# lyclyc52/NeRF_RPN

Measured on AMD Instinct MI355X. Metric: scenes/sec (160^3x4 grids, VGG19-3D+FPN+RPN fwd+bwd), higher is better.
Workload: dtype bf16; 1 GPU; configs[1]: one 160x160x160x4 rgb-sigma grid per GPU, VGG19-EF 3D + FPN + anchor RPN (OBB, 16 GT boxes per scene), fwd+bwd+clip+AdamW, random-init weights; scenes_per_gpu=1, parallelism=dp1, world_size_seen=1, backend=single process

## Files before the change

include/nerfrpn.h:

```cpp
#ifndef NERFRPN_H
#define NERFRPN_H

#include <stddef.h>
#include <stdint.h>

#ifdef __cplusplus
extern "C" {
#endif

typedef void *nrpn_stream_t;

enum nrpn_status {
  NRPN_OK = 0,
  NRPN_ERR_ARG = -1,
  NRPN_ERR_LAUNCH = -2,
  NRPN_ERR_DEVICE = -3
};

enum nrpn_dtype { NRPN_F32 = 0, NRPN_BF16 = 1 };

const char *nrpn_last_error(void);
int nrpn_abi_version(void);
int nrpn_check_device(int ordinal);

// ... 2 lines not shown
int nrpn_iou3d_obb_pair_f32(const float *b1, const float *b2, float *iou, int64_t n, nrpn_stream_t stream);
int nrpn_rotated_iou_loss_f32(const float *pred, const float *target, int64_t n, int mode, float *loss, float *grad, float *iou,
                              nrpn_stream_t stream);
int nrpn_projection_loss_f32(const float *pred, const float *target, int64_t n, int box_dim, const float *views, const float *intrinsics,
                             float beta, float max_mesh_dim, float *out, nrpn_stream_t stream);
int nrpn_recall_match_f32(float *overlaps, int num_proposals, int num_gt, float *covered, nrpn_stream_t stream);
int nrpn_ap_mark(const int64_t *order, const float *best_iou, const int64_t *key, int64_t n, int64_t num_keys, float iou_thresh,
                 int32_t *first_ws, uint8_t *tp, nrpn_stream_t stream);
int nrpn_iou3d_matrix_f32(const float *a, const float *b, float *iou, int64_t n, int64_t m, int box_dim,
                          nrpn_stream_t stream);

size_t nrpn_nms3d_workspace_bytes(int64_t n_max);
int nrpn_nms3d(const float *boxes, const int32_t *levels, const int32_t *d_count, int64_t n_max, int box_dim,
               float thr, uint8_t *keep, void *workspace, nrpn_stream_t stream);

int nrpn_segmented_topk_f32(const float *scores, const int64_t *h_offsets, int nseg, int k,
                            int32_t *out_idx, float *out_val, nrpn_stream_t stream);
size_t nrpn_segmented_topk_workspace_bytes(int nseg, int k);
int nrpn_segmented_topk_f32_ws(const float *scores, const int64_t *h_offsets, int nseg, int k,
                               int32_t *out_idx, float *out_val, void *workspace, size_t workspace_bytes, nrpn_stream_t stream);

int64_t nrpn_anchor_table_words(int levels, int anchors_per_cell);
int nrpn_anchors_f32(const int32_t *table, const int64_t *sel, int64_t count, float *anchors, nrpn_stream_t stream);
int nrpn_decode_boxes_f32(const int32_t *table, const float *deltas, const int64_t *sel, int64_t count,
                          int coder, float *boxes, nrpn_stream_t stream);
int nrpn_encode_boxes_f32(const int32_t *table, const float *gt, const int64_t *sel, int64_t count,
                          int coder, float *deltas, nrpn_stream_t stream);

int nrpn_coder_pairs_f32(const float *in, const float *anchors, int64_t count, int coder, int encode, float *out,
                         nrpn_stream_t stream);
int nrpn_head_flatten_f32(const float *head, int64_t cells, int ld, int anchors_per_cell, int dw, float *logits,
                          float *deltas, nrpn_stream_t stream);
int nrpn_head_unflatten(const float *g_logits, const float *g_deltas, int64_t cells, int ld, int anchors_per_cell, int dw,
                        const float *scale2, void *d_head, int dtype, nrpn_stream_t stream);

size_t nrpn_filter_workspace_bytes(int64_t n, int box_dim);
int nrpn_filter_candidates_f32(const float *boxes, const float *logits, const int32_t *levels,
                               const uint8_t *cand_valid, int64_t n, int box_dim, const float *h_grid_size3,
                               float min_size, float score_thresh, int fix_obb_clip, float *out_boxes,
                               float *out_scores, int32_t *out_levels, int32_t *d_count, void *workspace,
                               nrpn_stream_t stream);
int nrpn_select_kept_f32(const float *boxes, const float *scores, const int32_t *levels, const uint8_t *keep,
                         const int32_t *d_count, int64_t n, int box_dim, int post_top_n, float *out_boxes,
                         float *out_scores, float *out_levels, int32_t *d_out_count, nrpn_stream_t stream);

int nrpn_match_anchors_f32(const int32_t *table, int64_t total_anchors, const float *gt_aabb, int num_gt,
                           float fg_thresh, float bg_thresh, const float *h_ori_size3, float *labels,
                           int32_t *matched, float *workspace, nrpn_stream_t stream);
int nrpn_obb_to_aabb_f32(const float *obb, float *aabb, int64_t n, nrpn_stream_t stream);

size_t nrpn_sample_workspace_bytes(void);
int nrpn_sample_pos_neg(const float *labels, int64_t total, int max_pos, int batch, int64_t seed, void *workspace, int64_t *out_pos,
                        int64_t *out_neg, int32_t *counts, nrpn_stream_t stream);
int nrpn_rpn_sampled_loss_f32(const float *logits, const float *deltas, int dw, const float *targets,
                              const int64_t *pos, int64_t npos, const int64_t *neg, int64_t nneg, float beta,
                              float *loss2, float *g_logits, float *g_deltas, nrpn_stream_t stream);

enum { NRPN_CONV_BIAS = 1, NRPN_CONV_RELU = 2, NRPN_CONV_OUT_F32 = 4,
       NRPN_CONV_DEBUG_ALIAS_TAPS = 256, NRPN_CONV_DEBUG_NO_SYNC = 512,
       NRPN_CONV_DEBUG_STAGGER = 1024,
       NRPN_CONV_DEBUG_VARIANT = 0x3000 };
int nrpn_pack_conv_weight(const float *w_ref, int cout, int cin, int taps, int dtype, void *wp_fwd, void *wp_dgrad,
                          int rows_total, int row_offset, nrpn_stream_t stream);
int nrpn_unpack_conv_wgrad(const float *gw_packed, int cout, int cin, int taps, int rows_total, int row_offset,
                           float *gw_ref, int accumulate, int slices, nrpn_stream_t stream);
size_t nrpn_conv3d_fwd_workspace_bytes(int n, int gx, int gy, int gz, int cin, int cout, int ksize, int dtype);
int nrpn_conv3d_fwd(const void *x, const void *wp, const float *bias, void *y, int n, int gx, int gy, int gz, int cin,
                    int cout, int wrows, int ksize, int dtype, int flags, void *workspace, const void *relu_mask,
                    nrpn_stream_t stream);
enum { NRPN_TILE_AUTO = 0, NRPN_TILE_128 = 128, NRPN_TILE_256X128_WS = 256, NRPN_TILE_256X256 = 512, NRPN_TILE_256X256_W4 = 1024,
       NRPN_TILE_HALO = 2048  };
typedef struct nrpn_conv_opts {
  int32_t size;
  int32_t tile;
  int32_t lds_dma;
  int32_t kstep_bytes;
  int32_t stagger;
  int32_t big_split;
  int32_t debug;
  int32_t halo_pairing;
  const float *scale;
  const void *relu_mask;
  float *stats;
} nrpn_conv_opts;
int nrpn_conv3d_fwd_ex(const void *x, const void *wp, const float *bias, void *y, int n, int gx, int gy, int gz, int cin,
                       int cout, int wrows, int ksize, int dtype, int flags, void *workspace, const nrpn_conv_opts *opts,
                       nrpn_stream_t stream);
size_t nrpn_conv3d_fwd_workspace_bytes_ex(int n, int gx, int gy, int gz, int cin, int cout, int ksize, int dtype,
                                          const nrpn_conv_opts *opts);
int nrpn_conv3d_fwd_plan_ex(int n, int gx, int gy, int gz, int cin, int cout, int ksize, int dtype, const nrpn_conv_opts *opts);
int nrpn_conv3d_fwd_stats_rows_ex(int n, int gx, int gy, int gz, int cin, int cout, int ksize, int dtype, const nrpn_conv_opts *opts);
size_t nrpn_conv3d_wgrad_workspace_bytes(int n, int gx, int gy, int gz, int cin, int cout, int wrows, int ksize, int dtype);
int nrpn_conv3d_wgrad_slices(int n, int gx, int gy, int gz, int cin, int cout, int wrows, int ksize, int dtype);
enum { NRPN_WGRAD_ACC_BIAS = 1, NRPN_WGRAD_MASK_READY = 2,
       NRPN_WGRAD_DEFER_BIAS = 4  };
int nrpn_conv3d_wgrad(const void *x, const void *dy, float *gw_packed, float *gbias, int n, int gx, int gy, int gz,
                      int cin, int cout, int wrows, int ksize, int dtype, int accumulate_bias, void *workspace,
                      nrpn_stream_t stream);
int nrpn_conv3d_fwd_ragged(const void *x, const void *wp, const float *bias, void *y, int nseg, const int32_t *dims, int cin,
                           int cout, int wrows, int ksize, int dtype, int flags, void *workspace, nrpn_stream_t stream);
int nrpn_conv3d_wgrad_ragged(const void *x, const void *dy, float *gw_packed, float *gbias, int nseg, const int32_t *dims,
                             int cin, int cout, int wrows, int ksize, int dtype, int accumulate_bias, void *workspace,
                             nrpn_stream_t stream);
size_t nrpn_cone_workspace_bytes(int64_t total_voxels);
int nrpn_cone_build(const int64_t *pos, const int64_t *neg, const int32_t *counts, int n_scenes, int64_t pos_stride, int64_t neg_stride,
                    int nlevels, const int64_t *level_anchor_off, int num_anchors, const int32_t *dims, int depth, uint32_t *lists,
                    int64_t cap, int32_t *counts_out, void *workspace, nrpn_stream_t stream);
size_t nrpn_conv3d_fwd_rows_workspace_bytes(int64_t nrows, int cin, int cout, int ksize, int dtype);
int nrpn_conv3d_fwd_rows(const void *x, const void *wp, const float *bias, void *y, const uint32_t *rows, int64_t nrows, int nseg,
                         const int32_t *dims, int cin, int cout, int wrows, int ksize, int dtype, int flags, const void *relu_mask,
                         void *workspace, nrpn_stream_t stream);
int nrpn_conv3d_wgrad_rows(const void *x, const void *dy, float *gw_packed, float *gbias, const uint32_t *rows, int64_t nrows, int nseg,
                           const int32_t *dims, int cin, int cout, int wrows, int ksize, int dtype, int accumulate_bias, void *workspace,
                           nrpn_stream_t stream);
int nrpn_conv3d_fwd_plan(int n, int gx, int gy, int gz, int cin, int cout, int ksize, int dtype);
int nrpn_conv3d_fwd_stats_rows(int n, int gx, int gy, int gz, int cin, int cout, int ksize, int dtype);
int nrpn_conv3d_fwd_stats(const void *x, const void *wp, const float *bias, void *y, int n, int gx, int gy, int gz, int cin,
                          int cout, int wrows, int ksize, int dtype, int flags, float *stats, nrpn_stream_t stream);
int nrpn_bn_stats_finalize(const float *partials, int nparts, int64_t rows, int c, float *mean, float *var, float *running_mean,
                           float *running_var, float momentum, nrpn_stream_t stream);
int nrpn_conv3d_wgrad_plan(int n, int gx, int gy, int gz, int cin, int cout, int wrows, int ksize, int dtype);
int nrpn_stem_kpad(int dtype);
int nrpn_pack_stem_weight(const float *w_ref, int cout, int dtype, void *wp, nrpn_stream_t stream);
int nrpn_stem_wgrad_slices(int n, int gx, int gy, int gz, int cout, int stride, int dtype);
int64_t nrpn_stem_wgrad_slice_floats(int n, int gx, int gy, int gz, int cout, int stride, int dtype);
int nrpn_unpack_stem_wgrad(const float *gw_packed, int cout, int dtype, float *gw_ref, int accumulate, int slices,
                           int64_t slice_floats, nrpn_stream_t stream);
int nrpn_conv3d_stem_fwd(const void *x, const void *wp, const float *bias, void *y, int n, int gx, int gy, int gz,
                         int cout, int stride, int dtype, int flags, nrpn_stream_t stream);
int nrpn_stem_halo_supported(int gz, int cout, int stride, int dtype);
int nrpn_stem_halo_kpad(void);
int nrpn_pack_stem_weight_halo(const float *w_ref, int cout, void *wp, nrpn_stream_t stream);
int nrpn_conv3d_stem_fwd_halo(const void *x, const void *wp, const float *bias, const float *scale, void *y, int n, int gx, int gy,
                              int gz, int cout, int flags, nrpn_stream_t stream);
int nrpn_conv3d_stem_fwd_ex(const void *x, const void *wp, const float *bias, void *y, int n, int gx, int gy, int gz,
                            int cout, int stride, int dtype, int flags, const nrpn_conv_opts *opts, nrpn_stream_t stream);
size_t nrpn_stem_wgrad_workspace_bytes(int n, int gx, int gy, int gz, int cout, int stride, int dtype);
int nrpn_conv3d_stem_wgrad(const void *x, const void *dy, float *gw_packed, float *gbias, int n, int gx, int gy, int gz,
                           int cout, int stride, int dtype, int accumulate_bias, void *workspace, nrpn_stream_t stream);

size_t nrpn_bn_workspace_bytes(int64_t rows, int c);
int nrpn_bn_stats(const void *x, int64_t rows, int c, int dtype, float *mean, float *var, float *running_mean,
                  float *running_var, float momentum, void *workspace, nrpn_stream_t stream);
int nrpn_bn_apply(const void *x, void *y, int64_t rows, int c, int dtype, const float *mean, const float *var,
                  const float *gamma, const float *beta, float eps, int relu, nrpn_stream_t stream);
int nrpn_bn_backward(const void *x, const void *y, const void *dy, void *dx, int64_t rows, int c, int dtype,
                     const float *mean, const float *var, const float *gamma, const float *beta, float eps, int relu,
                     float *dgamma, float *dbeta, float *acc_dgamma, float *acc_dbeta, void *workspace, nrpn_stream_t stream);
int nrpn_relu_backward(const void *y, const void *dy, void *dx, int64_t count, int dtype, nrpn_stream_t stream);
int nrpn_pool_out_size(int in, int k, int s, int p, int ceil_mode);
int nrpn_maxpool3d_fwd(const void *x, void *y, int8_t *argmax, int n, int gx, int gy, int gz, int c, int k, int s,
                       int p, int ceil_mode, int dtype, nrpn_stream_t stream);
int nrpn_maxpool3d_bwd(const void *dy, const int8_t *argmax, void *dx, int n, int gx, int gy, int gz, int c, int k,
                       int s, int p, int ceil_mode, int dtype, nrpn_stream_t stream);
int nrpn_upsample_add_fwd(void *fine, const void *coarse, int n, int fx, int fy, int fz, int cx, int cy, int cz, int c,
                          int dtype, nrpn_stream_t stream);
int nrpn_upsample_add_bwd(const void *dfine, void *dcoarse, int n, int fx, int fy, int fz, int cx, int cy, int cz,
                          int c, int dtype, int accumulate, nrpn_stream_t stream);
int nrpn_subsample3d(const void *src, void *dst, int n, int gx, int gy, int gz, int c, int stride, int backward, int dtype,
                     nrpn_stream_t stream);
int nrpn_add_relu(const void *a, const void *b, void *y, int64_t count, int relu, int dtype, nrpn_stream_t stream);
int nrpn_ingest_rgbsigma(const void *src, int src_is_u8, void *dst, int64_t voxels, int alpha_mode, int dtype, nrpn_stream_t stream);
int nrpn_ingest_augment(const void *src, int src_is_u8, void *dst, int w, int l, int h, int alpha_mode, int dtype, int rot90,
                        int z_up, int flip0, int flip1, const float *h_xform, nrpn_stream_t stream);
int nrpn_ncdhw_to_ndhwc(const float *src, void *dst, int n, int c, int64_t voxels, int dtype, nrpn_stream_t stream);
int nrpn_ndhwc_to_ncdhw(const void *src, float *dst, int n, int c, int64_t voxels, int dtype, nrpn_stream_t stream);
int nrpn_cast(const void *src, void *dst, int64_t count, int src_dtype, int dst_dtype, nrpn_stream_t stream);
size_t nrpn_column_sum_workspace_bytes(int64_t rows, int c);
int nrpn_column_sum_f32(const float *x, int64_t rows, int c, float *out, int accumulate, void *workspace, nrpn_stream_t stream);
int nrpn_split_bf16x3(const float *src, int64_t rows, int c, void *interleaved, int ipattern, void *planes, int nplanes, int ppattern,
                      nrpn_stream_t stream);

int nrpn_patchify(const void *x, void *y, int n, int gx, int gy, int gz, int patch, int dtype, nrpn_stream_t stream);
int nrpn_layernorm_fwd(const void *x, void *y, const float *gamma, const float *beta, float *mean, float *rstd, int64_t rows,
                       int c, float eps, int dtype, nrpn_stream_t stream);
size_t nrpn_layernorm_workspace_bytes(int64_t rows, int c);
int nrpn_layernorm_bwd(const void *x, const void *dy, void *dx, const float *gamma, const float *mean, const float *rstd,
                       float *dgamma, float *dbeta, int64_t rows, int c, int dtype, int accumulate_params, void *workspace,
                       nrpn_stream_t stream);
int nrpn_gelu(const void *x, const void *dy, void *out, int64_t count, int backward, int dtype, nrpn_stream_t stream);
int nrpn_scale_add(const void *a, const void *b, const float *scale, void *y, int n, int64_t per_sample, int dtype,
                   nrpn_stream_t stream);
int nrpn_patch_merge(const void *src, void *dst, int n, int gx, int gy, int gz, int c, int backward, int dtype,
                     nrpn_stream_t stream);
int nrpn_window_attn_fwd(const void *qkv, const float *qkv_bias, const float *bias_table, const int32_t *rel_index, void *out,
                         int n, int gx, int gy, int gz, int c, int heads, int shift, int dtype, nrpn_stream_t stream);
size_t nrpn_window_attn_bwd_workspace_bytes(int n, int gx, int gy, int gz, int heads);
int nrpn_window_attn_bwd(const void *qkv, const float *qkv_bias, const float *bias_table, const int32_t *rel_index,
                         const void *dout, void *dqkv, float *dtable, float *dbias_pad, int n, int gx, int gy, int gz, int c,
                         int heads, int shift, int dtype, int accumulate_table, void *workspace, nrpn_stream_t stream);

size_t nrpn_groupnorm_workspace_bytes(int n, int c, int groups);
int nrpn_groupnorm_fwd(const void *x, void *y, const float *gamma, const float *beta, float *mean, float *rstd, int n,
                       int64_t rows, int c, int groups, float eps, int relu, int dtype, void *workspace, nrpn_stream_t stream);
int nrpn_groupnorm_bwd(const void *x, const void *y, const void *dy, void *dx, const float *gamma, const float *mean,
                       const float *rstd, float *dgamma, float *dbeta, int n, int64_t rows, int c, int groups, int relu, int dtype,
                       int accumulate_params, void *workspace, nrpn_stream_t stream);
int nrpn_fcos_reduce_floats(void);
int nrpn_fcos_head_out_f32(const float *cls_out, const float *box_out, int wrows, const float *scale, float stride_mul,
                           int norm_reg, int reg_dim, int ctr_on_reg, int64_t rows, float *logits, float *reg, float *ctr,
                           nrpn_stream_t stream);
int nrpn_fcos_head_out_bwd_f32(const float *box_out, int wrows, const float *scale, float stride_mul, int norm_reg, int reg_dim,
                               int ctr_on_reg, int64_t rows, const float *d_logits, const float *d_reg, const float *d_ctr,
                               float *d_cls_out, float *d_box_out, float *d_scale, nrpn_stream_t stream);
int nrpn_fcos_gt_summary_f32(const float *gt, int count, int width, float *summary, nrpn_stream_t stream);
int nrpn_fcos_targets_f32(const float *summary, const int32_t *gt_offsets, int n, int levels, const int32_t *dims,
                          const int32_t *strides, const float *ori_sizes, float radius, int norm_reg, int reg_dim, int8_t *labels,
                          float *reg_targets, int32_t *num_pos, nrpn_stream_t stream);
int nrpn_fcos_focal_f32(const float *logits, const int8_t *labels, int64_t count, float alpha, float *loss_sum, float *dlogits,
                        nrpn_stream_t stream);
int nrpn_fcos_scores_f32(const float *logits, const float *ctr, int n, int levels, const int32_t *dims, const int32_t *strides,
                         const float *ori_sizes, float pre_nms_thresh, float *scores, nrpn_stream_t stream);
int nrpn_fcos_decode_f32(const int32_t *idx, const float *score, int64_t count, int64_t seg_len, const float *reg, int n,
                         int levels, const int32_t *dims, const int32_t *strides, const float *ori_sizes, int reg_dim,
                         float min_size, float *boxes, float *out_scores, float *out_levels, nrpn_stream_t stream);

int nrpn_roi_align_rotated_3d_fwd(const void *feat, const float *rois, int num_rois, int n, int x, int y, int z, int c,
                                  float spatial_scale, int pw, int pl, int ph, int sampling_ratio, void *out, int dtype,
                                  nrpn_stream_t stream);
size_t nrpn_roi_align_rotated_3d_bwd_workspace_bytes(int n, int x, int y, int z, int c);
int nrpn_roi_align_rotated_3d_bwd(const void *grad_out, const float *rois, int num_rois, int n, int x, int y, int z, int c,
                                  float spatial_scale, int pw, int pl, int ph, int sampling_ratio, void *grad_in, void *workspace,
                                  int dtype, nrpn_stream_t stream);

size_t nrpn_roipool_bwd_workspace_bytes(int x, int y, int z, int c);
int nrpn_roipool_aabb_fwd(const void *feat, int x, int y, int z, int c, const int32_t *crop, const int32_t *level_of, int level, int num_rois,
                          int o0, int o1, int o2, float *out, int32_t *argmax, int dtype, nrpn_stream_t stream);
int nrpn_roipool_aabb_bwd(const float *dout, const int32_t *argmax, const int32_t *crop, const int32_t *level_of, int level, int num_rois,
                          int x, int y, int z, int c, int o0, int o1, int o2, void *dfeat, void *workspace, int dtype, nrpn_stream_t stream);
int nrpn_roipool_obb_fwd(const void *feat, int x, int y, int z, int c, const float *rois, const int32_t *level_of, int level, int num_rois,
                         float scale, int interpolation, int o0, int o1, int o2, float *out, int32_t *argmax, int dtype, nrpn_stream_t stream);
// ... 125 lines not shown
```

nerf_rpn_amd/csrc/common.h:

```cpp
#pragma once
#include <hip/hip_runtime.h>
#include <hip/hip_bf16.h>

#include <cstdarg>
#include <cstdint>
#include <cstdio>

#include "../../include/nerfrpn.h"
#include "../../include/nerfrpn_tools.h"

int nrpn_fail(int code, const char *fmt, ...);

#define NRPN_REQUIRE(cond, ...)                                 \
  do {                                                          \
    if (!(cond)) return nrpn_fail(NRPN_ERR_ARG, __VA_ARGS__);   \
  } while (0)

#define NRPN_HIP(call)                                                                          \
  do {                                                                                          \
    hipError_t e_ = (call);                                                                     \
    if (e_ != hipSuccess) return nrpn_fail(NRPN_ERR_LAUNCH, "%s: %s", #call, hipGetErrorString(e_)); \
  } while (0)

#define NRPN_LAUNCH_CHECK(name)                                                                  \
  do {                                                                                           \
    hipError_t e_ = hipGetLastError();                                                           \
    if (e_ != hipSuccess) return nrpn_fail(NRPN_ERR_LAUNCH, "%s: %s", name, hipGetErrorString(e_)); \
  } while (0)

struct FastDiv {
  unsigned m, sh, d;
};
static inline FastDiv make_fastdiv(unsigned d) {
  FastDiv f{0u, 0u, d};
  if (d <= 1) return f;
  unsigned l = 0;
  while ((1ull << l) < d) ++l;
  f.m = (unsigned)((((unsigned long long)1 << (31 + l)) + d - 1) / d);
  f.sh = l - 1;
  return f;
}
__device__ __forceinline__ unsigned fastdiv(unsigned n, const FastDiv &f) { return f.d == 1 ? n : (__umulhi(n, f.m) >> f.sh); }


int nrpn_ensure_dynamic_lds(const void *kernel, int bytes);
#define NRPN_LDS(kernel, bytes)                                                                         \
  do {                                                                                                  \
    if (int rc_ = nrpn_ensure_dynamic_lds(reinterpret_cast<const void *>(kernel), (int)(bytes))) return rc_; \
  } while (0)

static inline hipStream_t as_stream(nrpn_stream_t s) { return reinterpret_cast<hipStream_t>(s); }
static inline int64_t cdiv64(int64_t a, int64_t b) { return (a + b - 1) / b; }

__device__ __forceinline__ float bf16_bits_to_f32(unsigned short h) { return __uint_as_float(((unsigned)h) << 16); }
__device__ __forceinline__ unsigned short f32_to_bf16_bits(float f) { return __builtin_bit_cast(unsigned short, (__bf16)f); }

template <typename T> struct elem;
template <> struct elem<float> {
  static __device__ __forceinline__ float ld(const float *p) { return *p; }
  static __device__ __forceinline__ void st(float *p, float v) { *p = v; }
};
template <> struct elem<unsigned short> {
  static __device__ __forceinline__ float ld(const unsigned short *p) { return bf16_bits_to_f32(*p); }
  static __device__ __forceinline__ void st(unsigned short *p, float v) { *p = f32_to_bf16_bits(v); }
};
```

nerf_rpn_amd/csrc/conv3d.hip:

```cpp
#include "conv_common.cuh"

#ifndef NRPN_HALO_PAIRING_DEFAULT
#define NRPN_HALO_PAIRING_DEFAULT 2
#endif

template <typename T, int BN, int MODE, bool OUTF32, int KB, bool GLDS, int BM = 128, bool ROWS = false>
__global__ void __launch_bounds__(256, BM == 128 ? 2 : 1) conv_igemm_kernel(const ConvArgs p) {
  constexpr int WAVES_N = (BN == 128) ? 2 : 1;
  constexpr int TM = BM / (32 * (4 / WAVES_N));
  constexpr int TN = 2;
  constexpr int KE = KB / (int)sizeof(T);
  constexpr int PPR = KB / 16;
  constexpr int RSTEP = 256 / PPR;
  constexpr int A_RPT = BM / RSTEP;
  constexpr int B_RPT = BN / RSTEP;
  constexpr int SWZ_SH = (KB == 64) ? 2 : 1;
  constexpr int A_BYTES = BM * KB, B_BYTES = BN * KB;
  extern __shared__ __attribute__((aligned(16))) char lds[];

  const int tid = threadIdx.x, lane = tid & 63, wave = tid >> 6;
  const int wm = wave / WAVES_N, wn = wave % WAVES_N;
  const unsigned ntiles = (p.Cout + BN - 1) / BN;
  const unsigned tiles = (unsigned)((p.M + BM - 1) / BM) * ntiles;
  unsigned zsplit, tile;
  int my_ks = p.ksplit > 1 ? p.ksplit : 1;
  long long part_row0 = 0;
  if (p.tail_ks > 1) {
    const unsigned full = (unsigned)p.tail_tile0 * ntiles;
    if (blockIdx.x < full) {
      zsplit = 0; my_ks = 1;
      tile = xcd_remap(blockIdx.x, full);
    } else {
      const unsigned t = blockIdx.x - full, ntail = tiles - full;
      zsplit = t / ntail; my_ks = p.tail_ks;
      tile = full + t % ntail;
      part_row0 = (long long)p.tail_tile0 * BM;
    }
  } else {
    zsplit = blockIdx.x / tiles;
    tile = xcd_remap(blockIdx.x - zsplit * tiles, tiles);
  }
  const long long m0 = (long long)(tile / ntiles) * BM;
  const int n0 = (int)(tile % ntiles) * BN;
  const int lr = tid / PPR, ls = tid % PPR;

  long long a_off[A_RPT];
  int a_x[A_RPT], a_y[A_RPT], a_z[A_RPT];
  bool a_ok[A_RPT];
  unsigned a_mask[A_RPT];
  int a_yz[A_RPT], a_zs[A_RPT];
  long long a_nbase[A_RPT];
#pragma unroll
  for (int i = 0; i < A_RPT; ++i) {
    const long long v = m0 + lr + RSTEP * i;
    a_ok[i] = v < p.M;
    const long long vv = a_ok[i] ? v : 0;
    int ox, oy, oz, gX = p.X, gY = p.Y, gZ = p.Z;
    long long n = 0;
    unsigned row_word = 0;
    long long row_vox = vv;
    if (MODE == 0 && ROWS) {
      if (a_ok[i]) { row_vox = p.rows[2 * vv]; row_word = p.rows[2 * vv + 1]; }
      const int seg = (int)(row_word >> 27);
#pragma unroll
      for (int q = 0; q < kMaxSeg; ++q)
        if (q == seg && q < p.segs.n) { gY = p.segs.Y[q]; gZ = p.segs.Z[q]; }
      ox = oy = oz = 0;
    } else if (MODE == 0) {
      if (p.segs.n == 0) {
        const unsigned u = (unsigned)vv, sc = fastdiv(u, p.dvs), local = u - sc * (unsigned)(p.X * p.Y * p.Z), t1 = fastdiv(local, p.dvz);
        oz = (int)(local - t1 * (unsigned)p.Z);
        ox = (int)fastdiv(t1, p.dvy);
        oy = (int)(t1 - (unsigned)ox * (unsigned)p.Y);
      } else {
        locate_voxel(p.segs, vv, p.X, p.Y, p.Z, ox, oy, oz, gX, gY, gZ);
      }
    } else {
      oz = (int)(vv % p.OZ);
      const long long t1 = vv / p.OZ;
      oy = (int)(t1 % p.OY);
      const long long t2 = t1 / p.OY;
      ox = (int)(t2 % p.OX);
      n = t2 / p.OX;
    }
    a_x[i] = ox; a_y[i] = oy; a_z[i] = oz;
    a_yz[i] = gY * gZ * p.Cin * (int)sizeof(T);
    a_zs[i] = gZ * p.Cin * (int)sizeof(T);
    a_off[i] = (MODE == 0) ? row_vox * p.Cin : 0;
    a_nbase[i] = (MODE == 0) ? 0 : n * (long long)p.X * p.Y * p.Z * 4;
// ... 134 lines not shown
    const char *A = lds + buf * (A_BYTES + B_BYTES);
    const char *B = A + A_BYTES;
#pragma unroll
    for (int s = 0; s < KB / 32; ++s) {
      f4 af[TM], bfv[TN];
#pragma unroll
      for (int i = 0; i < TM; ++i) {
        const int r = (wm * TM + i) * 32 + fr;
        af[i] = *reinterpret_cast<const f4 *>(A + r * KB + (((s * 2 + fk) ^ ((r >> SWZ_SH) & (PPR - 1))) << 4));
      }
#pragma unroll
      for (int j = 0; j < TN; ++j) {
        const int r = (wn * TN + j) * 32 + fr;
        bfv[j] = *reinterpret_cast<const f4 *>(B + r * KB + (((s * 2 + fk) ^ ((r >> SWZ_SH) & (PPR - 1))) << 4));
      }
#pragma unroll
      for (int i = 0; i < TM; ++i)
#pragma unroll
        for (int j = 0; j < TN; ++j) Mma<T>::run(acc[i][j], af[i], bfv[j]);
    }
  };

  int ks = ks_begin;
  if (GLDS && MODE == 0) {
    issue_glds(0);
    __syncthreads();
    for (; ks + 1 < ks_end; ks += 2) {
      issue_glds(1);
      compute_step(0);
      __syncthreads();
      if (ks + 2 < ks_end) issue_glds(0);
      compute_step(1);
      __syncthreads();
    }
    if (ks < ks_end) {
      compute_step(0);
      __syncthreads();
    }
  } else {
    load_step(ks_begin, ra0, rb0);
    store_step(0, ra0, rb0);
    __syncthreads();
    for (; ks + 1 < ks_end; ks += 2) {
      load_step(ks + 1, ra0, rb0);
      compute_step(0);
      store_step(1, ra0, rb0);
      __syncthreads();
      if (ks + 2 < ks_end) load_step(ks + 2, ra0, rb0);
      compute_step(1);
      if (ks + 2 < ks_end) store_step(0, ra0, rb0);
      __syncthreads();
    }
    if (ks < ks_end) {
      compute_step(0);
      __syncthreads();
    }
  }

  if (my_ks > 1) {
    float *wsz = p.ws + (long long)zsplit * (p.M - part_row0) * p.Cout;
#pragma unroll
    for (int j = 0; j < TN; ++j) {
      const int col = n0 + (wn * TN + j) * 32 + fr;
      if (col >= p.Cout) continue;
#pragma unroll
      for (int i = 0; i < TM; ++i)
#pragma unroll
        for (int r = 0; r < 16; ++r) {
          const long long v = m0 + (wm * TM + i) * 32 + frag_row(r, lane);
          if (v < p.M) wsz[(v - part_row0) * p.Cout + col] = acc[i][j][r];
        }
    }
    return;
  }

  const bool has_bias = (p.flags & NRPN_CONV_BIAS) && p.bias;
  const bool relu = p.flags & NRPN_CONV_RELU;
  constexpr int PITCH = 144;
  if (sizeof(T) == 2 && !OUTF32 && 2 * (A_BYTES + B_BYTES) >= 4 * TM * 32 * PITCH && (p.Cout & 7) == 0) {
    char *stage = lds + wave * (TM * 32 * PITCH);
    const T *maskp = reinterpret_cast<const T *>(p.mask);
    T *yp = reinterpret_cast<T *>(p.y);
    const bool full_tile = m0 + BM <= p.M;
#pragma unroll
    for (int j = 0; j < TN; ++j) {
      const int col = n0 + (wn * TN + j) * 32 + fr;
      const float bv = (has_bias && col < p.Cout) ? p.bias[col] : 0.f;
      const float sv = (p.scale && col < p.Cout) ? p.scale[col] : 1.f;
      float ssum = 0.f, qsum = 0.f;
#pragma unroll
      for (int i = 0; i < TM; ++i)
#pragma unroll
        for (int r = 0; r < 16; ++r) {
          float o = acc[i][j][r] * sv + bv;
          if (relu) o = fmaxf(o, 0.f);
          const bf16s ob = f32_to_bf16_bits(o);
          *reinterpret_cast<bf16s *>(stage + (i * 32 + frag_row(r, lane)) * PITCH + (j * 32 + fr) * 2) = ob;
          if (p.stats && (full_tile || m0 + (wm * TM + i) * 32 + frag_row(r, lane) < p.M)) {
            const float of = bf16_bits_to_f32(ob);
            ssum += of;
            qsum += of * of;
          }
        }
      if (p.stats) store_col_stats(p.stats, (m0 / BM) * (BM / (TM * 32)) + wm, p.Cout, col, ssum, qsum, lane);
    }
    asm volatile("s_waitcnt lgkmcnt(0)" ::: "memory");
#pragma unroll
    for (int q = 0; q < TM * 4; ++q) {
      const int pc = lane + 64 * q;
      const int row = pc >> 3, seg = pc & 7;
      const long long vt = m0 + wm * (TM * 32) + row;
      const int col = n0 + wn * 64 + seg * 8;
      if (vt < p.M && col < p.Cout) {
        const long long v = ROWS ? (long long)p.rows[2 * vt] : vt;
        f4 val = *reinterpret_cast<const f4 *>(stage + row * PITCH + seg * 16);
        if (maskp) {
          typedef __attribute__((ext_vector_type(8))) unsigned short u8v;
          const u8v mk = __builtin_bit_cast(u8v, *reinterpret_cast<const f4 *>(maskp + v * p.Cout + col));
          u8v ov = __builtin_bit_cast(u8v, val);
#pragma unroll
          for (int e = 0; e < 8; ++e) ov[e] = (bf16_bits_to_f32(mk[e]) > 0.f) ? ov[e] : (unsigned short)0;
          val = __builtin_bit_cast(f4, ov);
        }
        *reinterpret_cast<f4 *>(yp + v * p.Cout + col) = val;
      }
    }
    return;
  }
#pragma unroll
  for (int j = 0; j < TN; ++j) {
    const int col = n0 + (wn * TN + j) * 32 + fr;
    if (col >= p.Cout) continue;
    const float bv = has_bias ? p.bias[col] : 0.f;
    const float sv = p.scale ? p.scale[col] : 1.f;
#pragma unroll
    for (int i = 0; i < TM; ++i) {
#pragma unroll
      for (int r = 0; r < 16; ++r) {
        const long long vt = m0 + (wm * TM + i) * 32 + frag_row(r, lane);
        if (vt < p.M) {
          const long long v = ROWS ? (long long)p.rows[2 * vt] : vt;
          float o = acc[i][j][r] * sv + bv;
          if (relu) o = fmaxf(o, 0.f);
          if (p.mask && !(elem<T>::ld(reinterpret_cast<const T *>(p.mask) + v * p.Cout + col) > 0.f)) o = 0.f;
          if (OUTF32) reinterpret_cast<float *>(p.y)[v * p.Cout + col] = o;
          else elem<T>::st(reinterpret_cast<T *>(p.y) + v * p.Cout + col, o);
        }
      }
    }
  }
}

template <bool OUTF32>
__global__ void __launch_bounds__(512, 1) conv_igemm_ws_kernel(const ConvArgs p) {
  typedef bf16s T;
  constexpr int BM = 256, BN = 128, KB = 128, KE = 64, PPR = 8, RSTEP = 32, TM = 4, TN = 2;
  constexpr int A_RPT = BM / RSTEP, B_RPT = BN / RSTEP;
  constexpr int A_BYTES = BM * KB, B_BYTES = BN * KB;
  extern __shared__ __attribute__((aligned(16))) char lds[];

  const int tid = threadIdx.x, lane = tid & 63, wave = tid >> 6;
  const bool producer = wave >= 4;
  const unsigned ntiles = (p.Cout + BN - 1) / BN;
  const unsigned tiles = (unsigned)((p.M + BM - 1) / BM) * ntiles;
  const unsigned tile = xcd_remap(blockIdx.x, tiles);
  const long long m0 = (long long)(tile / ntiles) * BM;
  const int n0 = (int)(tile % ntiles) * BN;
  const int cpt = p.Cin / KE;
  const int nk = p.taps * cpt;

  if (producer) {
    const int ptid = tid - 256, lr = ptid / PPR, ls = ptid % PPR;
    const int wave_u = __builtin_amdgcn_readfirstlane(wave - 4);
    const __amdgpu_buffer_rsrc_t xr = make_rsrc(p.x, p.x_bytes), wr = make_rsrc(p.w, p.w_bytes);
    unsigned a_voff[A_RPT], a_mask[A_RPT], b_voff[B_RPT];
#pragma unroll
    for (int i = 0; i < A_RPT; ++i) {
      const int r = lr + RSTEP * i;
      const long long v = m0 + r;
      const bool ok = v < p.M;
      const long long vv = ok ? v : 0;
      const int oz = (int)(vv % p.OZ);
      const long long t1 = vv / p.OZ;
      const int oy = (int)(t1 % p.OY);
      const int ox = (int)((t1 / p.OY) % p.OX);
      unsigned m = 0;
      if (ok) {
        if (p.taps == 27) {
#pragma unroll
          for (int t = 0; t < 27; ++t) {
            const int dx = t / 9 - 1, dy = (t / 3) % 3 - 1, dz = t % 3 - 1;
            const bool in = (unsigned)(ox + dx) < (unsigned)p.X && (unsigned)(oy + dy) < (unsigned)p.Y && (unsigned)(oz + dz) < (unsigned)p.Z;
            m |= in ? (1u << t) : 0u;
          }
        } else {
          m = 1u;
        }
      }
      a_mask[i] = m;
      a_voff[i] = (unsigned)(vv * p.Cin * 2) + ((ls ^ ((r >> 1) & (PPR - 1))) << 4);
    }
#pragma unroll
    for (int i = 0; i < B_RPT; ++i) {
      const int r = lr + RSTEP * i, row = n0 + r;
      b_voff[i] = row < p.wrows ? (unsigned)((long long)row * p.Cin * 2) + ((ls ^ ((r >> 1) & (PPR - 1))) << 4) : kOOB;
    }
    int l_tap = 0, l_chunk = 0, l_dx = 0, l_dy = 0, l_dz = 0;
    if (p.taps == 27) { l_dx = -1; l_dy = -1; l_dz = -1; }
    const long long w_tap_stride = (long long)p.wrows * p.Cin;
// ... 640 lines not shown
      for (int q = 0; q < 8; ++q) {
        const int pc = elane + 64 * q;
        const int row = pc >> 4, seg = pc & 15;
        const long long v = m0 + (wm * TM + i) * 32 + row;
        const int col = n0 + wn * 128 + seg * 8;
        if (v < p.M && col < p.Cout) {
          f4 val = *reinterpret_cast<const f4 *>(stage + row * PITCH + seg * 16);
          if (maskp) {
            typedef __attribute__((ext_vector_type(8))) unsigned short u8v;
            const u8v mk = __builtin_bit_cast(u8v, *reinterpret_cast<const f4 *>(maskp + v * p.Cout + col));
            u8v ov = __builtin_bit_cast(u8v, val);
#pragma unroll
            for (int e = 0; e < 8; ++e) ov[e] = (bf16_bits_to_f32(mk[e]) > 0.f) ? ov[e] : (unsigned short)0;
            val = __builtin_bit_cast(f4, ov);
          }
          *reinterpret_cast<f4 *>(yp + v * p.Cout + col) = val;
        }
      }
      asm volatile("s_waitcnt lgkmcnt(0)" ::: "memory");
    }
    if (p.stats) {
#pragma unroll
      for (int j = 0; j < TN; ++j)
        store_col_stats(p.stats, (m0 / BM) * 2 + wm, p.Cout, n0 + (wn * TN + j) * 32 + efr, ssum[j], qsum[j], elane);
    }
    return;
  }
#pragma unroll
  for (int j = 0; j < TN; ++j) {
    const int col = n0 + (wn * TN + j) * 32 + efr;
    if (col >= p.Cout) continue;
    const float bv = has_bias ? p.bias[col] : 0.f;
    const float sv = p.scale ? p.scale[col] : 1.f;
#pragma unroll
    for (int i = 0; i < TM; ++i) {
#pragma unroll
      for (int r = 0; r < 16; ++r) {
        const long long v = m0 + (wm * TM + i) * 32 + frag_row(r, elane);
        if (v < p.M) {
          float o = acc[i][j][r] * sv + bv;
          if (relu) o = fmaxf(o, 0.f);
          if (p.mask && !(elem<T>::ld(reinterpret_cast<const T *>(p.mask) + v * p.Cout + col) > 0.f)) o = 0.f;
          if (OUTF32) reinterpret_cast<float *>(p.y)[v * p.Cout + col] = o;
          else elem<T>::st(reinterpret_cast<T *>(p.y) + v * p.Cout + col, o);
        }
      }
    }
  }
}

namespace hk { constexpr int TX = 4, TY = 8, TZ = 8; }
int nrpn_launch_conv_halo(const ConvArgs &a, unsigned workgroups, hipStream_t st, int variant);

template <typename T, bool OUTF32>
__global__ void splitk_epilogue_kernel(const float *__restrict__ ws, const float *__restrict__ bias, void *__restrict__ y, long long total,
                                       int cout, int relu, int nslices, const T *__restrict__ mask, const float *__restrict__ scale) {
  for (long long i = (long long)blockIdx.x * blockDim.x + threadIdx.x; i < total; i += (long long)gridDim.x * blockDim.x) {
    float o = ws[i];
    for (int z = 1; z < nslices; ++z) o += ws[z * total + i];
    if (scale) o *= scale[i % cout];
    o += bias ? bias[i % cout] : 0.f;
    if (relu) o = fmaxf(o, 0.f);
    if (mask && !(elem<T>::ld(mask + i) > 0.f)) o = 0.f;
    if (OUTF32) reinterpret_cast<float *>(y)[i] = o;
    else elem<T>::st(reinterpret_cast<T *>(y) + i, o);
  }
}

template <typename T, bool OUTF32>
__global__ void rows_epilogue_kernel(const float *__restrict__ ws, const float *__restrict__ bias, void *__restrict__ y, long long total,
                                     int cout, int relu, int nslices, const T *__restrict__ mask, const unsigned *__restrict__ rows) {
  for (long long i = (long long)blockIdx.x * blockDim.x + threadIdx.x; i < total; i += (long long)gridDim.x * blockDim.x) {
    float o = ws[i];
    for (int z = 1; z < nslices; ++z) o += ws[z * total + i];
    const long long r = i / cout;
    const int col = (int)(i - r * cout);
    const long long dst = (long long)rows[2 * r] * cout + col;
    o += bias ? bias[col] : 0.f;
    if (relu) o = fmaxf(o, 0.f);
    if (mask && !(elem<T>::ld(mask + dst) > 0.f)) o = 0.f;
    if (OUTF32) reinterpret_cast<float *>(y)[dst] = o;
    else elem<T>::st(reinterpret_cast<T *>(y) + dst, o);
  }
}

struct Knobs {
  int glds;
  int bm;
  int stagger;
  int big_split;
  int kb;
  int dbg;
  int halo_auto;
  int halo_xp;
};
static std::atomic<int> g_conv_glds{1}, g_conv_bm{0}, g_conv_stagger{1}, g_conv_big_split{1}, g_conv_kb{128}, g_conv_halo_auto{1}, g_conv_halo_xp{NRPN_HALO_PAIRING_DEFAULT};
static Knobs resolve_knobs(const nrpn_conv_opts *o, int flags = 0) {
  Knobs k{g_conv_glds.load(std::memory_order_relaxed), g_conv_bm.load(std::memory_order_relaxed), g_conv_stagger.load(std::memory_order_relaxed),
          g_conv_big_split.load(std::memory_order_relaxed), g_conv_kb.load(std::memory_order_relaxed),
          flags & (NRPN_CONV_DEBUG_ALIAS_TAPS | NRPN_CONV_DEBUG_NO_SYNC | NRPN_CONV_DEBUG_STAGGER | NRPN_CONV_DEBUG_VARIANT), g_conv_halo_auto.load(std::memory_order_relaxed),
          g_conv_halo_xp.load(std::memory_order_relaxed)};
  if (o) {
    if (o->halo_pairing == 1 || o->halo_pairing == 2) k.halo_xp = o->halo_pairing == 1 ? 1 : 0;
    if (o->tile > 0) k.bm = o->tile;
    if (o->lds_dma >= 0) k.glds = o->lds_dma ? 1 : 0;
    if (o->kstep_bytes == 64 || o->kstep_bytes == 128) k.kb = o->kstep_bytes;
    if (o->stagger >= 0) k.stagger = o->stagger ? 1 : 0;
    if (o->big_split >= 0) k.big_split = o->big_split ? 1 : 0;
    k.dbg |= o->debug & (NRPN_CONV_DEBUG_ALIAS_TAPS | NRPN_CONV_DEBUG_NO_SYNC | NRPN_CONV_DEBUG_STAGGER | NRPN_CONV_DEBUG_VARIANT);
  }
  return k;
}
extern "C" int nrpn_set_conv_lds_dma(int on) { g_conv_glds = on ? 1 : 0; return NRPN_OK; }
extern "C" int nrpn_set_conv_halo_auto(int on) { g_conv_halo_auto = on ? 1 : 0; return NRPN_OK; }
extern "C" int nrpn_set_conv_halo_pairing(int mode) { g_conv_halo_xp = (mode == 1 || mode == 2) ? mode : 0; return NRPN_OK; }
extern "C" int nrpn_set_conv_stagger(int on) { g_conv_stagger = on ? 1 : 0; return NRPN_OK; }
extern "C" int nrpn_set_conv_big_split(int on) { g_conv_big_split = on ? 1 : 0; return NRPN_OK; }
extern "C" int nrpn_set_conv_kstep_bytes(int kb) {
  if (kb != 64 && kb != 128) return nrpn_fail(NRPN_ERR_ARG, "conv k-step must be 64 or 128 bytes");
  g_conv_kb = kb;
  return NRPN_OK;
}
extern "C" int nrpn_set_conv_tile_m(int bm) {
  if (bm != 0 && bm != 128 && bm != 256 && bm != 512 && bm != 1024 && bm != 2048)
    return nrpn_fail(NRPN_ERR_ARG, "conv tile selector must be 0 (auto), 128 (128x128), 256 (wave-specialised 256x128), 512 (256x256, 8 waves), "
                                   "1024 (256x256, 4 waves) or 2048 (halo form of the 3x3x3 kernel)");
  g_conv_bm = bm;
  return NRPN_OK;
}

static int conv_ksplit(long long M, int cout, int cin, int taps, int elem_bytes, const Knobs &kn) {
  const int bn = cout <= 64 ? 64 : 128;
  const long long tiles = cdiv64(M, 128) * ((cout + bn - 1) / bn);
  const int kb = (kn.kb == 128 && (cin * elem_bytes) % 128 == 0) ? 128 : 64;
  const int nk = taps * (cin * elem_bytes / kb);
  if (tiles >= 128 || nk < 16) return 1;
  long long s = (384 + tiles - 1) / tiles;
  if (s > nk / 8) s = nk / 8;
  if (s > 64) s = 64;
  if (s < 2) return 1;
  const long long per = (nk + s - 1) / s;
  s = (nk + per - 1) / per;
  return s < 2 ? 1 : (int)s;
}

static int conv_big_split(long long M, int cout, int cin, int taps, int elem_bytes, const Knobs &kn) {
  if (!kn.big_split) return 0;
  if (elem_bytes != 2 || !kn.glds || kn.kb != 128 || (kn.bm != 0 && kn.bm != 512 && kn.bm != 1024) || cout < 256 || (cin * 2) % 128 != 0) return 0;
  const long long tiles = cdiv64(M, 256) * ((cout + 255) / 256);
  if (tiles < 48 || tiles >= 200) return 0;
  const int nk = taps * (cin / 64);
  int s = (int)((256 + tiles - 1) / tiles);
  if (s > 8) s = 8;
  while (s > 1 && nk / s < 8) --s;
  return s >= 2 ? s : 0;
}

struct TailSplit { int tile0, ks; };
static TailSplit conv_tail_split(long long M, int cout, int cin, int taps, int elem_bytes, const Knobs &kn) {
  TailSplit none{0, 0};
  if (elem_bytes != 2 || !kn.glds || kn.kb != 128 || !kn.big_split || cout > 256 || cout < 256 || (cin * 2) % 128 != 0) return none;
  const long long tiles = cdiv64(M, 256);
  const long long rem = tiles % 256;
  if (tiles <= 256 || rem == 0 || rem > 128) return none;
  const int nk = taps * (cin / 64);
  int ks = (int)(256 / rem);
  if (ks > 8) ks = 8;
  while (ks > 1 && nk / ks < 8) --ks;
  if (ks < 2) return none;
  const int per = (nk + ks - 1) / ks;
  ks = (nk + per - 1) / per;
  return ks >= 2 ? TailSplit{(int)(tiles - rem), ks} : none;
}

template <typename K>
static int launch_igemm(K kernel, dim3 grid, size_t lds, hipStream_t st, const ConvArgs &a) {
  if (lds > 64 * 1024) NRPN_LDS(kernel, (int)lds);
  hipLaunchKernelGGL(kernel, grid, dim3(256), lds, st, a);
  return NRPN_OK;
}

struct Grid { int n, gx, gy, gz; };
static long long halo_tiles(const Grid &g) {
  return (long long)g.n * ((g.gx + hk::TX - 1) / hk::TX) * ((g.gy + hk::TY - 1) / hk::TY) * ((g.gz + hk::TZ - 1) / hk::TZ);
}
static bool halo_ok(const Grid &g, int cin, int cout, int taps, int elem_bytes, bool out_f32, const Knobs &kn) {
  (void)out_f32;
  if (g.n <= 0 || taps != 27 || elem_bytes != 2 || !kn.glds || (cin % 32) != 0 || (cout & 7) != 0 || cout < 256) return false;
  if (kn.bm != 2048 && !(kn.bm == 0 && kn.halo_auto)) return false;
  const long long tiles = halo_tiles(g) * ((cout + 255) / 256);
  const double waste = (double)halo_tiles(g) * 256.0 / ((double)g.n * g.gx * g.gy * g.gz);
  if (kn.bm == 2048) return true;
  return tiles >= 200 && waste <= 1.12;
}

static int conv_tile_kind(long long M, int cout, int cin, int elem_bytes, bool sliced_big, bool ragged, const Knobs &kn) {
  const bool wide = kn.kb == 128 && (cin * elem_bytes) % 128 == 0;
  const bool can = kn.glds && wide && cout > 64 && elem_bytes == 2;
  const long long tiles_big = cdiv64(M, 256) * ((cout + 255) / 256);
  const bool huge = can && cout >= 256 && (sliced_big || kn.bm == 512 || kn.bm == 1024 || (kn.bm == 0 && tiles_big >= 200));
  if (huge) return (kn.bm == 1024 && !ragged) ? 5 : 1;
  if (can && kn.bm == 256 && !ragged) return 4;
  return 0;
}

template <typename T, int MODE>
static int launch_conv(const ConvArgs &a, bool out_f32, hipStream_t st, const Knobs &kn) {
  const int bn = (a.Cout <= 64) ? 64 : 128;
  constexpr bool kDma = (MODE == 0);
  const bool wide = MODE == 0 && kn.kb == 128 && (a.Cin * (int)sizeof(T)) % 128 == 0;
  const int kind = (kDma && (a.ksplit <= 1 || a.slices)) ? conv_tile_kind(a.M, a.Cout, a.Cin, (int)sizeof(T), a.slices != 0, a.segs.n > 0, kn) : 0;
  const bool huge = kind == 1 || kind == 5, big = kind == 4;
  const int bm = (big || huge) ? 256 : 128;
  if (a.stats) {
    const bool staged = MODE == 0 && sizeof(T) == 2 && !out_f32 && (a.Cout & 7) == 0 && a.ksplit <= 1 && !big && (huge || wide);
    if (!staged) return nrpn_fail(NRPN_ERR_ARG, "conv3d_fwd_stats: this shape does not run a kernel with fused statistics (ask nrpn_conv3d_fwd_stats_rows first)");
  }
  dim3 grid((unsigned)(cdiv64(a.M, bm) * ((a.Cout + (huge ? 256 : bn) - 1) / (huge ? 256 : bn)) * (a.ksplit > 1 ? a.ksplit : 1)));
  if (a.tail_ks > 1) {
    if (kind != 1) return nrpn_fail(NRPN_ERR_ARG, "conv3d_fwd: internal: tail split planned for a shape that does not run the 256x256 tile");
    const long long mt = cdiv64(a.M, 256), nt = (a.Cout + 255) / 256;
    grid = dim3((unsigned)(a.tail_tile0 * nt + (mt - a.tail_tile0) * nt * a.tail_ks));
  }
  int rc = 0;
#define NRPN_LC(BN_, OF_, KB_)                                                                                                    \
  do {                                                                                                                           \
    const size_t lds_ = 2 * (size_t)(128 + BN_) * KB_;                                                                           \
    if (kDma && kn.glds) rc = launch_igemm(conv_igemm_kernel<T, BN_, MODE, OF_, KB_, kDma>, grid, lds_, st, a);                  \
    else rc = launch_igemm(conv_igemm_kernel<T, BN_, MODE, OF_, KB_, false>, grid, lds_, st, a);                                 \
  } while (0)
#define NRPN_LC2(BN_, OF_) do { if (wide) NRPN_LC(BN_, OF_, 128); else NRPN_LC(BN_, OF_, 64); } while (0)
#define NRPN_LBIG(...)                                                                       \
  do {                                                                                       \
    NRPN_LDS((conv_igemm_big_kernel<__VA_ARGS__>), (int)lds_);                               \
    hipLaunchKernelGGL((conv_igemm_big_kernel<__VA_ARGS__>), grid, dim3(512), lds_, st, a);  \
  } while (0)
  if (kind == 5) {
    if constexpr (MODE == 0 && sizeof(T) == 2) {
      const size_t lds_ = 2 * (size_t)(256 + 256) * 128;
      if (out_f32) {
        NRPN_LDS((conv_igemm_big4_kernel<true>), (int)lds_);
        hipLaunchKernelGGL(conv_igemm_big4_kernel<true>, grid, dim3(256), lds_, st, a);
      } else {
        NRPN_LDS((conv_igemm_big4_kernel<false>), (int)lds_);
        hipLaunchKernelGGL(conv_igemm_big4_kernel<false>, grid, dim3(256), lds_, st, a);
      }
    }
  } else if (huge) {
    if constexpr (MODE == 0 && sizeof(T) == 2) {
      const size_t lds_ = 2 * (size_t)(256 + 256) * 128;
      const int dbg = ((kn.dbg & NRPN_CONV_DEBUG_ALIAS_TAPS) ? 1 : 0) | ((kn.dbg & NRPN_CONV_DEBUG_NO_SYNC) ? 2 : 0);
      if (!out_f32 && (kn.stagger || (kn.dbg & NRPN_CONV_DEBUG_STAGGER))) {
        if (dbg == 0) NRPN_LBIG(false, true, 0);
        else if (dbg == 1) NRPN_LBIG(false, true, 1);
        else if (dbg == 2) NRPN_LBIG(false, true, 2);
        else NRPN_LBIG(false, true, 3);
      } else if (out_f32) {
        NRPN_LBIG(true, false, 0);
      } else {
        NRPN_LBIG(false, false, 0);
      }
    }
  } else if (big) {
    if constexpr (MODE == 0 && sizeof(T) == 2) {
      const size_t lds_ = 3 * (size_t)(256 + 128) * 128;
      if (out_f32) {
        NRPN_LDS((conv_igemm_ws_kernel<true>), (int)lds_);
        hipLaunchKernelGGL(conv_igemm_ws_kernel<true>, grid, dim3(512), lds_, st, a);
      } else {
        NRPN_LDS((conv_igemm_ws_kernel<false>), (int)lds_);
        hipLaunchKernelGGL(conv_igemm_ws_kernel<false>, grid, dim3(512), lds_, st, a);
      }
    }
  } else if (bn == 64) { if (out_f32) NRPN_LC2(64, true); else NRPN_LC2(64, false); }
  else { if (out_f32) NRPN_LC2(128, true); else NRPN_LC2(128, false); }
#undef NRPN_LBIG
#undef NRPN_LC2
#undef NRPN_LC
  if (rc) return rc;
  NRPN_LAUNCH_CHECK("conv_igemm");
  return NRPN_OK;
}

static size_t fwd_workspace_bytes(long long M, int cin, int cout, int ksize, int dtype, const Knobs &kn, const Grid &g) {
  if (halo_ok(g, cin, cout, ksize == 3 ? 27 : 1, dtype == NRPN_F32 ? 4 : 2, false, kn)) return 0;
  const int bs = conv_big_split(M, cout, cin, ksize == 3 ? 27 : 1, dtype == NRPN_F32 ? 4 : 2, kn);
  if (bs) return (size_t)bs * M * cout * 4;
  const int s = conv_ksplit(M, cout, cin, ksize == 3 ? 27 : 1, dtype == NRPN_F32 ? 4 : 2, kn);
  if (s > 1) return (size_t)s * M * cout * 4;
  if (conv_tile_kind(M, cout, cin, dtype == NRPN_F32 ? 4 : 2, false, false, kn) == 1) {
    const TailSplit t = conv_tail_split(M, cout, cin, ksize == 3 ? 27 : 1, dtype == NRPN_F32 ? 4 : 2, kn);
    if (t.ks > 1) return (size_t)t.ks * (M - (long long)t.tile0 * 256) * cout * 4;
  }
  return 0;
}
extern "C" size_t nrpn_conv3d_fwd_workspace_bytes(int n, int gx, int gy, int gz, int cin, int cout, int ksize, int dtype) {
  return fwd_workspace_bytes((long long)n * gx * gy * gz, cin, cout, ksize, dtype, resolve_knobs(nullptr), Grid{n, gx, gy, gz});
}
extern "C" size_t nrpn_conv3d_fwd_workspace_bytes_ex(int n, int gx, int gy, int gz, int cin, int cout, int ksize, int dtype,
                                                     const nrpn_conv_opts *opts) {
  return fwd_workspace_bytes((long long)n * gx * gy * gz, cin, cout, ksize, dtype, resolve_knobs(opts), Grid{n, gx, gy, gz});
}

static int fwd_plan(long long M, int cin, int cout, int ksize, int dtype, const Knobs &kn, const Grid &g) {
  const int es = dtype == NRPN_F32 ? 4 : 2, taps = ksize == 3 ? 27 : 1;
  if (halo_ok(g, cin, cout, taps, es, false, kn)) return 7;
  if (conv_big_split(M, cout, cin, taps, es, kn)) return conv_tile_kind(M, cout, cin, es, true, false, kn) == 5 ? 6 : 2;
  if (conv_ksplit(M, cout, cin, taps, es, kn) > 1) return 3;
  return conv_tile_kind(M, cout, cin, es, false, false, kn);
}
extern "C" int nrpn_conv3d_fwd_plan(int n, int gx, int gy, int gz, int cin, int cout, int ksize, int dtype) {
  return fwd_plan((long long)n * gx * gy * gz, cin, cout, ksize, dtype, resolve_knobs(nullptr), Grid{n, gx, gy, gz});
}
extern "C" int nrpn_conv3d_fwd_plan_ex(int n, int gx, int gy, int gz, int cin, int cout, int ksize, int dtype, const nrpn_conv_opts *opts) {
  return fwd_plan((long long)n * gx * gy * gz, cin, cout, ksize, dtype, resolve_knobs(opts), Grid{n, gx, gy, gz});
}

static int conv3d_fwd_impl(const void *x, const void *wp, const float *bias, const void *mask, void *y, long long M, int gx, int gy, int gz, const Segs *segs,
                           int cin, int cout, int wrows, int ksize, int dtype, int flags, void *workspace, nrpn_stream_t stream,
                           float *stats = nullptr, const nrpn_conv_opts *opts = nullptr) {
  NRPN_REQUIRE(ksize == 1 || ksize == 3, "conv3d_fwd: ksize must be 1 or 3 (got %d)", ksize);
  NRPN_REQUIRE(dtype == NRPN_F32 || dtype == NRPN_BF16, "conv3d_fwd: bad dtype %d", dtype);
  NRPN_REQUIRE(M > 0 && gx > 0 && gy > 0 && gz > 0 && cin > 0 && cout > 0 && wrows >= cout, "conv3d_fwd: bad sizes");
  const int es = dtype == NRPN_F32 ? 4 : 2;
  NRPN_REQUIRE((cin * es) % 64 == 0, "conv3d_fwd: Cin*elemsize must be a multiple of 64 bytes (Cin=%d)", cin);
  NRPN_REQUIRE(x && wp && y, "conv3d_fwd: null pointer");
  const Knobs kn = resolve_knobs(opts, flags);
  ConvArgs a{};
  a.x = x; a.w = wp; a.bias = bias; a.mask = mask; a.y = y; a.stats = stats;
  a.scale = opts ? opts->scale : nullptr;
  a.M = M;
  a.X = gx; a.Y = gy; a.Z = gz; a.OX = gx; a.OY = gy; a.OZ = gz;
  if (segs) a.segs = *segs;
  a.dvz = make_fastdiv((unsigned)gz); a.dvy = make_fastdiv((unsigned)gy);
  a.dvs = make_fastdiv((unsigned)min((long long)gx * gy * gz, (1ll << 31) - 1));
  a.Cin = cin; a.Cout = cout; a.wrows = wrows; a.taps = ksize == 3 ? 27 : 1; a.stride = 1;
  a.flags = flags & 3;
  NRPN_REQUIRE(a.M * cin * es < (1ll << 31) && (long long)a.taps * wrows * cin * es < (1ll << 31),
               "conv3d_fwd: activation / weight tensors must stay below 2 GiB (32-bit buffer offsets)");
  a.x_bytes = (unsigned)(a.M * cin * es); a.w_bytes = (unsigned)((long long)a.taps * wrows * cin * es);
  const bool out_f32 = (flags & NRPN_CONV_OUT_F32) != 0;
  hipStream_t st = as_stream(stream);
  if (!segs && dtype == NRPN_BF16) {
    const Grid g{(int)(M / ((long long)gx * gy * gz)), gx, gy, gz};
    if (halo_ok(g, cin, cout, a.taps, es, out_f32, kn)) {
      const long long wgs = halo_tiles(g) * ((cout + 255) / 256);
      NRPN_REQUIRE(wgs < (1ll << 31), "conv3d_fwd: too many tiles");
      const bool xp = cin % 128 == 0 && !((kn.dbg >> 12) & 3) && (kn.halo_xp == 1 || (kn.halo_xp == 2 && cin >= 256));
      const int variant = ((kn.dbg >> 12) & 3) | (xp ? 4 : 0) | (out_f32 ? 8 : 0);
      return nrpn_launch_conv_halo(a, (unsigned)wgs, st, variant);
    }
  }
  const int bs = workspace ? conv_big_split(a.M, cout, cin, a.taps, es, kn) : 0;
  if (bs) {
    a.ksplit = bs; a.slices = 1; a.ws = reinterpret_cast<float *>(workspace);
  } else {
    a.ksplit = workspace ? conv_ksplit(a.M, cout, cin, a.taps, es, kn) : 1;
    if (a.ksplit > 1) a.ws = reinterpret_cast<float *>(workspace);
  }
  const int nsl = a.ksplit;
  if (a.ksplit <= 1 && workspace && !segs && !stats && !out_f32 && dtype == NRPN_BF16 && conv_tile_kind(a.M, cout, cin, es, false, false, kn) == 1) {
    const TailSplit t = conv_tail_split(a.M, cout, cin, a.taps, es, kn);
    if (t.ks > 1) { a.tail_tile0 = t.tile0; a.tail_ks = t.ks; a.ws = reinterpret_cast<float *>(workspace); }
  }
  int rc = (dtype == NRPN_F32) ? launch_conv<float, 0>(a, true, st, kn) : launch_conv<bf16s, 0>(a, out_f32, st, kn);
  if (!rc && a.tail_ks > 1) {
    const long long row0 = (long long)a.tail_tile0 * 256, total = (a.M - row0) * cout;
    const int blocks = (int)min((long long)2048, (total + 255) / 256);
    const float *b = (flags & NRPN_CONV_BIAS) ? bias : nullptr;
    const bf16s *mk = a.mask ? reinterpret_cast<const bf16s *>(a.mask) + row0 * cout : nullptr;
    hipLaunchKernelGGL((splitk_epilogue_kernel<bf16s, false>), dim3(blocks), dim3(256), 0, st, a.ws, b, reinterpret_cast<bf16s *>(y) + row0 * cout, total, cout,
                       (flags & NRPN_CONV_RELU) ? 1 : 0, a.tail_ks, mk, a.scale);
    NRPN_LAUNCH_CHECK("splitk_epilogue (tail)");
    return NRPN_OK;
  }
  if (rc || a.ksplit <= 1) return rc;
  const long long total = a.M * cout;
  const int blocks = (int)min((long long)4096, (total + 255) / 256);
  const float *b = (flags & NRPN_CONV_BIAS) ? bias : nullptr;
  const int relu = (flags & NRPN_CONV_RELU) ? 1 : 0;
  if (dtype == NRPN_F32 || out_f32) {
    if (dtype == NRPN_F32) hipLaunchKernelGGL((splitk_epilogue_kernel<float, true>), dim3(blocks), dim3(256), 0, st, a.ws, b, y, total, cout, relu, nsl, (const float *)a.mask, a.scale);
    else hipLaunchKernelGGL((splitk_epilogue_kernel<bf16s, true>), dim3(blocks), dim3(256), 0, st, a.ws, b, y, total, cout, relu, nsl, (const bf16s *)a.mask, a.scale);
  } else {
    hipLaunchKernelGGL((splitk_epilogue_kernel<bf16s, false>), dim3(blocks), dim3(256), 0, st, a.ws, b, y, total, cout, relu, nsl, (const bf16s *)a.mask, a.scale);
  }
  NRPN_LAUNCH_CHECK("splitk_epilogue");
  return NRPN_OK;
}

extern "C" int nrpn_conv3d_fwd(const void *x, const void *wp, const float *bias, void *y, int n, int gx, int gy, int gz, int cin,
                               int cout, int wrows, int ksize, int dtype, int flags, void *workspace, const void *relu_mask,
                               nrpn_stream_t stream) {
  NRPN_REQUIRE(n > 0 && gx > 0 && gy > 0 && gz > 0, "conv3d_fwd: bad sizes");
  NRPN_REQUIRE(!relu_mask || !(flags & NRPN_CONV_OUT_F32) || dtype == NRPN_F32, "conv3d_fwd: relu_mask needs outputs in the input dtype");
  return conv3d_fwd_impl(x, wp, bias, relu_mask, y, (long long)n * gx * gy * gz, gx, gy, gz, nullptr, cin, cout, wrows, ksize, dtype, flags,
                         workspace, stream);
}

static int fwd_stats_rows(long long M, int cin, int cout, int ksize, int dtype, const Knobs &kn, const Grid &g) {
  if (dtype != NRPN_BF16 || (cout & 7) != 0 || !kn.glds || kn.bm == 256) return 0;
  const int plan = fwd_plan(M, cin, cout, ksize, dtype, kn, g);
  if (plan == 7) return (int)(halo_tiles(g) * 2);
  if (plan == 1 || plan == 5) return (int)(cdiv64(M, 256) * 2);
  if (plan != 0 || kn.kb != 128 || (cin * 2) % 128 != 0) return 0;
  return (int)(cdiv64(M, 128) * (cout <= 64 ? 4 : 2));
}
extern "C" int nrpn_conv3d_fwd_stats_rows(int n, int gx, int gy, int gz, int cin, int cout, int ksize, int dtype) {
  return fwd_stats_rows((long long)n * gx * gy * gz, cin, cout, ksize, dtype, resolve_knobs(nullptr), Grid{n, gx, gy, gz});
}
extern "C" int nrpn_conv3d_fwd_stats_rows_ex(int n, int gx, int gy, int gz, int cin, int cout, int ksize, int dtype, const nrpn_conv_opts *opts) {
  return fwd_stats_rows((long long)n * gx * gy * gz, cin, cout, ksize, dtype, resolve_knobs(opts), Grid{n, gx, gy, gz});
}

extern "C" int nrpn_conv3d_fwd_stats(const void *x, const void *wp, const float *bias, void *y, int n, int gx, int gy, int gz, int cin,
                                     int cout, int wrows, int ksize, int dtype, int flags, float *stats, nrpn_stream_t stream) {
  NRPN_REQUIRE(n > 0 && gx > 0 && gy > 0 && gz > 0 && stats, "conv3d_fwd_stats: bad sizes / null statistics buffer");
  NRPN_REQUIRE(nrpn_conv3d_fwd_stats_rows(n, gx, gy, gz, cin, cout, ksize, dtype) > 0 && !(flags & NRPN_CONV_OUT_F32) && wrows == cout,
               "conv3d_fwd_stats: this shape does not run a kernel with fused statistics");
  return conv3d_fwd_impl(x, wp, bias, nullptr, y, (long long)n * gx * gy * gz, gx, gy, gz, nullptr, cin, cout, wrows, ksize, dtype, flags,
                         nullptr, stream, stats);
}

extern "C" int nrpn_conv3d_fwd_ex(const void *x, const void *wp, const float *bias, void *y, int n, int gx, int gy, int gz, int cin,
                                  int cout, int wrows, int ksize, int dtype, int flags, void *workspace, const nrpn_conv_opts *opts,
                                  nrpn_stream_t stream) {
  NRPN_REQUIRE(n > 0 && gx > 0 && gy > 0 && gz > 0, "conv3d_fwd_ex: bad sizes");
  NRPN_REQUIRE(!opts || opts->size == (int32_t)sizeof(nrpn_conv_opts), "conv3d_fwd_ex: opts->size must be sizeof(nrpn_conv_opts)");
  const void *mask = opts ? opts->relu_mask : nullptr;
  float *stats = opts ? opts->stats : nullptr;
  NRPN_REQUIRE(!mask || !(flags & NRPN_CONV_OUT_F32) || dtype == NRPN_F32, "conv3d_fwd_ex: relu_mask needs outputs in the input dtype");
  if (stats) {
    NRPN_REQUIRE(fwd_stats_rows((long long)n * gx * gy * gz, cin, cout, ksize, dtype, resolve_knobs(opts), Grid{n, gx, gy, gz}) > 0 && !(flags & NRPN_CONV_OUT_F32) &&
                     wrows == cout && !mask,
                 "conv3d_fwd_ex: this shape / plan does not run a kernel with fused statistics (nrpn_conv3d_fwd_stats_rows_ex)");
    workspace = nullptr;
  }
  return conv3d_fwd_impl(x, wp, bias, mask, y, (long long)n * gx * gy * gz, gx, gy, gz, nullptr, cin, cout, wrows, ksize, dtype, flags,
                         workspace, stream, stats, opts);
}

extern "C" int nrpn_conv3d_fwd_ragged(const void *x, const void *wp, const float *bias, void *y, int nseg, const int32_t *dims, int cin,
                                      int cout, int wrows, int ksize, int dtype, int flags, void *workspace, nrpn_stream_t stream) {
  Segs sg{};
  long long M = 0;
  if (int rc = fill_segs(sg, nseg, dims, M)) return rc;
  return conv3d_fwd_impl(x, wp, bias, nullptr, y, M, 1, 1, 1, &sg, cin, cout, wrows, ksize, dtype, flags, workspace, stream);
}

static std::atomic<int> g_rows_big{0};
extern "C" int nrpn_set_rows_big_tile(int on) { g_rows_big = on ? 1 : 0; return NRPN_OK; }

static int rows_ksplit(long long nrows, int cin, int cout, int taps, int es) {
  const long long tiles = cdiv64(nrows, 128) * ((cout + 127) / 128);
  const int nk = taps * (cin * es / 128);
  if (tiles >= 128 || nk < 12) return 1;
  long long s = (256 + tiles - 1) / tiles;
  if (s > nk / 6) s = nk / 6;
  if (s > 32) s = 32;
  if (s < 2) return 1;
  const long long per = (nk + s - 1) / s;
  s = (nk + per - 1) / per;
  return s < 2 ? 1 : (int)s;
}
static std::atomic<int> g_rows_tail{1};
extern "C" int nrpn_set_rows_tail_split(int on) { g_rows_tail = on ? 1 : 0; return NRPN_OK; }
static TailSplit rows_tail_split(long long nrows, int cin, int cout, int taps, int es) {
  TailSplit none{0, 0};
  if (!g_rows_tail.load(std::memory_order_relaxed)) return none;
  const long long mt = cdiv64(nrows, 128), nt = (cout + 127) / 128, tiles = mt * nt;
  const long long rem = tiles % 512;
  if (tiles <= 512 || rem == 0 || rem > 256) return none;
  const long long tail_mt = (rem + nt - 1) / nt;
  const int nk = taps * (cin * es / 128);
  int ks = (int)(512 / (tail_mt * nt));
  if (ks > 8) ks = 8;
  while (ks > 1 && nk / ks < 6) --ks;
  if (ks < 2) return none;
  const int per = (nk + ks - 1) / ks;
  ks = (nk + per - 1) / per;
  return ks >= 2 ? TailSplit{(int)(mt - tail_mt), ks} : none;
}
extern "C" size_t nrpn_conv3d_fwd_rows_workspace_bytes(int64_t nrows, int cin, int cout, int ksize, int dtype) {
  const int es = dtype == NRPN_F32 ? 4 : 2, taps = ksize == 3 ? 27 : 1;
  const int s = rows_ksplit(nrows, cin, cout, taps, es);
  if (s > 1) return (size_t)s * nrows * cout * 4;
  const TailSplit t = rows_tail_split(nrows, cin, cout, taps, es);
  return t.ks > 1 ? (size_t)t.ks * (nrows - (long long)t.tile0 * 128) * cout * 4 : 0;
}

extern "C" int nrpn_conv3d_fwd_rows(const void *x, const void *wp, const float *bias, void *y, const uint32_t *rows, int64_t nrows, int nseg,
                                    const int32_t *dims, int cin, int cout, int wrows, int ksize, int dtype, int flags, const void *relu_mask,
                                    void *workspace, nrpn_stream_t stream) {
  NRPN_REQUIRE(ksize == 1 || ksize == 3, "conv3d_fwd_rows: ksize must be 1 or 3 (got %d)", ksize);
  NRPN_REQUIRE(dtype == NRPN_F32 || dtype == NRPN_BF16, "conv3d_fwd_rows: bad dtype %d", dtype);
  NRPN_REQUIRE(x && wp && y && rows && nrows >= 0 && cin > 0 && cout > 0 && wrows >= cout, "conv3d_fwd_rows: bad arguments");
  if (nrows == 0) return NRPN_OK;
  const int es = dtype == NRPN_F32 ? 4 : 2;
  NRPN_REQUIRE((cin * es) % 128 == 0, "conv3d_fwd_rows: Cin*elemsize must be a multiple of 128 bytes (Cin=%d)", cin);
  const bool out_f32 = (flags & NRPN_CONV_OUT_F32) != 0 || dtype == NRPN_F32;
  NRPN_REQUIRE(!relu_mask || !(flags & NRPN_CONV_OUT_F32) || dtype == NRPN_F32, "conv3d_fwd_rows: relu_mask needs outputs in the input dtype");
  ConvArgs a{};
  long long total = 0;
  if (int rc = fill_segs(a.segs, nseg, dims, total)) return rc;
  a.x = x; a.w = wp; a.bias = bias; a.mask = relu_mask; a.y = y; a.rows = rows;
  a.M = nrows;
  a.X = a.Y = a.Z = a.OX = a.OY = a.OZ = 1;
  a.Cin = cin; a.Cout = cout; a.wrows = wrows; a.taps = ksize == 3 ? 27 : 1; a.stride = 1; a.flags = flags & 3; a.ksplit = 1;
  NRPN_REQUIRE(total * cin * es < (1ll << 31) && total * cout * 4 < (1ll << 32) && (long long)a.taps * wrows * cin * es < (1ll << 31),
               "conv3d_fwd_rows: activation / weight tensors must stay below 2 GiB (32-bit buffer offsets)");
  a.x_bytes = (unsigned)(total * cin * es); a.w_bytes = (unsigned)((long long)a.taps * wrows * cin * es);
  hipStream_t st = as_stream(stream);
  const int ks = workspace ? rows_ksplit(nrows, cin, cout, a.taps, es) : 1;
  if (ks > 1) { a.ksplit = ks; a.ws = reinterpret_cast<float *>(workspace); }
  if (g_rows_big.load(std::memory_order_relaxed) && dtype == NRPN_BF16 && !out_f32 && ks == 1 && cout >= 256 && (cout & 7) == 0 &&
      cdiv64(nrows, 256) * ((cout + 255) / 256) >= 96) {
    const size_t lds_big = 2 * (size_t)(256 + 256) * 128;
    dim3 gbig((unsigned)(cdiv64(nrows, 256) * ((cout + 255) / 256)));
    NRPN_LDS((conv_igemm_big_kernel<false, true, 0, true>), (int)lds_big);
    hipLaunchKernelGGL((conv_igemm_big_kernel<false, true, 0, true>), gbig, dim3(512), lds_big, st, a);
    NRPN_LAUNCH_CHECK("conv3d_fwd_rows (256x256 tile)");
    return NRPN_OK;
  }
  dim3 grid((unsigned)(cdiv64(nrows, 128) * ((cout + 127) / 128) * ks));
  if (ks == 1 && workspace) {
    const TailSplit t = rows_tail_split(nrows, cin, cout, a.taps, es);
    if (t.ks > 1) {
      a.tail_tile0 = t.tile0; a.tail_ks = t.ks; a.ws = reinterpret_cast<float *>(workspace);
      const long long mt = cdiv64(nrows, 128), nt = (cout + 127) / 128;
      grid = dim3((unsigned)(t.tile0 * nt + (mt - t.tile0) * nt * t.ks));
    }
  }
  const size_t lds_ = 2 * (size_t)(128 + 128) * 128;
  int rc;
  if (dtype == NRPN_F32) rc = launch_igemm(conv_igemm_kernel<float, 128, 0, true, 128, true, 128, true>, grid, lds_, st, a);
  else if (out_f32) rc = launch_igemm(conv_igemm_kernel<bf16s, 128, 0, true, 128, true, 128, true>, grid, lds_, st, a);
  else rc = launch_igemm(conv_igemm_kernel<bf16s, 128, 0, false, 128, true, 128, true>, grid, lds_, st, a);
  if (rc) return rc;
  NRPN_LAUNCH_CHECK("conv3d_fwd_rows");
  if (ks > 1 || a.tail_ks > 1) {
    const long long row0 = a.tail_ks > 1 ? (long long)a.tail_tile0 * 128 : 0;
    const int nsl = a.tail_ks > 1 ? a.tail_ks : ks;
    const long long total = (nrows - row0) * cout;
    const int blocks = (int)min((long long)2048, (total + 255) / 256);
    const float *b = (flags & NRPN_CONV_BIAS) ? bias : nullptr;
    const int relu = (flags & NRPN_CONV_RELU) ? 1 : 0;
    const uint32_t *rw = rows + 2 * row0;
    if (dtype == NRPN_F32) hipLaunchKernelGGL((rows_epilogue_kernel<float, true>), dim3(blocks), dim3(256), 0, st, a.ws, b, y, total, cout, relu, nsl, (const float *)relu_mask, rw);
    else if (out_f32) hipLaunchKernelGGL((rows_epilogue_kernel<bf16s, true>), dim3(blocks), dim3(256), 0, st, a.ws, b, y, total, cout, relu, nsl, (const bf16s *)relu_mask, rw);
    else hipLaunchKernelGGL((rows_epilogue_kernel<bf16s, false>), dim3(blocks), dim3(256), 0, st, a.ws, b, y, total, cout, relu, nsl, (const bf16s *)relu_mask, rw);
    NRPN_LAUNCH_CHECK("rows_epilogue");
  }
  return NRPN_OK;
}

static int stem_fwd_impl(const void *x, const void *wp, const float *bias, void *y, int n, int gx, int gy, int gz, int cout,
                         int stride, int dtype, int flags, const nrpn_conv_opts *opts, nrpn_stream_t stream) {
  NRPN_REQUIRE(stride == 1 || stride == 2, "stem: stride must be 1 or 2 (got %d)", stride);
  NRPN_REQUIRE(dtype == NRPN_F32 || dtype == NRPN_BF16, "stem: bad dtype %d", dtype);
  NRPN_REQUIRE(n > 0 && gx > 0 && gy > 0 && gz > 0 && cout > 0, "stem: bad sizes");
  NRPN_REQUIRE(x && wp && y, "stem: null pointer");
  NRPN_REQUIRE(!opts || opts->size == (int32_t)sizeof(nrpn_conv_opts), "stem: opts->size must be sizeof(nrpn_conv_opts)");
  NRPN_REQUIRE(!opts || (!opts->relu_mask && !opts->stats), "stem: relu_mask / stats are not available on the stem");
  ConvArgs a{};
  a.x = x; a.w = wp; a.bias = bias; a.y = y;
  a.scale = opts ? opts->scale : nullptr;
  a.X = gx; a.Y = gy; a.Z = gz;
  a.OX = (gx + 6 - 7) / stride + 1; a.OY = (gy + 6 - 7) / stride + 1; a.OZ = (gz + 6 - 7) / stride + 1;
  a.M = (long long)n * a.OX * a.OY * a.OZ;
  a.Cin = 4; a.Cout = cout; a.wrows = cout; a.taps = 343; a.stride = stride; a.flags = flags & 3;
  {
    const long long xb = (long long)n * gx * gy * gz * 4 * (dtype == NRPN_F32 ? 4 : 2);
    NRPN_REQUIRE(xb < (1ll << 31), "stem: input must stay below 2 GiB");
    a.x_bytes = (unsigned)xb; a.w_bytes = 0;
  }
  const Knobs kn = resolve_knobs(opts);
  if (dtype == NRPN_F32) return launch_conv<float, 1>(a, true, as_stream(stream), kn);
  return launch_conv<bf16s, 1>(a, false, as_stream(stream), kn);
}

extern "C" int nrpn_conv3d_stem_fwd(const void *x, const void *wp, const float *bias, void *y, int n, int gx, int gy, int gz, int cout,
                                    int stride, int dtype, int flags, nrpn_stream_t stream) {
  return stem_fwd_impl(x, wp, bias, y, n, gx, gy, gz, cout, stride, dtype, flags, nullptr, stream);
}

extern "C" int nrpn_conv3d_stem_fwd_ex(const void *x, const void *wp, const float *bias, void *y, int n, int gx, int gy, int gz, int cout,
                                       int stride, int dtype, int flags, const nrpn_conv_opts *opts, nrpn_stream_t stream) {
  return stem_fwd_impl(x, wp, bias, y, n, gx, gy, gz, cout, stride, dtype, flags, opts, stream);
}


struct StemHaloArgs {
  const void *x, *w;
  const float *bias, *scale;
  void *y;
  int N, X, Y, Z, OX, OY, OZ;
  int tx, ty, tz;
  int flags;
  unsigned x_bytes, w_bytes;
};
namespace sh {
constexpr int TX = 4, TY = 4, TZ = 16, HX = 13, HY = 14, PITCH = 320, PPRZ = PITCH / 16;
constexpr int HALO_PIECES = HX * HY * PPRZ;
constexpr int HALO_INSTR = (HALO_PIECES + 63) / 64;
constexpr int HALO_BYTES = HALO_INSTR * 1024;
constexpr int KTAPS = 50, KROW = KTAPS * 32;
constexpr int B_BYTES = 64 * 128;
constexpr int LDS_BYTES = HALO_BYTES + 2 * B_BYTES;
}

__global__ void __launch_bounds__(256, 2) stem_fwd_halo_kernel(const StemHaloArgs p) {
  using namespace sh;
  typedef bf16s T;
  extern __shared__ __attribute__((aligned(16))) char lds[];
  char *halo = lds;
  char *Bt = lds + HALO_BYTES;
  const int tid = threadIdx.x, lane = tid & 63, wave = tid >> 6;
  const int wave_u = __builtin_amdgcn_readfirstlane(wave);
  unsigned t = blockIdx.x;
  const int tzi = (int)(t % p.tz); t /= p.tz;
  const int tyi = (int)(t % p.ty); t /= p.ty;
  const int txi = (int)(t % p.tx);
  const int n = (int)(t / p.tx);
  const int ox0 = txi * TX, oy0 = tyi * TY, oz0 = tzi * TZ;

  const __amdgpu_buffer_rsrc_t xr = make_rsrc(p.x, p.x_bytes), wr = make_rsrc(p.w, p.w_bytes);
#pragma unroll 1
  for (int inst = wave_u; inst < HALO_INSTR; inst += 4) {
    const int q = inst * 64 + lane;
    const int row = q / PPRZ, pz = q - row * PPRZ;
    const int hx = row / HY, hy = row - hx * HY;
    const int ix = 2 * ox0 - 3 + hx, iy = 2 * oy0 - 3 + hy, iz = 2 * oz0 - 4 + 2 * pz;
    const bool ok = q < HALO_PIECES && hy < 13 && (unsigned)ix < (unsigned)p.X && (unsigned)iy < (unsigned)p.Y && iz >= 0 && iz + 2 <= p.Z;
    const unsigned off = ok ? (unsigned)(((((long long)n * p.X + ix) * p.Y + iy) * p.Z + iz) * 8) : kOOB;
    lds_dma16(xr, halo + inst * 1024, off);
  }
  const int br = tid >> 3, bs = tid & 7;
  unsigned b_voff[2];
#pragma unroll
  for (int i = 0; i < 2; ++i) {
    const int r = br + 32 * i;
    b_voff[i] = (unsigned)(r * KROW * 2) + ((bs ^ ((r >> 1) & 7)) << 4);
  }
  auto issue_b = [&](int buf, int ks) {
#pragma unroll
    for (int i = 0; i < 2; ++i) lds_dma16(wr, Bt + buf * B_BYTES + (wave_u * 8 + 32 * i) * 128, b_voff[i] + (unsigned)(ks * 128));
// ... 1301 lines not shown
```

nerf_rpn_amd/csrc/conv_common.cuh:

```cuda
#pragma once
#include "common.h"

#include <atomic>

typedef __attribute__((ext_vector_type(4))) float f4;
typedef __attribute__((ext_vector_type(2))) float f2;
typedef __attribute__((ext_vector_type(16))) float f16v;
typedef __attribute__((ext_vector_type(8))) __bf16 bf8;
typedef __attribute__((ext_vector_type(4))) short s4v;
typedef unsigned short bf16s;


template <typename T> struct Mma;
template <> struct Mma<float> {
  static __device__ __forceinline__ void run(f16v &acc, const f4 &a, const f4 &b) {
    acc = __builtin_amdgcn_mfma_f32_32x32x2f32(a[0], b[0], acc, 0, 0, 0);
    acc = __builtin_amdgcn_mfma_f32_32x32x2f32(a[1], b[1], acc, 0, 0, 0);
    acc = __builtin_amdgcn_mfma_f32_32x32x2f32(a[2], b[2], acc, 0, 0, 0);
    acc = __builtin_amdgcn_mfma_f32_32x32x2f32(a[3], b[3], acc, 0, 0, 0);
  }
};
template <> struct Mma<bf16s> {
  static __device__ __forceinline__ void run(f16v &acc, const f4 &a, const f4 &b) {
    acc = __builtin_amdgcn_mfma_f32_32x32x16_bf16(__builtin_bit_cast(bf8, a), __builtin_bit_cast(bf8, b), acc, 0, 0, 0);
// ... 16 lines not shown
  return (xcd < r ? xcd * (q + 1) : r * (q + 1) + (xcd - r) * q) + slot;
}

__device__ __forceinline__ void lds_dma16(__amdgpu_buffer_rsrc_t r, void *lds_dst, unsigned voff) {
  __builtin_amdgcn_raw_ptr_buffer_load_lds(r, (__attribute__((address_space(3))) void *)lds_dst, 16, voff, 0, 0, 0);
}

__device__ __forceinline__ int frag_row(int r, int lane) { return (r & 3) + 8 * (r >> 2) + 4 * (lane >> 5); }

constexpr int kMaxSeg = 16;
struct Segs {
  int n;
  int start[kMaxSeg + 1];
  int X[kMaxSeg], Y[kMaxSeg], Z[kMaxSeg];
};

__device__ __forceinline__ int locate_voxel(const Segs &s, long long v, int cX, int cY, int cZ, int &x, int &y, int &z, int &X, int &Y,
                                            int &Z) {
  int seg = 0;
  long long local = v;
  if (s.n > 0) {
    X = s.X[0]; Y = s.Y[0]; Z = s.Z[0];
    int st = 0;
#pragma unroll
    for (int k = 1; k < kMaxSeg; ++k)
      if (k < s.n && v >= s.start[k]) { X = s.X[k]; Y = s.Y[k]; Z = s.Z[k]; st = s.start[k]; seg = k; }
    local = v - st;
  } else {
    X = cX; Y = cY; Z = cZ;
  }
  z = (int)(local % Z);
  const long long t1 = local / Z;
  y = (int)(t1 % Y);
  x = (int)((t1 / Y) % X);
  return seg;
}

__device__ __forceinline__ unsigned tap_mask27(int x, int y, int z, int X, int Y, int Z) {
  const unsigned mz = (z > 0 ? 1u : 0u) | 2u | (z + 1 < Z ? 4u : 0u);
  const unsigned my = (y > 0 ? 1u : 0u) | 2u | (y + 1 < Y ? 4u : 0u);
  const unsigned m9 = (my & 1u ? mz : 0u) | (my & 2u ? mz << 3 : 0u) | (my & 4u ? mz << 6 : 0u);
  return (x > 0 ? m9 : 0u) | (m9 << 9) | (x + 1 < X ? m9 << 18 : 0u);
}

static inline int fill_segs(Segs &sg, int nseg, const int32_t *dims, long long &M) {
  if (nseg < 1 || nseg > kMaxSeg || !dims) return nrpn_fail(NRPN_ERR_ARG, "ragged conv: 1..%d segments", kMaxSeg);
  sg.n = nseg;
  long long off = 0;
  for (int k = 0; k < nseg; ++k) {
    if (dims[3 * k] <= 0 || dims[3 * k + 1] <= 0 || dims[3 * k + 2] <= 0) return nrpn_fail(NRPN_ERR_ARG, "ragged conv: bad segment %d", k);
    sg.start[k] = (int)off; sg.X[k] = dims[3 * k]; sg.Y[k] = dims[3 * k + 1]; sg.Z[k] = dims[3 * k + 2];
    off += (long long)dims[3 * k] * dims[3 * k + 1] * dims[3 * k + 2];
    if (off >= (1ll << 31)) return nrpn_fail(NRPN_ERR_ARG, "ragged conv: too many voxels");
  }
  for (int k = nseg; k <= kMaxSeg; ++k) sg.start[k] = (int)off;
  M = off;
  return 0;
}

struct ConvArgs {
  const void *x;
  const void *w;
  const float *bias;
  const float *scale;
  const void *mask;
  void *y;
  long long M;
  int X, Y, Z;
  int OX, OY, OZ;
  int Cin, Cout;
  int wrows;
  int taps;
  int stride;
  int flags;
  unsigned x_bytes, w_bytes;
  int ksplit;
  float *ws;
  int slices;
  Segs segs;
  int tail_tile0, tail_ks;
  const unsigned *rows;
  FastDiv dvz, dvy, dvs;
  float *stats;
};

__device__ __forceinline__ void store_col_stats(float *stats, long long pidx, int cout, int col, float s, float q, int lane) {
  s += __shfl_xor(s, 32, 64);
  q += __shfl_xor(q, 32, 64);
  if (lane < 32 && col < cout) {
    stats[(pidx * 2) * cout + col] = s;
    stats[(pidx * 2 + 1) * cout + col] = q;
  }
}
```

nerf_rpn_amd/csrc/elementwise.hip:

```cpp
#include "common.h"
#include <atomic>

typedef unsigned short bf16s;
typedef __attribute__((ext_vector_type(4))) float f4;
typedef __attribute__((ext_vector_type(4))) unsigned short us4;

template <typename T> struct vec4;
template <> struct vec4<float> {
  static __device__ __forceinline__ f4 ld(const float *p) { return *reinterpret_cast<const f4 *>(p); }
  static __device__ __forceinline__ void st(float *p, f4 v) { *reinterpret_cast<f4 *>(p) = v; }
};
template <> struct vec4<bf16s> {
  static __device__ __forceinline__ f4 ld(const bf16s *p) {
    const us4 u = *reinterpret_cast<const us4 *>(p);
    f4 v = {bf16_bits_to_f32(u[0]), bf16_bits_to_f32(u[1]), bf16_bits_to_f32(u[2]), bf16_bits_to_f32(u[3])};
    return v;
  }
  static __device__ __forceinline__ void st(bf16s *p, f4 v) {
    typedef __attribute__((ext_vector_type(4))) __bf16 b4;
    *reinterpret_cast<us4 *>(p) = __builtin_bit_cast(us4, __builtin_convertvector(v, b4));
  }
};

template <typename T, int V> struct vecv;
template <typename T> struct vecv<T, 4> {
  static __device__ __forceinline__ void ld(const T *p, float *o) { const f4 v = vec4<T>::ld(p); o[0] = v[0]; o[1] = v[1]; o[2] = v[2]; o[3] = v[3]; }
  static __device__ __forceinline__ void st(T *p, const float *o) { vec4<T>::st(p, f4{o[0], o[1], o[2], o[3]}); }
};
template <> struct vecv<bf16s, 8> {
  typedef __attribute__((ext_vector_type(8))) unsigned short us8;
  static __device__ __forceinline__ void ld(const bf16s *p, float *o) {
    const us8 u = *reinterpret_cast<const us8 *>(p);
#pragma unroll
    for (int q = 0; q < 8; ++q) o[q] = bf16_bits_to_f32(u[q]);
  }
  static __device__ __forceinline__ void st(bf16s *p, const float *o) {
    typedef __attribute__((ext_vector_type(8))) float f8;
    typedef __attribute__((ext_vector_type(8))) __bf16 b8;
    const f8 v = {o[0], o[1], o[2], o[3], o[4], o[5], o[6], o[7]};
    *reinterpret_cast<us8 *>(p) = __builtin_bit_cast(us8, __builtin_convertvector(v, b8));
  }
};

#define DISPATCH_T(dtype, ...)                       \
  if ((dtype) == NRPN_F32) { typedef float T; __VA_ARGS__; } \
  else { typedef bf16s T; __VA_ARGS__; }

static inline int slab_rows(long long rows) { const long long s = (rows + 1023) / 1024; return (int)(s < 64 ? 64 : s); }

#ifndef NRPN_CHAN_UNROLL
#define NRPN_CHAN_UNROLL 4
#endif
template <typename T, int MODE, int V>
__global__ void __launch_bounds__(256)
chan_partial_kernel(const T *__restrict__ x, const T *__restrict__ y, const T *__restrict__ dy, long long rows, int c,
                    const float *__restrict__ mean, const float *__restrict__ var, float eps, int relu, float *__restrict__ partial,
                    int kSlab, const float *__restrict__ gamma = nullptr, const float *__restrict__ beta = nullptr) {
  __shared__ float red[2][256][V];
  const int cw = min(c, 1024), coff = blockIdx.y * 1024;
  x += coff; y = y ? y + coff : y; dy = dy ? dy + coff : dy;
  if (MODE == 1) { mean += coff; var += coff; if (beta) { gamma += coff; beta += coff; } }
  const int ct = min(cw, c - coff) / V;
  const int ty_n = 256 / ct;
  const int tx = threadIdx.x % ct, ty = threadIdx.x / ct;
  const long long r0 = (long long)blockIdx.x * kSlab, r1 = min(rows, r0 + kSlab);
  float s0[V], s1[V];
#pragma unroll
  for (int k = 0; k < V; ++k) { s0[k] = 0.f; s1[k] = 0.f; }
  if (ty < ty_n) {
    float mu[V], is[V], ga[V], be[V];
#pragma unroll
    for (int k = 0; k < V; ++k) { mu[k] = 0.f; is[k] = 1.f; ga[k] = 1.f; be[k] = 0.f; }
    if (MODE == 1) {
#pragma unroll
      for (int k = 0; k < V; ++k) {
        mu[k] = mean[tx * V + k];
        is[k] = 1.0f / sqrtf(var[tx * V + k] + eps);
        if (beta) { ga[k] = gamma[tx * V + k]; be[k] = beta[tx * V + k]; }
      }
    }
#pragma unroll NRPN_CHAN_UNROLL
    for (long long r = r0 + ty; r < r1; r += ty_n) {
      float xv[V];
      vecv<T, V>::ld(x + r * c + tx * V, xv);
      if (MODE == 0) {
#pragma unroll
        for (int k = 0; k < V; ++k) { s0[k] += xv[k]; s1[k] += xv[k] * xv[k]; }
      } else {
        float g[V];
        vecv<T, V>::ld(dy + r * c + tx * V, g);
        if (relu && beta) {
#pragma unroll
          for (int k = 0; k < V; ++k) g[k] = ((xv[k] - mu[k]) * is[k] * ga[k] + be[k]) > 0.f ? g[k] : 0.f;
        } else if (relu) {
          float yv[V];
          vecv<T, V>::ld(y + r * c + tx * V, yv);
#pragma unroll
          for (int k = 0; k < V; ++k) g[k] = yv[k] > 0.f ? g[k] : 0.f;
        }
#pragma unroll
        for (int k = 0; k < V; ++k) { s0[k] += g[k]; s1[k] += g[k] * ((xv[k] - mu[k]) * is[k]); }
      }
    }
  }
#pragma unroll
  for (int k = 0; k < V; ++k) { red[0][threadIdx.x][k] = s0[k]; red[1][threadIdx.x][k] = s1[k]; }
  __syncthreads();
  if (threadIdx.x < ct) {
    float a[V], b[V];
#pragma unroll
    for (int k = 0; k < V; ++k) { a[k] = 0.f; b[k] = 0.f; }
    for (int q = 0; q < ty_n; ++q)
#pragma unroll
      for (int k = 0; k < V; ++k) { a[k] += red[0][q * ct + threadIdx.x][k]; b[k] += red[1][q * ct + threadIdx.x][k]; }
    float *out = partial + (long long)blockIdx.x * 2 * c + coff;
#pragma unroll
    for (int k = 0; k < V; k += 4) {
      *reinterpret_cast<f4 *>(out + threadIdx.x * V + k) = f4{a[k], a[k + 1], a[k + 2], a[k + 3]};
      *reinterpret_cast<f4 *>(out + c + threadIdx.x * V + k) = f4{b[k], b[k + 1], b[k + 2], b[k + 3]};
    }
  }
}
static std::atomic<int> g_chan_v8{0};
extern "C" int nrpn_set_bn_reduce_v8(int on) { g_chan_v8 = on ? 1 : 0; return NRPN_OK; }
static inline bool chan_v8(int dtype, int c, const void *a, const void *b, const void *d) {
  const int tile = c > 1024 ? 1024 : c;
  return dtype == NRPN_BF16 && c % 8 == 0 && tile % 8 == 0 && 256 % (tile / 8) == 0 &&
         ((reinterpret_cast<uintptr_t>(a) | reinterpret_cast<uintptr_t>(b) | reinterpret_cast<uintptr_t>(d)) & 15) == 0;
}

constexpr int kFinCh = 16, kFinLanes = 64;
__device__ __forceinline__ void reduce_partials(const float *__restrict__ partial, int nblocks, int c, int ch, double &s, double &q) {
  __shared__ double rs[kFinLanes][kFinCh], rq[kFinLanes][kFinCh];
  __shared__ double rs2[4][kFinCh], rq2[4][kFinCh];
  double a = 0.0, b = 0.0;
  if (ch < c) {
    double a2[2] = {0.0, 0.0}, b2[2] = {0.0, 0.0};
    int blk = threadIdx.y;
    for (; blk + kFinLanes < nblocks; blk += 2 * kFinLanes) {
#pragma unroll
      for (int u = 0; u < 2; ++u) {
        a2[u] += (double)partial[(long long)(blk + kFinLanes * u) * 2 * c + ch];
        b2[u] += (double)partial[(long long)(blk + kFinLanes * u) * 2 * c + c + ch];
      }
    }
    for (; blk < nblocks; blk += kFinLanes) {
      a2[0] += (double)partial[(long long)blk * 2 * c + ch];
      b2[0] += (double)partial[(long long)blk * 2 * c + c + ch];
    }
    a = a2[0] + a2[1];
    b = b2[0] + b2[1];
  }
  rs[threadIdx.y][threadIdx.x] = a;
  rq[threadIdx.y][threadIdx.x] = b;
  __syncthreads();
  if (threadIdx.y < 4) {
    double t = 0.0, u = 0.0;
    for (int k = 0; k < kFinLanes / 4; ++k) { t += rs[threadIdx.y * (kFinLanes / 4) + k][threadIdx.x]; u += rq[threadIdx.y * (kFinLanes / 4) + k][threadIdx.x]; }
    rs2[threadIdx.y][threadIdx.x] = t;
    rq2[threadIdx.y][threadIdx.x] = u;
  }
  __syncthreads();
  s = 0.0; q = 0.0;
  if (threadIdx.y == 0)
    for (int k = 0; k < 4; ++k) { s += rs2[k][threadIdx.x]; q += rq2[k][threadIdx.x]; }
}

__global__ void bn_stats_finalize_kernel(const float *__restrict__ partial, int nblocks, long long rows, int c, float *__restrict__ mean,
                                         float *__restrict__ var, float *__restrict__ rmean, float *__restrict__ rvar, float momentum) {
  const int ch = blockIdx.x * kFinCh + threadIdx.x;
  double s, q;
  reduce_partials(partial, nblocks, c, ch, s, q);
  if (threadIdx.y != 0 || ch >= c) return;
  const double m = s / (double)rows;
  double v = q / (double)rows - m * m;
  if (v < 0.0) v = 0.0;
  mean[ch] = (float)m;
  var[ch] = (float)v;
  if (rmean) {
    const double unbiased = rows > 1 ? v * (double)rows / (double)(rows - 1) : v;
    rmean[ch] = (float)((1.0 - momentum) * (double)rmean[ch] + momentum * m);
    rvar[ch] = (float)((1.0 - momentum) * (double)rvar[ch] + momentum * unbiased);
  }
}

__global__ void bn_bwd_finalize_kernel(const float *__restrict__ partial, int nblocks, int c, float *__restrict__ dbeta,
                                       float *__restrict__ dgamma, float *__restrict__ acc_beta, float *__restrict__ acc_gamma) {
  const int ch = blockIdx.x * kFinCh + threadIdx.x;
  double s, q;
  reduce_partials(partial, nblocks, c, ch, s, q);
  if (threadIdx.y != 0 || ch >= c) return;
  dbeta[ch] = (float)s;
  dgamma[ch] = (float)q;
  if (acc_beta) acc_beta[ch] += (float)s;
  if (acc_gamma) acc_gamma[ch] += (float)q;
}

extern "C" size_t nrpn_bn_workspace_bytes(int64_t rows, int c) { return (size_t)(cdiv64(rows, slab_rows(rows)) * 2 * c * 4); }

static int check_bn_shape(const char *who, int64_t rows, int c) {
  const int tile = c > 1024 ? 1024 : c;
  if (rows <= 0 || c <= 0 || c % 4 != 0 || c % tile != 0 || 256 % (tile / 4) != 0)
    return nrpn_fail(NRPN_ERR_ARG, "%s: C=%d must be a multiple of 4 with min(C,1024)/4 dividing 256 and C %% 1024 == 0 above 1024 (rows=%lld)", who, c, (long long)rows);
  return 0;
}

extern "C" int nrpn_bn_stats(const void *x, int64_t rows, int c, int dtype, float *mean, float *var, float *running_mean,
                             float *running_var, float momentum, void *workspace, nrpn_stream_t stream) {
  if (int rc = check_bn_shape("bn_stats", rows, c)) return rc;
  NRPN_REQUIRE(x && mean && var && workspace, "bn_stats: null pointer");
  const int kSlab = slab_rows(rows);
  const int nb = (int)cdiv64(rows, kSlab);
  hipStream_t st = as_stream(stream);
  if (g_chan_v8.load(std::memory_order_relaxed) && chan_v8(dtype, c, x, nullptr, nullptr)) {
    hipLaunchKernelGGL((chan_partial_kernel<bf16s, 0, 8>), dim3(nb, (c + 1023) / 1024), dim3(256), 0, st, (const bf16s *)x, (const bf16s *)nullptr,
                       (const bf16s *)nullptr, (long long)rows, c, (const float *)nullptr, (const float *)nullptr, 0.f, 0, (float *)workspace, kSlab);
  } else {
    DISPATCH_T(dtype, hipLaunchKernelGGL((chan_partial_kernel<T, 0, 4>), dim3(nb, (c + 1023) / 1024), dim3(256), 0, st, (const T *)x, (const T *)nullptr,
                                         (const T *)nullptr, (long long)rows, c, (const float *)nullptr, (const float *)nullptr, 0.f, 0,
                                         (float *)workspace, kSlab));
  }
  hipLaunchKernelGGL(bn_stats_finalize_kernel, dim3((c + kFinCh - 1) / kFinCh), dim3(kFinCh, kFinLanes), 0, st, (const float *)workspace, nb, (long long)rows, c, mean,
                     var, running_mean, running_var, momentum);
  NRPN_LAUNCH_CHECK("bn_stats");
  return NRPN_OK;
}

extern "C" int nrpn_bn_stats_finalize(const float *partials, int nparts, int64_t rows, int c, float *mean, float *var, float *running_mean,
                                      float *running_var, float momentum, nrpn_stream_t stream) {
  NRPN_REQUIRE(partials && mean && var && nparts > 0 && rows > 0 && c > 0, "bn_stats_finalize: bad arguments");
  hipLaunchKernelGGL(bn_stats_finalize_kernel, dim3((c + kFinCh - 1) / kFinCh), dim3(kFinCh, kFinLanes), 0, as_stream(stream), partials, nparts, (long long)rows, c,
                     mean, var, running_mean, running_var, momentum);
  NRPN_LAUNCH_CHECK("bn_stats_finalize");
  return NRPN_OK;
}

template <typename T>
__global__ void bn_apply_kernel(const T *__restrict__ x, T *__restrict__ y, long long groups, int c, const float *__restrict__ mean,
                                const float *__restrict__ var, const float *__restrict__ gamma, const float *__restrict__ beta, float eps,
                                int relu) {
  const int ct = c / 4;
  for (long long g = (long long)blockIdx.x * blockDim.x + threadIdx.x; g < groups; g += (long long)gridDim.x * blockDim.x) {
    const int cg = (int)(g % ct) * 4;
    const f4 xv = vec4<T>::ld(x + g * 4);
    const f4 mu = *reinterpret_cast<const f4 *>(mean + cg), vv = *reinterpret_cast<const f4 *>(var + cg);
    const f4 ga = *reinterpret_cast<const f4 *>(gamma + cg), be = *reinterpret_cast<const f4 *>(beta + cg);
    f4 o;
#pragma unroll
    for (int k = 0; k < 4; ++k) {
      const float is = 1.0f / sqrtf(vv[k] + eps);
      o[k] = (xv[k] - mu[k]) * is * ga[k] + be[k];
      if (relu) o[k] = fmaxf(o[k], 0.f);
    }
    vec4<T>::st(y + g * 4, o);
  }
}

static inline int ew_blocks(long long work) { long long b = (work + 255) / 256; return (int)(b > 8192 ? 8192 : (b < 1 ? 1 : b)); }

static std::atomic<int> g_bn_fast{1};
extern "C" int nrpn_set_bn_fast(int on) { g_bn_fast = on ? 1 : 0; return NRPN_OK; }
static inline int bn_fast_v(int c, int dtype) {
  if (!g_bn_fast) return 0;
  const int v = (dtype != NRPN_F32 && c % 8 == 0) ? 8 : 4;
  const int ctv = c / v;
  return (c % v == 0 && ctv > 0 && ctv <= 256 && 256 % ctv == 0) ? v : 0;
}

template <int V>
__device__ __forceinline__ void ld_params(const float *__restrict__ p, float *o) {
#pragma unroll
  for (int q = 0; q < V; q += 4) {
    const f4 v = *reinterpret_cast<const f4 *>(p + q);
    o[q] = v[0]; o[q + 1] = v[1]; o[q + 2] = v[2]; o[q + 3] = v[3];
  }
}

static inline int bn_fast_blocks(long long groups, int per_cu) {
  const long long b = (groups + 255) / 256, cap = 256ll * per_cu;
  return (int)(b > cap ? cap : (b < 1 ? 1 : b));
}

template <typename T, int V>
__global__ void __launch_bounds__(256) bn_apply_fast_kernel(const T *__restrict__ x, T *__restrict__ y, long long groups, int c,
                                                            const float *__restrict__ mean, const float *__restrict__ var,
                                                            const float *__restrict__ gamma, const float *__restrict__ beta, float eps, int relu) {
  const long long stride = (long long)gridDim.x * 256;
  long long g = (long long)blockIdx.x * 256 + threadIdx.x;
  const int cg = ((int)g & (c / V - 1)) * V;
  float mu[V], is[V], ga[V], be[V];
  ld_params<V>(mean + cg, mu); ld_params<V>(var + cg, is); ld_params<V>(gamma + cg, ga); ld_params<V>(beta + cg, be);
#pragma unroll
  for (int k = 0; k < V; ++k) is[k] = 1.0f / sqrtf(is[k] + eps);
#pragma unroll 2
  for (; g < groups; g += stride) {
    float xv[V], o[V];
    vecv<T, V>::ld(x + g * V, xv);
#pragma unroll
    for (int k = 0; k < V; ++k) {
      o[k] = (xv[k] - mu[k]) * is[k] * ga[k] + be[k];
      if (relu) o[k] = fmaxf(o[k], 0.f);
    }
    vecv<T, V>::st(y + g * V, o);
  }
}

template <typename T, int V>
__global__ void __launch_bounds__(256) bn_bwd_apply_fast_kernel(const T *__restrict__ x, const T *__restrict__ y, const T *__restrict__ dy,
                                                                T *__restrict__ dx, long long groups, int c, long long rows,
                                                                const float *__restrict__ mean, const float *__restrict__ var,
                                                                const float *__restrict__ gamma, float eps, int relu,
                                                                const float *__restrict__ dgamma, const float *__restrict__ dbeta,
                                                                const float *__restrict__ beta) {
  const float invr = 1.0f / (float)rows;
  const long long stride = (long long)gridDim.x * 256;
  long long g = (long long)blockIdx.x * 256 + threadIdx.x;
  const int cg = ((int)g & (c / V - 1)) * V;
  float mu[V], is[V], ga[V], dg[V], db[V], be[V];
  ld_params<V>(mean + cg, mu); ld_params<V>(var + cg, is); ld_params<V>(gamma + cg, ga); ld_params<V>(dgamma + cg, dg); ld_params<V>(dbeta + cg, db);
#pragma unroll
  for (int k = 0; k < V; ++k) { is[k] = 1.0f / sqrtf(is[k] + eps); be[k] = 0.f; }
  if (relu && beta) ld_params<V>(beta + cg, be);
#pragma unroll 2
  for (; g < groups; g += stride) {
    float xv[V], gv[V], o[V];
    vecv<T, V>::ld(x + g * V, xv);
    vecv<T, V>::ld(dy + g * V, gv);
    if (relu && !beta) {
      float yv[V];
      vecv<T, V>::ld(y + g * V, yv);
#pragma unroll
      for (int k = 0; k < V; ++k) gv[k] = yv[k] > 0.f ? gv[k] : 0.f;
    }
#pragma unroll
    for (int k = 0; k < V; ++k) {
      if (relu && beta && !(((xv[k] - mu[k]) * is[k] * ga[k] + be[k]) > 0.f)) gv[k] = 0.f;
      const float xh = (xv[k] - mu[k]) * is[k];
      o[k] = ga[k] * is[k] * (gv[k] - db[k] * invr - xh * dg[k] * invr);
    }
    vecv<T, V>::st(dx + g * V, o);
  }
}

extern "C" int nrpn_bn_apply(const void *x, void *y, int64_t rows, int c, int dtype, const float *mean, const float *var,
                             const float *gamma, const float *beta, float eps, int relu, nrpn_stream_t stream) {
  NRPN_REQUIRE(rows > 0 && c > 0 && c % 4 == 0, "bn_apply: C=%d must be a multiple of 4", c);
  NRPN_REQUIRE(x && y && mean && var && gamma && beta, "bn_apply: null pointer");
  int fv = bn_fast_v(c, dtype);
  if (fv == 8 && ((reinterpret_cast<uintptr_t>(x) | reinterpret_cast<uintptr_t>(y)) & 15)) fv = 0;
  const long long groups = rows * (c / (fv ? fv : 4));
  if (fv == 8)
    hipLaunchKernelGGL((bn_apply_fast_kernel<bf16s, 8>), dim3(bn_fast_blocks(groups, 8)), dim3(256), 0, as_stream(stream), (const bf16s *)x, (bf16s *)y,
                       groups, c, mean, var, gamma, beta, eps, relu);
  else if (fv == 4) {
    DISPATCH_T(dtype, hipLaunchKernelGGL((bn_apply_fast_kernel<T, 4>), dim3(bn_fast_blocks(groups, 8)), dim3(256), 0, as_stream(stream), (const T *)x,
                                         (T *)y, groups, c, mean, var, gamma, beta, eps, relu));
  } else {
    DISPATCH_T(dtype, hipLaunchKernelGGL(bn_apply_kernel<T>, dim3(ew_blocks(groups)), dim3(256), 0, as_stream(stream), (const T *)x, (T *)y,
                                         groups, c, mean, var, gamma, beta, eps, relu));
  }
  NRPN_LAUNCH_CHECK("bn_apply");
  return NRPN_OK;
}

template <typename T>
__global__ void bn_bwd_apply_kernel(const T *__restrict__ x, const T *__restrict__ y, const T *__restrict__ dy, T *__restrict__ dx,
                                    long long groups, int c, long long rows, const float *__restrict__ mean, const float *__restrict__ var,
                                    const float *__restrict__ gamma, float eps, int relu, const float *__restrict__ dgamma,
                                    const float *__restrict__ dbeta, const float *__restrict__ beta) {
  const int ct = c / 4;
  const float invr = 1.0f / (float)rows;
  for (long long g = (long long)blockIdx.x * blockDim.x + threadIdx.x; g < groups; g += (long long)gridDim.x * blockDim.x) {
    const int cg = (int)(g % ct) * 4;
    const f4 xv = vec4<T>::ld(x + g * 4);
    f4 gv = vec4<T>::ld(dy + g * 4);
    const f4 mu = *reinterpret_cast<const f4 *>(mean + cg), vv = *reinterpret_cast<const f4 *>(var + cg);
    const f4 ga = *reinterpret_cast<const f4 *>(gamma + cg);
    const f4 dg = *reinterpret_cast<const f4 *>(dgamma + cg), db = *reinterpret_cast<const f4 *>(dbeta + cg);
    if (relu && !beta) {
      const f4 yv = vec4<T>::ld(y + g * 4);
#pragma unroll
      for (int k = 0; k < 4; ++k) gv[k] = yv[k] > 0.f ? gv[k] : 0.f;
    }
    f4 be = {0, 0, 0, 0};
    if (relu && beta) be = *reinterpret_cast<const f4 *>(beta + cg);
    f4 o;
#pragma unroll
    for (int k = 0; k < 4; ++k) {
      const float is = 1.0f / sqrtf(vv[k] + eps);
      if (relu && beta && !(((xv[k] - mu[k]) * is * ga[k] + be[k]) > 0.f)) gv[k] = 0.f;
      const float xh = (xv[k] - mu[k]) * is;
      o[k] = ga[k] * is * (gv[k] - db[k] * invr - xh * dg[k] * invr);
    }
    vec4<T>::st(dx + g * 4, o);
  }
}

extern "C" int nrpn_bn_backward(const void *x, const void *y, const void *dy, void *dx, int64_t rows, int c, int dtype, const float *mean,
                                const float *var, const float *gamma, const float *beta, float eps, int relu, float *dgamma, float *dbeta,
                                float *acc_dgamma, float *acc_dbeta, void *workspace, nrpn_stream_t stream) {
  if (int rc = check_bn_shape("bn_backward", rows, c)) return rc;
  NRPN_REQUIRE(x && dy && dx && mean && var && gamma && dgamma && dbeta && workspace && (!relu || y || beta), "bn_backward: null pointer");
  const int kSlab = slab_rows(rows);
  const int nb = (int)cdiv64(rows, kSlab);
  hipStream_t st = as_stream(stream);
  if (g_chan_v8.load(std::memory_order_relaxed) && chan_v8(dtype, c, x, y, dy)) {
    hipLaunchKernelGGL((chan_partial_kernel<bf16s, 1, 8>), dim3(nb, (c + 1023) / 1024), dim3(256), 0, st, (const bf16s *)x, (const bf16s *)y,
                       (const bf16s *)dy, (long long)rows, c, mean, var, eps, relu, (float *)workspace, kSlab, gamma, beta);
  } else {
    DISPATCH_T(dtype, hipLaunchKernelGGL((chan_partial_kernel<T, 1, 4>), dim3(nb, (c + 1023) / 1024), dim3(256), 0, st, (const T *)x, (const T *)y, (const T *)dy,
                                         (long long)rows, c, mean, var, eps, relu, (float *)workspace, kSlab, gamma, beta));
  }
  hipLaunchKernelGGL(bn_bwd_finalize_kernel, dim3((c + kFinCh - 1) / kFinCh), dim3(kFinCh, kFinLanes), 0, st, (const float *)workspace, nb, c, dbeta, dgamma, acc_dbeta, acc_dgamma);
  int fv = bn_fast_v(c, dtype);
  if (fv == 8 && ((reinterpret_cast<uintptr_t>(x) | reinterpret_cast<uintptr_t>(y) | reinterpret_cast<uintptr_t>(dy) | reinterpret_cast<uintptr_t>(dx)) & 15))
    fv = 0;
  const long long groups = rows * (c / (fv ? fv : 4));
  if (fv == 8)
    hipLaunchKernelGGL((bn_bwd_apply_fast_kernel<bf16s, 8>), dim3(bn_fast_blocks(groups, 5)), dim3(256), 0, st, (const bf16s *)x, (const bf16s *)y,
                       (const bf16s *)dy, (bf16s *)dx, groups, c, (long long)rows, mean, var, gamma, eps, relu, (const float *)dgamma,
                       (const float *)dbeta, beta);
  else if (fv == 4) {
    DISPATCH_T(dtype, hipLaunchKernelGGL((bn_bwd_apply_fast_kernel<T, 4>), dim3(bn_fast_blocks(groups, 8)), dim3(256), 0, st, (const T *)x, (const T *)y,
                                         (const T *)dy, (T *)dx, groups, c, (long long)rows, mean, var, gamma, eps, relu,
                                         (const float *)dgamma, (const float *)dbeta, beta));
  } else {
    DISPATCH_T(dtype, hipLaunchKernelGGL(bn_bwd_apply_kernel<T>, dim3(ew_blocks(groups)), dim3(256), 0, st, (const T *)x, (const T *)y,
                                         (const T *)dy, (T *)dx, groups, c, (long long)rows, mean, var, gamma, eps, relu,
                                         (const float *)dgamma, (const float *)dbeta, beta));
  }
  NRPN_LAUNCH_CHECK("bn_backward");
  return NRPN_OK;
}

template <typename T>
__global__ void relu_bwd_kernel(const T *__restrict__ y, const T *__restrict__ dy, T *__restrict__ dx, long long groups) {
  for (long long g = (long long)blockIdx.x * blockDim.x + threadIdx.x; g < groups; g += (long long)gridDim.x * blockDim.x) {
    const f4 yv = vec4<T>::ld(y + g * 4);
    f4 gv = vec4<T>::ld(dy + g * 4);
#pragma unroll
    for (int k = 0; k < 4; ++k) gv[k] = yv[k] > 0.f ? gv[k] : 0.f;
    vec4<T>::st(dx + g * 4, gv);
  }
}

extern "C" int nrpn_relu_backward(const void *y, const void *dy, void *dx, int64_t count, int dtype, nrpn_stream_t stream) {
  NRPN_REQUIRE(count > 0 && count % 4 == 0, "relu_backward: count must be a positive multiple of 4");
  NRPN_REQUIRE(y && dy && dx, "relu_backward: null pointer");
  const long long groups = count / 4;
  DISPATCH_T(dtype, hipLaunchKernelGGL(relu_bwd_kernel<T>, dim3(ew_blocks(groups)), dim3(256), 0, as_stream(stream), (const T *)y,
                                       (const T *)dy, (T *)dx, groups));
  NRPN_LAUNCH_CHECK("relu_backward");
  return NRPN_OK;
}

static inline int pool_out(int in, int k, int s, int p, int ceil_mode) {
  int o = ceil_mode ? (in + 2 * p - k + s - 1) / s + 1 : (in + 2 * p - k) / s + 1;
  if (ceil_mode && (o - 1) * s >= in + p) --o;
  return o;
}
extern "C" int nrpn_pool_out_size(int in, int k, int s, int p, int ceil_mode) { return pool_out(in, k, s, p, ceil_mode); }

template <int V> struct argpack;
template <> struct argpack<4> { typedef unsigned int type; };
template <> struct argpack<8> { typedef unsigned long long type; };

template <typename T, int V, typename I>
__global__ void maxpool_fwd_kernel(const T *__restrict__ x, T *__restrict__ y, int8_t *__restrict__ arg, int n, int gx, int gy, int gz, int ox,
                                   int oy, int oz, int c, int k, int s, int p) {
  const I ct = (I)(c / V);
  const I total = (I)n * ox * oy * oz * ct;
  for (I g = (I)blockIdx.x * blockDim.x + threadIdx.x; g < total; g += (I)gridDim.x * blockDim.x) {
    const I vox = g / ct;
    const int cg = (int)(g - vox * ct) * V;
    I v = vox;
    const int z = (int)(v % (I)oz); v /= (I)oz;
    const int yy = (int)(v % (I)oy); v /= (I)oy;
    const int xx = (int)(v % (I)ox);
    const long long b = (long long)(v / (I)ox);
    float best[V];
    int bi[V];
    bool first = true;
    const int a0 = max(0, p - xx * s), a1 = min(k, gx + p - xx * s);
    const int b0 = max(0, p - yy * s), b1 = min(k, gy + p - yy * s);
    const int d0 = max(0, p - z * s), d1 = min(k, gz + p - z * s);
    for (int a = a0; a < a1; ++a) {
      const int ix = xx * s - p + a;
      for (int bq = b0; bq < b1; ++bq) {
        const int iy = yy * s - p + bq;
        for (int d = d0; d < d1; ++d) {
          const int iz = z * s - p + d;
          float xv[V];
          vecv<T, V>::ld(x + ((((b * gx + ix) * gy + iy) * gz + iz) * (long long)c + cg), xv);
          const int code = (a * k + bq) * k + d;
#pragma unroll
          for (int q = 0; q < V; ++q)
            if (first || xv[q] > best[q]) { best[q] = xv[q]; bi[q] = code; }
          first = false;
        }
      }
    }
    if (first) {
#pragma unroll
      for (int q = 0; q < V; ++q) { best[q] = -INFINITY; bi[q] = 0; }
    }
    const long long o = (long long)vox * c + cg;
    vecv<T, V>::st(y + o, best);
    if (arg) {
      typename argpack<V>::type pk = 0;
#pragma unroll
      for (int q = 0; q < V; ++q) pk |= (typename argpack<V>::type)(unsigned char)bi[q] << (8 * q);
      *reinterpret_cast<typename argpack<V>::type *>(arg + o) = pk;
    }
  }
// ... 1073 lines not shown
```

nerf_rpn_amd/lib.py:

```python
import ctypes
import os
import re
import subprocess

_HERE = os.path.dirname(os.path.abspath(__file__))
SO_PATH = os.environ.get("NRPN_LIBRARY") or os.path.join(_HERE, "libnerfrpn_hip.so")
HEADER = os.path.join(os.path.dirname(_HERE), "include", "nerfrpn.h")
TOOLS_HEADER = os.path.join(os.path.dirname(_HERE), "include", "nerfrpn_tools.h")

F32, BF16 = 0, 1
CONV_BIAS, CONV_RELU, CONV_OUT_F32 = 1, 2, 4

_lib = None

TILE_AUTO, TILE_128, TILE_256X128_WS, TILE_256X256, TILE_256X256_W4, TILE_HALO = 0, 128, 256, 512, 1024, 2048


class ConvOpts(ctypes.Structure):
    _fields_ = [("size", ctypes.c_int32), ("tile", ctypes.c_int32), ("lds_dma", ctypes.c_int32), ("kstep_bytes", ctypes.c_int32),
                ("stagger", ctypes.c_int32), ("big_split", ctypes.c_int32), ("debug", ctypes.c_int32), ("halo_pairing", ctypes.c_int32),
                ("scale", ctypes.c_void_p), ("relu_mask", ctypes.c_void_p), ("stats", ctypes.c_void_p)]

    def __init__(self, tile=0, lds_dma=-1, kstep_bytes=0, stagger=-1, big_split=-1, debug=0, scale=0, relu_mask=0, stats=0, halo_pairing=0):
        super().__init__(ctypes.sizeof(ConvOpts), tile, lds_dma, kstep_bytes, stagger, big_split, debug, halo_pairing, scale or None,
                         relu_mask or None, stats or None)

    def ptr(self):
        return ctypes.addressof(self)


class NrpnError(RuntimeError):
    pass


def build(force=False):
    if force:
        subprocess.check_call(["make", "-C", os.path.join(_HERE, "csrc"), "clean"])
    subprocess.check_call(["make", "-C", os.path.join(_HERE, "csrc"), "-j4"])
    return SO_PATH


def declared_symbols(tools=True):
    text = open(HEADER).read() + (open(TOOLS_HEADER).read() if tools else "")
    text = re.sub(r"/\*.*?\*/", "", text, flags=re.S)
    return sorted(set(re.findall(r"\b(nrpn_[a-z0-9_]+)\s*\(", text)))


def _ctype(decl):
    decl = decl.strip()
    if "*" in decl or decl.startswith("nrpn_stream_t"):
        return ctypes.c_void_p
    base = decl.replace("const", "").split()
    t = " ".join(base[:-1]) if len(base) > 1 else base[0]
    if t in ("int64_t", "long long", "size_t"):
        return ctypes.c_int64
    if t == "int":
        return ctypes.c_int
    if t == "float":
        return ctypes.c_float
    raise NrpnError(f"unmapped C type in nerfrpn.h: {decl!r}")


def _prototypes():
    text = open(HEADER).read() + open(TOOLS_HEADER).read()
    text = re.sub(r"/\*.*?\*/", "", text, flags=re.S)
    protos = {}
    for ret, name, args in re.findall(r"\b(int|size_t|int64_t|const char \*)\s*(nrpn_[a-z0-9_]+)\s*\(([^)]*)\)\s*;", text):
        args = args.strip()
        argtypes = [] if args in ("", "void") else [_ctype(a) for a in args.split(",")]
        restype = {"int": ctypes.c_int, "size_t": ctypes.c_size_t, "int64_t": ctypes.c_int64,
                   "const char *": ctypes.c_char_p}[ret]
        protos[name] = (restype, argtypes)
    return protos


def load():
    global _lib
    if _lib is not None:
        return _lib
    if not os.path.exists(SO_PATH):
        raise NrpnError(f"{SO_PATH} is missing: run `python -c 'import __graft_entry__ as g; g.build()'` "
                        "(there is no CPU fallback for the HIP path)")
    lib = ctypes.CDLL(SO_PATH)
    for name, (restype, argtypes) in _prototypes().items():
        fn = getattr(lib, name)
        fn.restype, fn.argtypes = restype, argtypes
    _lib = lib
    return lib


KNOB_EPOCH = [0]


def call(name, *args):
    lib = load()
    if name.startswith("set_"):
        KNOB_EPOCH[0] += 1
    rc = getattr(lib, "nrpn_" + name)(*args)
    if rc != 0:
        raise NrpnError(f"nrpn_{name} failed ({rc}): {lib.nrpn_last_error().decode()}")
    return rc


def query(name, *args):
    return getattr(load(), "nrpn_" + name)(*args)
```

nerf_rpn_amd/model/hip_nn.py:

```python
import torch
from torch import nn

from .. import ops


def _pack_of(mod):
    pk = mod.__dict__.get("_nrpn_pack")
    if pk is None:
        pk = ops.PackedWeight()
        mod.__dict__["_nrpn_pack"] = pk
    return pk


def conv3d(mod, x, relu=False, out_f32=False, segs=None, chain=0, stats=None, affine=None):
    k = mod.kernel_size[0]
    if k == 7:
        if mod.in_channels != 4 or mod.padding[0] != 3:
            raise NotImplementedError("k7 conv is only implemented for the 4-channel stem")
        cache = mod.__dict__.setdefault("_nrpn_stem", {})
        if affine is not None:
            return ops.StemFn.apply(x, mod.weight, mod.bias, mod.stride[0], cache, affine, relu)
        y = ops.StemFn.apply(x, mod.weight, mod.bias, mod.stride[0], cache)
        if relu:
            raise NotImplementedError("stem is always followed by BatchNorm in this model family")
        return y
    if k == 1 and mod.stride[0] > 1 and mod.padding[0] == 0:
        x = ops.SubsampleFn.apply(x, mod.stride[0])
    elif k not in (1, 3) or mod.stride[0] != 1 or mod.padding[0] != k // 2:
        raise NotImplementedError(f"Conv3d k={k} stride={mod.stride} padding={mod.padding} has no HIP kernel yet")
    if segs is not None and (k == 7 or mod.stride[0] != 1):
        raise NotImplementedError("ragged voxel lists are supported by the stride-1 k1 / k3 convolutions only")
    mode = (relu, chain, stats, affine) if affine is not None else ((relu, chain, stats) if stats is not None else ((relu, chain) if chain else relu))
    return ops.ConvFn.apply(x, _pack_of(mod), mod.out_channels, mode, out_f32, 1 if segs is None else (1, tuple(segs)), mod.weight, mod.bias)


def ragged_cat(feats):
    import torch
    n, c = feats[0].shape[0], feats[0].shape[-1]
    segs = [tuple(int(v) for v in f.shape[1:4]) for f in feats for _ in range(n)]
    x = torch.cat([f.reshape(-1, c) for f in feats], dim=0)
    return x.view(1, x.shape[0], 1, 1, c), segs


def ragged_split(x, feats):
    outs, off = [], 0
    for f in feats:
        cnt = f.shape[0] * f.shape[1] * f.shape[2] * f.shape[3]
        outs.append(x[0, off:off + cnt, 0, 0, :].view(f.shape[0], f.shape[1], f.shape[2], f.shape[3], x.shape[-1]))
        off += cnt
    return outs


class BNCounters:

    def __init__(self, root):
        self.root, self.flat, self.mods = root, None, None

    def step(self):
        if self.mods is None:
            self.mods = [m for m in self.root.modules()
                         if isinstance(m, nn.BatchNorm3d) and m.track_running_stats and m.num_batches_tracked is not None]
        if not self.mods:
            return
        stale = self.flat is None or any(m.num_batches_tracked.data_ptr() != self.flat[i].data_ptr() for i, m in enumerate(self.mods))
        if stale:
            self.flat = torch.stack([m.num_batches_tracked.detach().reshape(()) for m in self.mods]).contiguous()
            for i, m in enumerate(self.mods):
                m.num_batches_tracked = self.flat[i]
        if all(m.training for m in self.mods):
            self.flat.add_(1)
        else:
            for m in self.mods:
                if m.training:
                    m.num_batches_tracked.add_(1)


def bn_counters(root):
    c = root.__dict__.get("_nrpn_bn_counters")
    if c is None:
        c = BNCounters(root)
        root.__dict__["_nrpn_bn_counters"] = c
    return c


import os as _os

FUSED_BN_STATS = _os.environ.get("NRPN_BN_FUSED_STATS", "1") != "0"
FOLD_EVAL_BN = _os.environ.get("NRPN_BN_FOLD", "1") != "0"


def bn_fold(conv, bn):
    ts = [conv.bias, bn.weight, bn.bias, bn.running_mean, bn.running_var]
    key = tuple((t.data_ptr(), t._version) if t is not None else None for t in ts) + (bn.eps, ops._weight_epoch, ops.BN_STATS_EPOCH[0])
    ent = bn.__dict__.get("_nrpn_fold")
    if ent is None or ent[0] != key:
        with torch.no_grad():
            var = bn.running_var.detach().float()
            gamma = bn.weight.detach().float() if bn.weight is not None else torch.ones_like(var)
            beta = bn.bias.detach().float() if bn.bias is not None else torch.zeros_like(var)
            scale = gamma * torch.rsqrt(var + bn.eps)
            cb = conv.bias.detach().float() if conv.bias is not None else torch.zeros_like(var)
            shift = (cb - bn.running_mean.detach().float()) * scale + beta
        ent = (key, scale.contiguous(), shift.contiguous())
        bn.__dict__["_nrpn_fold"] = ent
    return ent[1], ent[2]


def _can_fold(conv, bn, x):
    if not FOLD_EVAL_BN or bn.training or bn.running_mean is None:
        return False
    if torch.is_grad_enabled() and (x.requires_grad or conv.weight.requires_grad):
        return False
    k = conv.kernel_size[0]
    return k == 7 or k == 1 or (k == 3 and conv.stride[0] == 1)


def conv_bn(conv, bn, x, relu, counted=False):
    if _can_fold(conv, bn, x):
        return conv3d(conv, x, relu=relu, affine=bn_fold(conv, bn))
    holder = {} if (FUSED_BN_STATS and (bn.training or bn.running_mean is None) and conv.kernel_size[0] != 7) else None
    return batch_norm(bn, conv3d(conv, x, stats=holder), relu, counted, holder)


def batch_norm(mod, x, relu, counted=False, stats=None):
    training = mod.training or mod.running_mean is None
    if mod.training and mod.track_running_stats and mod.num_batches_tracked is not None and not counted:
        mod.num_batches_tracked.add_(1)
    return ops.BatchNormFn.apply(x, mod.weight, mod.bias, mod.running_mean, mod.running_var, training,
                                 mod.momentum if mod.momentum is not None else 0.1, mod.eps, relu,
                                 stats.get("partials") if (stats and training) else None)


def max_pool(mod, x):
    k = mod.kernel_size if isinstance(mod.kernel_size, int) else mod.kernel_size[0]
    s = mod.stride if isinstance(mod.stride, int) else mod.stride[0]
    p = mod.padding if isinstance(mod.padding, int) else mod.padding[0]
    return ops.MaxPoolFn.apply(x, k, s, p, bool(mod.ceil_mode))


def run_modules(mods, x, counted=False):
    mods = list(mods)
    i = 0
    while i < len(mods):
        m = mods[i]
        nxt = mods[i + 1] if i + 1 < len(mods) else None
        nxt2 = mods[i + 2] if i + 2 < len(mods) else None
        if isinstance(m, nn.Conv3d):
            if isinstance(nxt, nn.BatchNorm3d) and _can_fold(m, nxt, x):
                fuse = isinstance(nxt2, nn.ReLU)
                x = conv3d(m, x, relu=fuse, affine=bn_fold(m, nxt))
                i += 3 if fuse else 2
            elif isinstance(nxt, nn.BatchNorm3d):
                holder = {} if (FUSED_BN_STATS and (nxt.training or nxt.running_mean is None)) else None
                x = conv3d(m, x, stats=holder)
                fuse = isinstance(nxt2, nn.ReLU)
                x = batch_norm(nxt, x, fuse, counted, holder)
                i += 3 if fuse else 2
            elif isinstance(nxt, nn.ReLU):
                x = conv3d(m, x, relu=True)
                i += 2
            else:
                x = conv3d(m, x)
                i += 1
        elif isinstance(m, nn.MaxPool3d):
            x = max_pool(m, x)
            i += 1
        elif isinstance(m, nn.Sequential):
            x = run_modules(m, x, counted)
            i += 1
        elif isinstance(m, nn.BatchNorm3d):
            fuse = isinstance(nxt, nn.ReLU)
            x = batch_norm(m, x, fuse, counted)
            i += 2 if fuse else 1
        else:
            raise NotImplementedError(f"no HIP kernel mapping for module {type(m).__name__}")
    return x


def conv_out(size, k, s, p):
    return tuple((int(g) + 2 * p - k) // s + 1 for g in size)


def module_out_size(mods, size):
    for m in mods:
        if isinstance(m, nn.Sequential):
            size = module_out_size(list(m), size)
        elif isinstance(m, nn.Conv3d):
            size = conv_out(size, m.kernel_size[0], m.stride[0], m.padding[0])
        elif isinstance(m, nn.MaxPool3d):
            k = m.kernel_size if isinstance(m.kernel_size, int) else m.kernel_size[0]
            st = m.stride if isinstance(m.stride, int) else m.stride[0]
            pd = m.padding if isinstance(m.padding, int) else m.padding[0]
            size = tuple(ops.query("pool_out_size", int(g), k, st, pd, int(bool(m.ceil_mode))) for g in size)
    return size


def as_ncdhw(x):
    return x.permute(0, 4, 1, 2, 3)


def as_ndhwc(x, dtype):
    cl = x.permute(0, 2, 3, 4, 1)
    if cl.is_contiguous() and cl.dtype == dtype:
        return cl
    return ops.to_channels_last(x, dtype)
```

nerf_rpn_amd/ops.py:

```python
import itertools
import math
from types import SimpleNamespace

import torch

from . import lib
from .lib import BF16, CONV_BIAS, CONV_OUT_F32, CONV_RELU, F32, call

_QCACHE = {"epoch": -1, "map": {}}


def query(name, *args):
    if _QCACHE["epoch"] != lib.KNOB_EPOCH[0]:
        _QCACHE["epoch"], _QCACHE["map"] = lib.KNOB_EPOCH[0], {}
    m = _QCACHE["map"]
    key = (name, args)
    v = m.get(key)
    if v is None:
        v = m[key] = lib.query(name, *args)
    return v


def _query_opts(name, opts, *args):
    if _QCACHE["epoch"] != lib.KNOB_EPOCH[0]:
# ... 565 lines not shown
        taps = weights[0][0].numel() // cin
        arena = getattr(weights[0], "_nrpn_arena", None) if len(weights) == 1 else None
        if arena is not None and rows_total == weights[0].shape[0] and arena[0].entries[arena[1]][1:4] == (taps, rows_total, cin):
            aw, idx = arena
            return aw.fwd(idx, dtype), (aw.dgrad(idx, dtype) if need_dgrad else None)
        key = tuple((w.data_ptr(), w._version) for w in weights) + (dtype, rows_total, need_dgrad, _weight_epoch)
        if key == self.key:
            return self.fwd, self.dgrad
        PACK_COUNT["conv"] += 1
        dev = weights[0].device
        padded = rows_total != sum(w.shape[0] for w in weights)
        alloc = torch.zeros if padded else torch.empty
        fwd = alloc((taps, rows_total, cin), dtype=dtype, device=dev)
        dgrad = alloc((taps, cin, rows_total), dtype=dtype, device=dev) if need_dgrad else None
        row = 0
        for w in weights:
            wc = w.detach().contiguous()
            call("pack_conv_weight", _p(wc), w.shape[0], cin, taps, _dt(fwd), _p(fwd), _p(dgrad), rows_total, row, _s())
            row += w.shape[0]
        self.key, self.fwd, self.dgrad = key, fwd, dgrad
        return fwd, dgrad



SPLIT3 = [_os.environ.get("NRPN_BF16X3", "0") == "1"]
_ACT_I, _W_I = 0b100, 0b010
_X_P, _DY_P = 0b010, 0b100


def split3(src, ipattern=None, nplanes=0, ppattern=0):
    src = src.contiguous()
    _chk(src)
    c = src.shape[-1]
    inter = torch.empty(tuple(src.shape[:-1]) + (3 * c,), dtype=torch.bfloat16, device=src.device) if ipattern is not None else None
    planes = torch.empty((nplanes,) + tuple(src.shape), dtype=torch.bfloat16, device=src.device) if nplanes else None
    call("split_bf16x3", _p(src), src.numel() // c, c, _p(inter), ipattern or 0, _p(planes), nplanes, ppattern, _s())
    return inter, planes


def _x3_ok(x, ksize, segs, rows_total, differentiable):
    return (SPLIT3[0] and x.dtype == torch.float32 and ksize == 3 and (segs is None or not differentiable)
            and x.shape[-1] % 32 == 0 and rows_total % 32 == 0)


def _x3_weights(pack, weights, wp, wpd):
    arena = getattr(weights[0], "_nrpn_arena", None) if len(weights) == 1 else None
    key = (wp.data_ptr(), wpd.data_ptr() if wpd is not None else 0, _weight_epoch, arena[0].epoch if arena is not None else pack.key)
    ent = pack.__dict__.get("x3")
    if ent is None or ent[0] != key:
        w3 = split3(wp, _W_I)[0]
        if wpd is not None:
            _wait_dgrad_operands()
        wd3 = split3(wpd, _W_I)[0] if wpd is not None else None
        ent = (key, w3, wd3)
        pack.__dict__["x3"] = ent
    return ent[1], ent[2]


def column_sum_f32(t, out=None, accumulate=False):
    t = t.contiguous()
    rows, c = t.shape
    tile = min(c, 1024)
    if c % 4 == 0 and 256 % (tile // 4) == 0 and c % tile == 0:
        mean, var = torch.empty(c, dtype=torch.float32, device=t.device), torch.empty(c, dtype=torch.float32, device=t.device)
        ws = torch.empty(query("bn_workspace_bytes", rows, c), dtype=torch.uint8, device=t.device)
        call("bn_stats", _p(t), rows, c, F32, _p(mean), _p(var), 0, 0, 0.1, _p(ws), _s())
        res = mean * float(rows)
        if out is None:
            return res
        return out.add_(res) if accumulate else out.copy_(res)
    if out is None:
        out = torch.empty(c, dtype=torch.float32, device=t.device)
    ws = torch.empty(query("column_sum_workspace_bytes", rows, c), dtype=torch.uint8, device=t.device)
    call("column_sum_f32", _p(t), rows, c, _p(out), 1 if accumulate else 0, _p(ws), _s())
    return out


def _seg_dims(segs):
    import ctypes
    flat = [int(v) for d in segs for v in d]
    return (ctypes.c_int32 * len(flat))(*flat)


def _conv_fwd(x, wp, bias, cout, wrows, ksize, flags, out_dtype, segs=None, mask=None, stats=None, scale=None, tile=0, halo_pairing=0):
    import ctypes
    n, gx, gy, gz, cin = x.shape
    y = torch.empty((n, gx, gy, gz, cout), dtype=out_dtype, device=x.device)
    if out_dtype == torch.float32 and x.dtype == torch.bfloat16:
        flags |= CONV_OUT_F32
    if bias is not None:
        flags |= CONV_BIAS
    if segs is not None and ksize != 1:
        if scale is not None or mask is not None or tile:
            raise lib.NrpnError("ragged conv launches take no per-call options")
        wsb = query("conv3d_fwd_workspace_bytes", n, gx, gy, gz, cin, cout, ksize, _dt(x))
        ws = torch.empty(wsb, dtype=torch.uint8, device=x.device) if wsb else None
        dims = _seg_dims(segs)
        call("conv3d_fwd_ragged", _p(x), _p(wp), _p(bias), _p(y), len(segs), ctypes.addressof(dims), cin, cout, wrows, ksize, _dt(x), flags,
             _p(ws), _s())
        return y
    opts = lib.ConvOpts(tile=tile or CONV_TILE[0], scale=_p(scale), relu_mask=_p(mask), halo_pairing=halo_pairing or CONV_HALO_PAIRING[0])
    if stats is not None and segs is None and mask is None and out_dtype == x.dtype and wrows == cout:
        rows = _query_opts("conv3d_fwd_stats_rows_ex", opts, n, gx, gy, gz, cin, cout, ksize, _dt(x))
        if rows > 0:
            part = torch.empty((rows, 2, cout), dtype=torch.float32, device=x.device)
            opts.stats = part.data_ptr()
            call("conv3d_fwd_ex", _p(x), _p(wp), _p(bias), _p(y), n, gx, gy, gz, cin, cout, wrows, ksize, _dt(x), flags, 0, opts.ptr(), _s())
            stats["partials"] = part
            return y
    wsb = _query_opts("conv3d_fwd_workspace_bytes_ex", opts, n, gx, gy, gz, cin, cout, ksize, _dt(x))
    ws = torch.empty(wsb, dtype=torch.uint8, device=x.device) if wsb else None
    call("conv3d_fwd_ex", _p(x), _p(wp), _p(bias), _p(y), n, gx, gy, gz, cin, cout, wrows, ksize, _dt(x), flags, _p(ws), opts.ptr(), _s())
    return y


CONV_TILE = [int(_os.environ.get("NRPN_CONV_TILE", "0"))]
CONV_HALO_PAIRING = [int(_os.environ.get("NRPN_HALO_PAIRING", "0"))]


_WGRAD_WS = {}


def _wgrad_workspace(device, key, nbytes):
    key = (device.index, _s()) + key
    ent = _WGRAD_WS.get(key)
    if ent is None or ent[0].numel() < nbytes:
        ent = [torch.empty(nbytes, dtype=torch.uint8, device=device), False]
        _WGRAD_WS[key] = ent
    ready, ent[1] = ent[1], True
    return ent[0], ready


CHAIN_MASK_INPUT_GRAD, CHAIN_GRAD_PREMASKED = 1, 2


IN_BACKWARD = [0]


class ConvFn(torch.autograd.Function):

    @staticmethod
    def forward(ctx, x, pack, rows_total, relu, out_f32, nw, *wb):
        segs = None
        chain = 0
        stats = None
        affine = None
        if isinstance(relu, tuple):
            relu, chain, *rest = relu
            stats = rest[0] if rest else None
            affine = rest[1] if len(rest) > 1 else None
        if isinstance(nw, tuple):
            nw, segs = nw
        weights, biases = wb[:nw], wb[nw:]
        _chk(x)
        ksize = weights[0].shape[2] if weights[0][0].numel() != x.shape[-1] else 1
        need_dgrad = x.requires_grad
        wp, wpd = pack.get(weights, x.dtype, rows_total, need_dgrad, x.shape[-1])
        bias = None
        if biases[0] is not None:
            if nw == 1 and biases[0].numel() == rows_total:
                bias = biases[0].detach().float().contiguous()
            else:
                bkey = tuple((b.data_ptr(), b._version) for b in biases) + (rows_total, _weight_epoch)
                if getattr(pack, "bias_key", None) != bkey:
                    parts = [b.detach().float().reshape(-1) for b in biases]
                    used = sum(p.numel() for p in parts)
                    if used < rows_total:
                        parts.append(parts[0].new_zeros(rows_total - used))
                    pack.bias, pack.bias_key = torch.cat(parts), bkey
                bias = pack.bias
        out_dtype = torch.float32 if out_f32 else x.dtype
        x3 = _x3_ok(x, ksize, segs, rows_total, any(ctx.needs_input_grad))
        xin = x
        if x3:
            wp, wpd = _x3_weights(pack, weights, wp, wpd)
            xin, stats = split3(x, _ACT_I)[0], None
        if affine is not None:
            scale, shift = affine
            y = _conv_fwd(xin, wp, shift, rows_total, rows_total, ksize, CONV_RELU if relu else 0, out_dtype, segs, None, None, scale)
            ctx.mark_non_differentiable(y)
            return y
        y = _conv_fwd(xin, wp, bias, rows_total, rows_total, ksize, CONV_RELU if relu else 0, out_dtype, segs, None, stats)
        ctx.save_for_backward(x, y if relu else None, wpd, *weights)
        ctx.x3 = x3
        ctx.meta = (rows_total, relu, nw, ksize, biases[0] is not None, segs, chain)
        ctx.sinks = ([_sink(w) for w in weights], [_sink(b) for b in biases])
        return y

    @staticmethod
    def backward(ctx, dy):
        IN_BACKWARD[0] += 1
        try:
            return ConvFn._backward(ctx, dy)
        finally:
            IN_BACKWARD[0] -= 1

    @staticmethod
    def _backward(ctx, dy):
        x, y, wpd, *weights = ctx.saved_tensors
        rows_total, relu, nw, ksize, has_bias, segs, chain = ctx.meta
        n, gx, gy, gz, cin = x.shape
        dy = dy.contiguous()
        if dy.dtype != x.dtype:
            dy = dy.to(x.dtype)
        if relu and not (chain & CHAIN_GRAD_PREMASKED):
            dyr = torch.empty_like(dy)
            yy = y if y.dtype == dy.dtype else y.to(dy.dtype)
            call("relu_backward", _p(yy), _p(dy), _p(dyr), dy.numel(), _dt(dy), _s())
            dy = dyr
        dx = None
        x3 = getattr(ctx, "x3", False)
        dyp = None
        if x3 and segs is not None:
            raise lib.NrpnError("bf16x3 backward of a ragged conv: the split dgrad / wgrad launches take no segments")
        if x3:
            dys, dyp = split3(dy, _ACT_I if ctx.needs_input_grad[0] else None, 3, _DY_P)
        if ctx.needs_input_grad[0]:
            _wait_dgrad_operands()
            mask = x if (chain & CHAIN_MASK_INPUT_GRAD) and segs is None else None
            if x3:
                dx = _conv_fwd(dys, wpd, None, cin, cin, ksize, 0, torch.float32)
                if mask is not None:
                    dxm = torch.empty_like(dx)
                    call("relu_backward", _p(x), _p(dx), _p(dxm), dx.numel(), _dt(dx), _s())
                    dx = dxm
            else:
                dx = _conv_fwd(dy, wpd, None, cin, cin, ksize, 0, x.dtype, segs, mask)
        taps = ksize ** 3
        wsinks, bsinks = ctx.sinks
        side = _wgrad_side_stream(x.device) if all(k is not None for k in wsinks) and (not has_bias or all(k is not None for k in bsinks)) else None
        wgrad = (lambda: ConvFn._wgrad_x3(ctx, x, dy, dyp, weights)) if x3 else (lambda: ConvFn._wgrad(ctx, x, dy, weights))
        if side is None:
            return (dx, None, None, None, None, None, *wgrad())
        main = torch.cuda.current_stream(x.device)
        side.wait_stream(main)
        x.record_stream(side)
        dy.record_stream(side)
        if dyp is not None:
            dyp.record_stream(side)
        _WGRAD_SIDE["keep"].append((x, dy, dyp))
        with torch.cuda.stream(side):
            res = wgrad()
        if not _WGRAD_SIDE["dirty"]:
            _WGRAD_SIDE["dirty"] = True
            torch.autograd.Variable._execution_engine.queue_callback(wgrad_stream_join)
        return (dx, None, None, None, None, None, *res)

    @staticmethod
    def _wgrad_x3(ctx, x, dy, dyp, weights):
        rows_total, relu, nw, ksize, has_bias, segs, chain = ctx.meta
        n, gx, gy, gz, cin = x.shape
        taps = ksize ** 3
        wsinks, bsinks = ctx.sinks
        xp = split3(x, None, 3, _X_P)[1]
        n3 = 3 * n
        slices = query("conv3d_wgrad_slices", n3, gx, gy, gz, cin, rows_total, rows_total, ksize, BF16)
        gwp = torch.empty((slices, taps, rows_total, cin), dtype=torch.float32, device=x.device)
        ws, mask_ready = _wgrad_workspace(x.device, (n3, gx, gy, gz, ksize, None),
                                          query("conv3d_wgrad_workspace_bytes", n3, gx, gy, gz, cin, rows_total, rows_total, ksize, BF16))
        call("conv3d_wgrad", _p(xp), _p(dyp), _p(gwp), 0, n3, gx, gy, gz, cin, rows_total, rows_total, ksize, BF16, 2 if mask_ready else 0, _p(ws), _s())
        res = _deliver_wgrad(weights, wsinks, bsinks, gwp, None, 0, slices, rows_total, cin, taps, False, False, False)
        gbs = _deliver_bias_x3(dy.reshape(-1, rows_total), weights, bsinks) if has_bias else tuple([None] * nw)
        return (*res[:nw], *gbs)

    @staticmethod
    def _wgrad(ctx, x, dy, weights):
        rows_total, relu, nw, ksize, has_bias, segs, chain = ctx.meta
        n, gx, gy, gz, cin = x.shape
        taps = ksize ** 3
        wsinks, bsinks = ctx.sinks
        slices = query("conv3d_wgrad_slices", n, gx, gy, gz, cin, rows_total, rows_total, ksize, _dt(x))
        gwp = torch.empty((slices, taps, rows_total, cin), dtype=torch.float32, device=x.device)
        direct_bias = has_bias and nw == 1 and bsinks[0] is not None
        gb = bsinks[0].slot if direct_bias else (torch.empty(rows_total, dtype=torch.float32, device=x.device) if has_bias else None)
        ws, mask_ready = _wgrad_workspace(x.device, (n, gx, gy, gz, ksize, segs),
                                          query("conv3d_wgrad_workspace_bytes", n, gx, gy, gz, cin, rows_total, rows_total, ksize, _dt(x)))
        fused_reduce = nw == 1 and wsinks[0] is not None and wsinks[0].flat is not None and rows_total == weights[0].shape[0]
        defer_bias = fused_reduce and direct_bias
        wflags = int(direct_bias) | (2 if mask_ready else 0) | (4 if defer_bias else 0)
        if segs is None or ksize == 1:
            call("conv3d_wgrad", _p(x), _p(dy), _p(gwp), _p(gb), n, gx, gy, gz, cin, rows_total, rows_total, ksize, _dt(x), wflags, _p(ws), _s())
        else:
            import ctypes
            dims = _seg_dims(segs)
            call("conv3d_wgrad_ragged", _p(x), _p(dy), _p(gwp), _p(gb), len(segs), ctypes.addressof(dims), cin, rows_total, rows_total, ksize,
                 _dt(x), wflags, _p(ws), _s())
        bias_part = ws.data_ptr() + query("conv3d_wgrad_bias_offset", n, gx, gy, gz, ksize) if defer_bias else 0
        return _deliver_wgrad(weights, wsinks, bsinks, gwp, gb, bias_part, slices, rows_total, cin, taps, has_bias, direct_bias, defer_bias)


def _deliver_wgrad(weights, wsinks, bsinks, gwp, gb, bias_part, slices, rows_total, cin, taps, has_bias, direct_bias, defer_bias):
    nw = len(weights)
    gws, gbs, row = [], [], 0
    for i, w in enumerate(weights):
        if wsinks[i] is not None and wsinks[i].flat is not None and nw == 1 and rows_total == w.shape[0]:
            call("reduce_slices", _p(gwp), slices, gwp[0].numel(), _p(wsinks[i].flat), 1, bias_part if defer_bias else 0, rows_total, rows_total,
                 _p(gb) if defer_bias else 0, 1, _s())
            wsinks[i].notify()
            gws.append(None)
        elif wsinks[i] is not None:
            if not wsinks[i].slot.is_contiguous():
                raise lib.NrpnError("a GEMM-layout arena weight reached a fused multi-weight GEMM (mark the module _nrpn_fused_gemm)")
            call("unpack_conv_wgrad", _p(gwp), w.shape[0], cin, taps, rows_total, row, _p(wsinks[i].slot), 1, slices, _s())
            wsinks[i].notify()
            gws.append(None)
        else:
            gw = torch.empty_like(w, dtype=torch.float32)
            call("unpack_conv_wgrad", _p(gwp), w.shape[0], cin, taps, rows_total, row, _p(gw), 0, slices, _s())
            gws.append(gw)
        if not has_bias:
# ... 319 lines not shown


STEM_HALO = [_os.environ.get("NRPN_STEM_HALO", "1") != "0"]


class StemFn(torch.autograd.Function):

    @staticmethod
    def forward(ctx, x, weight, bias, stride, cache, affine=None, relu=False):
        _chk(x)
        n, gx, gy, gz, _ = x.shape
        cout = weight.shape[0]
        halo = STEM_HALO[0] and bool(query("stem_halo_supported", gz, cout, stride, _dt(x)))
        key = (weight.data_ptr(), weight._version, x.dtype, _weight_epoch, halo)
        if cache.get("key") != key:
            PACK_COUNT["stem"] += 1
            wc = weight.detach().contiguous()
            if halo:
                wp = torch.empty((cout, query("stem_halo_kpad")), dtype=x.dtype, device=x.device)
                call("pack_stem_weight_halo", _p(wc), cout, _p(wp), _s())
            else:
                kpad = query("stem_kpad", _dt(x))
                wp = torch.empty((cout, kpad), dtype=x.dtype, device=x.device)
                call("pack_stem_weight", _p(wc), cout, _dt(x), _p(wp), _s())
            cache["key"], cache["wp"] = key, wp
        wp = cache["wp"]
        o = [(g - 1) // stride + 1 for g in (gx, gy, gz)]
        y = torch.empty((n, o[0], o[1], o[2], cout), dtype=x.dtype, device=x.device)
        if affine is not None:
            scale, shift = affine
            if halo:
                call("conv3d_stem_fwd_halo", _p(x), _p(wp), _p(shift), _p(scale), _p(y), n, gx, gy, gz, cout, CONV_BIAS | (CONV_RELU if relu else 0), _s())
            else:
                opts = lib.ConvOpts(scale=_p(scale))
                call("conv3d_stem_fwd_ex", _p(x), _p(wp), _p(shift), _p(y), n, gx, gy, gz, cout, stride, _dt(x),
                     CONV_BIAS | (CONV_RELU if relu else 0), opts.ptr(), _s())
            ctx.mark_non_differentiable(y)
            return y
        b = bias.detach().float().contiguous() if bias is not None else None
        if halo:
            call("conv3d_stem_fwd_halo", _p(x), _p(wp), _p(b), 0, _p(y), n, gx, gy, gz, cout, CONV_BIAS if b is not None else 0, _s())
        else:
            call("conv3d_stem_fwd", _p(x), _p(wp), _p(b), _p(y), n, gx, gy, gz, cout, stride, _dt(x), CONV_BIAS if b is not None else 0, _s())
        ctx.save_for_backward(x, weight)
        ctx.meta = (stride, bias is not None)
        ctx.sinks = (_sink(weight), _sink(bias))
        return y

    @staticmethod
    def backward(ctx, dy):
        x, weight = ctx.saved_tensors
        stride, has_bias = ctx.meta
        dy = dy.contiguous()
        n, gx, gy, gz, _ = x.shape
        cout = weight.shape[0]
        kpad = query("stem_kpad", _dt(x))
        slices = query("stem_wgrad_slices", n, gx, gy, gz, cout, stride, _dt(x))
        per = query("stem_wgrad_slice_floats", n, gx, gy, gz, cout, stride, _dt(x))
        gwp = torch.empty((slices, per), dtype=torch.float32, device=x.device)
        wsink, bsink = ctx.sinks
        direct_bias = has_bias and bsink is not None
        gb = bsink.slot if direct_bias else (torch.empty(cout, dtype=torch.float32, device=x.device) if has_bias else None)
        ws = torch.empty(query("stem_wgrad_workspace_bytes", n, gx, gy, gz, cout, stride, _dt(x)), dtype=torch.uint8, device=x.device) if has_bias else None
        call("conv3d_stem_wgrad", _p(x), _p(dy), _p(gwp), _p(gb), n, gx, gy, gz, cout, stride, _dt(x), int(direct_bias), _p(ws), _s())
        if wsink is not None:
            call("unpack_stem_wgrad", _p(gwp), cout, _dt(x), _p(wsink.slot), 1, slices, per, _s())
            wsink.notify()
            gw = None
        else:
            gw = torch.empty_like(weight, dtype=torch.float32)
            call("unpack_stem_wgrad", _p(gwp), cout, _dt(x), _p(gw), 0, slices, per, _s())
        if direct_bias:
            bsink.notify()
            gb = None
        return None, gw, gb, None, None, None, None


BN_STATS_EPOCH = [0]


class BatchNormFn(torch.autograd.Function):

    @staticmethod
    def forward(ctx, x, gamma, beta, rmean, rvar, training, momentum, eps, relu, partials=None):
        _chk(x)
        c = x.shape[-1]
        rows = x.numel() // c
        dev = x.device
        g32, b32 = gamma.detach().float().contiguous(), beta.detach().float().contiguous()
        if training:
            BN_STATS_EPOCH[0] += 1
            mean = torch.empty(c, dtype=torch.float32, device=dev)
            var = torch.empty(c, dtype=torch.float32, device=dev)
            if partials is not None:
                call("bn_stats_finalize", _p(partials), partials.shape[0], rows, c, _p(mean), _p(var), _p(rmean), _p(rvar), float(momentum), _s())
            else:
                ws = torch.empty(query("bn_workspace_bytes", rows, c), dtype=torch.uint8, device=dev)
                call("bn_stats", _p(x), rows, c, _dt(x), _p(mean), _p(var), _p(rmean), _p(rvar), float(momentum), _p(ws), _s())
        else:
            mean, var = rmean.float().contiguous(), rvar.float().contiguous()
        y = torch.empty_like(x)
        call("bn_apply", _p(x), _p(y), rows, c, _dt(x), _p(mean), _p(var), _p(g32), _p(b32), float(eps), int(relu), _s())
        ctx.save_for_backward(x, mean, var, g32, b32)
        ctx.meta = (training, eps, relu)
        ctx.sinks = (_sink(gamma), _sink(beta))
        return y

    @staticmethod
    def backward(ctx, dy):
        x, mean, var, g32, b32 = ctx.saved_tensors
        training, eps, relu = ctx.meta
        if not training:
            raise lib.NrpnError("BatchNorm backward in eval mode is not supported by the HIP path")
        dy = dy.contiguous()
        c = x.shape[-1]
        rows = x.numel() // c
        dev = x.device
        dx = torch.empty_like(x)
        dgamma = torch.empty(c, dtype=torch.float32, device=dev)
        dbeta = torch.empty(c, dtype=torch.float32, device=dev)
        ws = torch.empty(query("bn_workspace_bytes", rows, c), dtype=torch.uint8, device=dev)
        gsink, bsink = ctx.sinks
        call("bn_backward", _p(x), 0, _p(dy), _p(dx), rows, c, _dt(x), _p(mean), _p(var), _p(g32), _p(b32), float(eps), int(relu), _p(dgamma),
             _p(dbeta), _p(gsink.slot) if gsink is not None else 0, _p(bsink.slot) if bsink is not None else 0, _p(ws), _s())
        if gsink is not None:
            gsink.notify()
            dgamma = None
        if bsink is not None:
            bsink.notify()
            dbeta = None
        return dx, dgamma, dbeta, None, None, None, None, None, None, None


class MaxPoolFn(torch.autograd.Function):
    @staticmethod
    def forward(ctx, x, k, s, p, ceil_mode):
        _chk(x)
        n, gx, gy, gz, c = x.shape
        o = [query("pool_out_size", g, k, s, p, int(ceil_mode)) for g in (gx, gy, gz)]
        y = torch.empty((n, o[0], o[1], o[2], c), dtype=x.dtype, device=x.device)
        arg = torch.empty(y.shape, dtype=torch.int8, device=x.device) if x.requires_grad else None
        call("maxpool3d_fwd", _p(x), _p(y), _p(arg), n, gx, gy, gz, c, k, s, p, int(ceil_mode), _dt(x), _s())
        ctx.save_for_backward(arg)
        ctx.meta = (x.shape, k, s, p, ceil_mode)
        return y

    @staticmethod
    def backward(ctx, dy):
        (arg,) = ctx.saved_tensors
        shape, k, s, p, ceil_mode = ctx.meta
        dy = dy.contiguous()
        n, gx, gy, gz, c = shape
        dx = torch.empty(shape, dtype=dy.dtype, device=dy.device)
        call("maxpool3d_bwd", _p(dy), _p(arg), _p(dx), n, gx, gy, gz, c, k, s, p, int(ceil_mode), _dt(dy), _s())
        return dx, None, None, None, None


class UpsampleAddFn(torch.autograd.Function):

    @staticmethod
    def forward(ctx, fine, coarse):
        _chk(fine, coarse)
        n, fx, fy, fz, c = fine.shape
        _, cx, cy, cz, _ = coarse.shape
        call("upsample_add_fwd", _p(fine), _p(coarse), n, fx, fy, fz, cx, cy, cz, c, _dt(fine), _s())
        ctx.mark_dirty(fine)
        ctx.meta = (fine.shape, coarse.shape)
        return fine

    @staticmethod
    def backward(ctx, d):
        fshape, cshape = ctx.meta
        d = d.contiguous()
        n, fx, fy, fz, c = fshape
        _, cx, cy, cz, _ = cshape
        dc = torch.empty(cshape, dtype=d.dtype, device=d.device)
        call("upsample_add_bwd", _p(d), _p(dc), n, fx, fy, fz, cx, cy, cz, c, _dt(d), 0, _s())
        return d, dc


class SubsampleFn(torch.autograd.Function):

    @staticmethod
    def forward(ctx, x, s):
        _chk(x)
        n, gx, gy, gz, c = x.shape
        o = [(g - 1) // s + 1 for g in (gx, gy, gz)]
        y = torch.empty((n, o[0], o[1], o[2], c), dtype=x.dtype, device=x.device)
        call("subsample3d", _p(x), _p(y), n, gx, gy, gz, c, s, 0, _dt(x), _s())
        ctx.meta = (x.shape, s)
        return y

    @staticmethod
    def backward(ctx, dy):
        shape, s = ctx.meta
        dy = dy.contiguous()
        n, gx, gy, gz, c = shape
        dx = torch.empty(shape, dtype=dy.dtype, device=dy.device)
        call("subsample3d", _p(dy), _p(dx), n, gx, gy, gz, c, s, 1, _dt(dy), _s())
        return dx, None


class AddReluFn(torch.autograd.Function):

    @staticmethod
    def forward(ctx, a, b, relu):
        a, b = a.contiguous(), b.contiguous()
        _chk(a, b)
        y = torch.empty_like(a)
        call("add_relu", _p(a), _p(b), _p(y), a.numel(), int(relu), _dt(a), _s())
        ctx.relu = relu
        ctx.save_for_backward(y if relu else None)
        return y

# ... 1373 lines not shown
```

Measured before the change: 115.5 scenes/sec.

## Fuse BatchNorm backward ReLU mask and reductions into conv dgrad epilogue

When a BatchNorm (optionally with ReLU) feeds a conv, the conv's data-gradient kernel epilogue now applies the BN-ReLU mask to its bf16 output. It also accumulates per-channel sum(dy) and sum(dy*xhat) partials, in both the direct tile path and a new split-K epilogue kernel. BN backward then calls a lighter finish kernel that consumes these partials instead of re-reading x and dy for a separate reduction pass. This removes one full-activation read pass per BN layer in backward. In exchange it adds epilogue register and LDS pressure, an extended opts struct with versioning, and Python-side link tracking between the BN and the following conv.

```diff
diff --git a/include/nerfrpn.h b/include/nerfrpn.h
--- a/include/nerfrpn.h
+++ b/include/nerfrpn.h
@@ -108,6 +108,14 @@
   const float *scale;
   const void *relu_mask;
   float *stats;
+  const void *bn_x;
+  const float *bn_mean;
+  const float *bn_var;
+  const float *bn_gamma;
+  const float *bn_beta;
+  float bn_eps;
+  int32_t bn_relu;
+  float *bn_sums;
 } nrpn_conv_opts;
 int nrpn_conv3d_fwd_ex(const void *x, const void *wp, const float *bias, void *y, int n, int gx, int gy, int gz, int cin,
                        int cout, int wrows, int ksize, int dtype, int flags, void *workspace, const nrpn_conv_opts *opts,
@@ -116,6 +124,7 @@
                                           const nrpn_conv_opts *opts);
 int nrpn_conv3d_fwd_plan_ex(int n, int gx, int gy, int gz, int cin, int cout, int ksize, int dtype, const nrpn_conv_opts *opts);
 int nrpn_conv3d_fwd_stats_rows_ex(int n, int gx, int gy, int gz, int cin, int cout, int ksize, int dtype, const nrpn_conv_opts *opts);
+int nrpn_conv3d_bn_bwd_rows_ex(int n, int gx, int gy, int gz, int cin, int cout, int ksize, int dtype, const nrpn_conv_opts *opts);
 size_t nrpn_conv3d_wgrad_workspace_bytes(int n, int gx, int gy, int gz, int cin, int cout, int wrows, int ksize, int dtype);
 int nrpn_conv3d_wgrad_slices(int n, int gx, int gy, int gz, int cin, int cout, int wrows, int ksize, int dtype);
 enum { NRPN_WGRAD_ACC_BIAS = 1, NRPN_WGRAD_MASK_READY = 2,
@@ -173,6 +182,9 @@
 int nrpn_bn_backward(const void *x, const void *y, const void *dy, void *dx, int64_t rows, int c, int dtype,
                      const float *mean, const float *var, const float *gamma, const float *beta, float eps, int relu,
                      float *dgamma, float *dbeta, float *acc_dgamma, float *acc_dbeta, void *workspace, nrpn_stream_t stream);
+int nrpn_bn_backward_finish(const void *x, const void *dy_masked, void *dx, int64_t rows, int c, int dtype, const float *mean,
+                            const float *var, const float *gamma, const float *beta, float eps, const float *partials, int nparts,
+                            float *dgamma, float *dbeta, float *acc_dgamma, float *acc_dbeta, nrpn_stream_t stream);
 int nrpn_relu_backward(const void *y, const void *dy, void *dx, int64_t count, int dtype, nrpn_stream_t stream);
 int nrpn_pool_out_size(int in, int k, int s, int p, int ceil_mode);
 int nrpn_maxpool3d_fwd(const void *x, void *y, int8_t *argmax, int n, int gx, int gy, int gz, int c, int k, int s,
diff --git a/nerf_rpn_amd/csrc/common.h b/nerf_rpn_amd/csrc/common.h
--- a/nerf_rpn_amd/csrc/common.h
+++ b/nerf_rpn_amd/csrc/common.h
@@ -55,6 +55,15 @@
 __device__ __forceinline__ float bf16_bits_to_f32(unsigned short h) { return __uint_as_float(((unsigned)h) << 16); }
 __device__ __forceinline__ unsigned short f32_to_bf16_bits(float f) { return __builtin_bit_cast(unsigned short, (__bf16)f); }
 
+__device__ __forceinline__ float bn_invstd(float var, float eps) { return 1.0f / sqrtf(var + eps); }
+__device__ __forceinline__ float bn_xhat(float x, float mean, float invstd) { return __fmul_rn(__fsub_rn(x, mean), invstd); }
+__device__ __forceinline__ float bn_affine(float x, float mean, float invstd, float gamma, float beta) {
+  return __fmaf_rn(bn_xhat(x, mean, invstd), gamma, beta);
+}
+__device__ __forceinline__ bool bn_relu_on(float x, float mean, float invstd, float gamma, float beta) {
+  return bn_affine(x, mean, invstd, gamma, beta) > 0.f;
+}
+
 template <typename T> struct elem;
 template <> struct elem<float> {
   static __device__ __forceinline__ float ld(const float *p) { return *p; }
diff --git a/nerf_rpn_amd/csrc/conv3d.hip b/nerf_rpn_amd/csrc/conv3d.hip
--- a/nerf_rpn_amd/csrc/conv3d.hip
+++ b/nerf_rpn_amd/csrc/conv3d.hip
@@ -1,10 +1,12 @@
 #include "conv_common.cuh"
+#include <cstddef>
+#include <cstring>
 
 #ifndef NRPN_HALO_PAIRING_DEFAULT
 #define NRPN_HALO_PAIRING_DEFAULT 2
 #endif
 
-template <typename T, int BN, int MODE, bool OUTF32, int KB, bool GLDS, int BM = 128, bool ROWS = false>
+template <typename T, int BN, int MODE, bool OUTF32, int KB, bool GLDS, int BM = 128, bool ROWS = false, bool BNB = false>
 __global__ void __launch_bounds__(256, BM == 128 ? 2 : 1) conv_igemm_kernel(const ConvArgs p) {
   constexpr int WAVES_N = (BN == 128) ? 2 : 1;
   constexpr int TM = BM / (32 * (4 / WAVES_N));
@@ -305,6 +307,8 @@
     const T *maskp = reinterpret_cast<const T *>(p.mask);
     T *yp = reinterpret_cast<T *>(p.y);
     const bool full_tile = m0 + BM <= p.M;
+    BnbLane bnb;
+    if constexpr (BNB) bnb_init(bnb, p, lds + 4 * (TM * 32 * PITCH) + wave * 1024, n0 + wn * 64, lane);
 #pragma unroll
     for (int j = 0; j < TN; ++j) {
       const int col = n0 + (wn * TN + j) * 32 + fr;
@@ -344,10 +348,13 @@
 #pragma unroll
           for (int e = 0; e < 8; ++e) ov[e] = (bf16_bits_to_f32(mk[e]) > 0.f) ? ov[e] : (unsigned short)0;
           val = __builtin_bit_cast(f4, ov);
+        } else if constexpr (BNB) {
+          val = bnb_piece(bnb, p.bn_relu, reinterpret_cast<const bf16s *>(p.bn_x) + v * p.Cout + col, val);
         }
         *reinterpret_cast<f4 *>(yp + v * p.Cout + col) = val;
       }
     }
+    if constexpr (BNB) bnb_flush(bnb, p, stage, (m0 / BM) * (BM / (TM * 32)) + wm, n0 + wn * 64, lane);
     return;
   }
 #pragma unroll
@@ -1154,6 +1161,72 @@
     if (OUTF32) reinterpret_cast<float *>(y)[dst] = o;
     else elem<T>::st(reinterpret_cast<T *>(y) + dst, o);
   }
+}
+
+__global__ void __launch_bounds__(256) splitk_epilogue_bnb_kernel(const ConvArgs p, int slab) {
+  __shared__ float red[2][256][8];
+  const int ct = p.Cout / 8, ty_n = 256 / ct;
+  const int tx = threadIdx.x % ct, ty = threadIdx.x / ct;
+  const long long r0 = (long long)blockIdx.x * slab, r1 = min(p.M, r0 + slab), total = p.M * p.Cout;
+  float mu[8], is[8], ga[8], be[8], s0[8], s1[8];
+#pragma unroll
+  for (int k = 0; k < 8; ++k) {
+    mu[k] = p.bn_mean[tx * 8 + k]; is[k] = bn_invstd(p.bn_var[tx * 8 + k], p.bn_eps); ga[k] = p.bn_gamma[tx * 8 + k];
+    be[k] = p.bn_relu ? p.bn_beta[tx * 8 + k] : 0.f; s0[k] = 0.f; s1[k] = 0.f;
+  }
+  bf16s *yp = reinterpret_cast<bf16s *>(p.y);
+  for (long long r = r0 + ty; r < r1; r += ty_n) {
+    const long long i = r * p.Cout + tx * 8;
+    f4 lo = *reinterpret_cast<const f4 *>(p.ws + i), hi = *reinterpret_cast<const f4 *>(p.ws + i + 4);
+    for (int z = 1; z < p.ksplit; ++z) {
+      lo += *reinterpret_cast<const f4 *>(p.ws + z * total + i);
+      hi += *reinterpret_cast<const f4 *>(p.ws + z * total + i + 4);
+    }
+    bnb_u8v ov;
+#pragma unroll
+    for (int k = 0; k < 4; ++k) { ov[k] = f32_to_bf16_bits(lo[k]); ov[4 + k] = f32_to_bf16_bits(hi[k]); }
+    const bnb_u8v xv = __builtin_bit_cast(bnb_u8v, ldg16(reinterpret_cast<const bf16s *>(p.bn_x) + i));
+#pragma unroll
+    for (int k = 0; k < 8; ++k) {
+      unsigned short o = ov[k];
+      bnb_elem(bf16_bits_to_f32(xv[k]), mu[k], is[k], ga[k], be[k], p.bn_relu, o, s0[k], s1[k]);
+      ov[k] = o;
+    }
+    *reinterpret_cast<f4 *>(yp + i) = __builtin_bit_cast(f4, ov);
+  }
+#pragma unroll
+  for (int k = 0; k < 8; ++k) { red[0][threadIdx.x][k] = s0[k]; red[1][threadIdx.x][k] = s1[k]; }
+  __syncthreads();
+  if (threadIdx.x < ct) {
+    float s[8], q[8];
+#pragma unroll
+    for (int k = 0; k < 8; ++k) { s[k] = 0.f; q[k] = 0.f; }
+    for (int l = 0; l < ty_n; ++l)
+#pragma unroll
+      for (int k = 0; k < 8; ++k) { s[k] += red[0][l * ct + threadIdx.x][k]; q[k] += red[1][l * ct + threadIdx.x][k]; }
+    float *out = p.bn_sums + (long long)blockIdx.x * 2 * p.Cout + threadIdx.x * 8;
+#pragma unroll
+    for (int k = 0; k < 8; k += 4) {
+      *reinterpret_cast<f4 *>(out + k) = f4{s[k], s[k + 1], s[k + 2], s[k + 3]};
+      *reinterpret_cast<f4 *>(out + p.Cout + k) = f4{q[k], q[k + 1], q[k + 2], q[k + 3]};
+    }
+  }
+}
+static bool splitk_bnb_ok(int cout) { const int ct = cout / 8; return (cout & 7) == 0 && ct >= 1 && ct <= 256 && (ct & (ct - 1)) == 0; }
+static int splitk_bnb_slab(long long M, int cout) {
+  const int ty_n = 256 / (cout / 8);
+  return (int)(cdiv64(cdiv64(M, 256), ty_n) * ty_n);
+}
+
+constexpr size_t kConvOptsV1 = offsetof(nrpn_conv_opts, bn_x);
+static int normalise_opts(const nrpn_conv_opts *&o, nrpn_conv_opts &full, const char *who) {
+  if (!o || o->size == (int32_t)sizeof(nrpn_conv_opts)) return 0;
+  if (o->size != (int32_t)kConvOptsV1) return nrpn_fail(NRPN_ERR_ARG, "%s: opts->size must be sizeof(nrpn_conv_opts)", who);
+  memset(&full, 0, sizeof full);
+  memcpy(&full, o, kConvOptsV1);
+  full.size = (int32_t)sizeof full;
+  o = &full;
+  return 0;
 }
 
 struct Knobs {
@@ -1288,6 +1361,10 @@
     const bool staged = MODE == 0 && sizeof(T) == 2 && !out_f32 && (a.Cout & 7) == 0 && a.ksplit <= 1 && !big && (huge || wide);
     if (!staged) return nrpn_fail(NRPN_ERR_ARG, "conv3d_fwd_stats: this shape does not run a kernel with fused statistics (ask nrpn_conv3d_fwd_stats_rows first)");
   }
+  if (a.bn_sums && a.ksplit <= 1) {
+    const bool staged = MODE == 0 && sizeof(T) == 2 && !out_f32 && (a.Cout & 7) == 0 && !big && !huge && bn == 128 && wide && kn.glds && a.segs.n == 0;
+    if (!staged) return nrpn_fail(NRPN_ERR_ARG, "conv3d_fwd_ex: this shape does not run a kernel with fused BatchNorm backward sums (ask nrpn_conv3d_bn_bwd_rows_ex first)");
+  }
   dim3 grid((unsigned)(cdiv64(a.M, bm) * ((a.Cout + (huge ? 256 : bn) - 1) / (huge ? 256 : bn)) * (a.ksplit > 1 ? a.ksplit : 1)));
   if (a.tail_ks > 1) {
     if (kind != 1) return nrpn_fail(NRPN_ERR_ARG, "conv3d_fwd: internal: tail split planned for a shape that does not run the 256x256 tile");
@@ -1344,6 +1421,8 @@
         hipLaunchKernelGGL(conv_igemm_ws_kernel<false>, grid, dim3(512), lds_, st, a);
       }
     }
+  } else if (a.bn_sums && a.ksplit <= 1) {
+    if constexpr (MODE == 0 && sizeof(T) == 2) rc = launch_igemm(conv_igemm_kernel<T, 128, 0, false, 128, true, 128, false, true>, grid, 2 * (size_t)(128 + 128) * 128, st, a);
   } else if (bn == 64) { if (out_f32) NRPN_LC2(64, true); else NRPN_LC2(64, false); }
   else { if (out_f32) NRPN_LC2(128, true); else NRPN_LC2(128, false); }
 #undef NRPN_LBIG
@@ -1401,6 +1480,10 @@
   ConvArgs a{};
   a.x = x; a.w = wp; a.bias = bias; a.mask = mask; a.y = y; a.stats = stats;
   a.scale = opts ? opts->scale : nullptr;
+  if (opts && opts->bn_sums) {
+    a.bn_x = opts->bn_x; a.bn_mean = opts->bn_mean; a.bn_var = opts->bn_var; a.bn_gamma = opts->bn_gamma; a.bn_beta = opts->bn_beta;
+    a.bn_eps = opts->bn_eps; a.bn_relu = opts->bn_relu ? 1 : 0; a.bn_sums = opts->bn_sums;
+  }
   a.M = M;
   a.X = gx; a.Y = gy; a.Z = gz; a.OX = gx; a.OY = gy; a.OZ = gz;
   if (segs) a.segs = *segs;
@@ -1451,6 +1534,12 @@
   const int blocks = (int)min((long long)4096, (total + 255) / 256);
   const float *b = (flags & NRPN_CONV_BIAS) ? bias : nullptr;
   const int relu = (flags & NRPN_CONV_RELU) ? 1 : 0;
+  if (a.bn_sums) {
+    const int slab = splitk_bnb_slab(a.M, cout);
+    hipLaunchKernelGGL(splitk_epilogue_bnb_kernel, dim3((unsigned)cdiv64(a.M, slab)), dim3(256), 0, st, a, slab);
+    NRPN_LAUNCH_CHECK("splitk_epilogue (bn sums)");
+    return NRPN_OK;
+  }
   if (dtype == NRPN_F32 || out_f32) {
     if (dtype == NRPN_F32) hipLaunchKernelGGL((splitk_epilogue_kernel<float, true>), dim3(blocks), dim3(256), 0, st, a.ws, b, y, total, cout, relu, nsl, (const float *)a.mask, a.scale);
     else hipLaunchKernelGGL((splitk_epilogue_kernel<bf16s, true>), dim3(blocks), dim3(256), 0, st, a.ws, b, y, total, cout, relu, nsl, (const bf16s *)a.mask, a.scale);
@@ -1485,6 +1574,17 @@
   return fwd_stats_rows((long long)n * gx * gy * gz, cin, cout, ksize, dtype, resolve_knobs(opts), Grid{n, gx, gy, gz});
 }
 
+static int bn_bwd_rows(long long M, int cin, int cout, int ksize, int dtype, const Knobs &kn, const Grid &g) {
+  if (dtype != NRPN_BF16 || (cout & 7) != 0 || !kn.glds || kn.bm == 256) return 0;
+  const int plan = fwd_plan(M, cin, cout, ksize, dtype, kn, g);
+  if (plan == 2 || plan == 3) return splitk_bnb_ok(cout) ? (int)cdiv64(M, splitk_bnb_slab(M, cout)) : 0;
+  if (plan == 0 && cout > 64) return fwd_stats_rows(M, cin, cout, ksize, dtype, kn, g);
+  return 0;
+}
+extern "C" int nrpn_conv3d_bn_bwd_rows_ex(int n, int gx, int gy, int gz, int cin, int cout, int ksize, int dtype, const nrpn_conv_opts *opts) {
+  return bn_bwd_rows((long long)n * gx * gy * gz, cin, cout, ksize, dtype, resolve_knobs(opts), Grid{n, gx, gy, gz});
+}
+
 extern "C" int nrpn_conv3d_fwd_stats(const void *x, const void *wp, const float *bias, void *y, int n, int gx, int gy, int gz, int cin,
                                      int cout, int wrows, int ksize, int dtype, int flags, float *stats, nrpn_stream_t stream) {
   NRPN_REQUIRE(n > 0 && gx > 0 && gy > 0 && gz > 0 && stats, "conv3d_fwd_stats: bad sizes / null statistics buffer");
@@ -1498,7 +1598,8 @@
                                   int cout, int wrows, int ksize, int dtype, int flags, void *workspace, const nrpn_conv_opts *opts,
                                   nrpn_stream_t stream) {
   NRPN_REQUIRE(n > 0 && gx > 0 && gy > 0 && gz > 0, "conv3d_fwd_ex: bad sizes");
-  NRPN_REQUIRE(!opts || opts->size == (int32_t)sizeof(nrpn_conv_opts), "conv3d_fwd_ex: opts->size must be sizeof(nrpn_conv_opts)");
+  nrpn_conv_opts full;
+  if (int rc = normalise_opts(opts, full, "conv3d_fwd_ex")) return rc;
   const void *mask = opts ? opts->relu_mask : nullptr;
   float *stats = opts ? opts->stats : nullptr;
   NRPN_REQUIRE(!mask || !(flags & NRPN_CONV_OUT_F32) || dtype == NRPN_F32, "conv3d_fwd_ex: relu_mask needs outputs in the input dtype");
@@ -1507,6 +1608,18 @@
                      wrows == cout && !mask,
                  "conv3d_fwd_ex: this shape / plan does not run a kernel with fused statistics (nrpn_conv3d_fwd_stats_rows_ex)");
     workspace = nullptr;
+  }
+  if (opts && opts->bn_sums) {
+    const Knobs kn = resolve_knobs(opts);
+    const Grid g{n, gx, gy, gz};
+    const long long M = (long long)n * gx * gy * gz;
+    NRPN_REQUIRE(bn_bwd_rows(M, cin, cout, ksize, dtype, kn, g) > 0 && !(flags & (NRPN_CONV_OUT_F32 | NRPN_CONV_BIAS | NRPN_CONV_RELU)) && wrows == cout &&
+                     !mask && !stats && !opts->scale,
+                 "conv3d_fwd_ex: this shape / plan / flag set has no fused BatchNorm backward sums (nrpn_conv3d_bn_bwd_rows_ex)");
+    NRPN_REQUIRE(opts->bn_x && opts->bn_mean && opts->bn_var && opts->bn_gamma && (opts->bn_beta || !opts->bn_relu), "conv3d_fwd_ex: bn_sums needs bn_x, bn_mean, bn_var, bn_gamma (and bn_beta with bn_relu)");
+    const int plan = fwd_plan(M, cin, cout, ksize, dtype, kn, g);
+    NRPN_REQUIRE((plan != 2 && plan != 3) || workspace, "conv3d_fwd_ex: bn_sums on a K-sliced plan needs the workspace (nrpn_conv3d_fwd_workspace_bytes_ex)");
+    if (plan != 2 && plan != 3) workspace = nullptr;
   }
   return conv3d_fwd_impl(x, wp, bias, mask, y, (long long)n * gx * gy * gz, gx, gy, gz, nullptr, cin, cout, wrows, ksize, dtype, flags,
                          workspace, stream, stats, opts);
@@ -1632,8 +1745,9 @@
   NRPN_REQUIRE(dtype == NRPN_F32 || dtype == NRPN_BF16, "stem: bad dtype %d", dtype);
   NRPN_REQUIRE(n > 0 && gx > 0 && gy > 0 && gz > 0 && cout > 0, "stem: bad sizes");
   NRPN_REQUIRE(x && wp && y, "stem: null pointer");
-  NRPN_REQUIRE(!opts || opts->size == (int32_t)sizeof(nrpn_conv_opts), "stem: opts->size must be sizeof(nrpn_conv_opts)");
-  NRPN_REQUIRE(!opts || (!opts->relu_mask && !opts->stats), "stem: relu_mask / stats are not available on the stem");
+  nrpn_conv_opts full;
+  if (int rc = normalise_opts(opts, full, "stem")) return rc;
+  NRPN_REQUIRE(!opts || (!opts->relu_mask && !opts->stats && !opts->bn_sums), "stem: relu_mask / stats / bn_sums are not available on the stem");
   ConvArgs a{};
   a.x = x; a.w = wp; a.bias = bias; a.y = y;
   a.scale = opts ? opts->scale : nullptr;
diff --git a/nerf_rpn_amd/csrc/conv_common.cuh b/nerf_rpn_amd/csrc/conv_common.cuh
--- a/nerf_rpn_amd/csrc/conv_common.cuh
+++ b/nerf_rpn_amd/csrc/conv_common.cuh
@@ -122,7 +122,71 @@
   const unsigned *rows;
   FastDiv dvz, dvy, dvs;
   float *stats;
+  const void *bn_x;
+  const float *bn_mean, *bn_var, *bn_gamma, *bn_beta;
+  float bn_eps;
+  int bn_relu;
+  float *bn_sums;
 };
+
+struct BnbLane {
+  const float *par;
+  float s0[8], s1[8];
+};
+__device__ __forceinline__ void bnb_elem(float x, float mu, float is, float ga, float be, int relu, unsigned short &o, float &s0, float &s1) {
+  const float xh = bn_xhat(x, mu, is);
+  if (relu && !(__fmaf_rn(xh, ga, be) > 0.f)) o = (unsigned short)0;
+  const float g = bf16_bits_to_f32(o);
+  s0 += g;
+  s1 = __fmaf_rn(g, xh, s1);
+}
+__device__ __forceinline__ void bnb_init(BnbLane &b, const ConvArgs &p, char *par_bytes, int col0, int lane) {
+  float *par = reinterpret_cast<float *>(par_bytes);
+  const int col = col0 + lane;
+  const bool ok = col < p.Cout;
+  par[lane] = ok ? p.bn_mean[col] : 0.f;
+  par[64 + lane] = ok ? bn_invstd(p.bn_var[col], p.bn_eps) : 0.f;
+  par[128 + lane] = ok ? p.bn_gamma[col] : 0.f;
+  par[192 + lane] = (ok && p.bn_relu) ? p.bn_beta[col] : 0.f;
+  asm volatile("s_waitcnt lgkmcnt(0)" ::: "memory");
+  b.par = par + (lane & 7) * 8;
+#pragma unroll
+  for (int k = 0; k < 8; ++k) { b.s0[k] = 0.f; b.s1[k] = 0.f; }
+}
+typedef __attribute__((ext_vector_type(8))) unsigned short bnb_u8v;
+__device__ __forceinline__ f4 bnb_piece(BnbLane &b, int relu, const bf16s *xrow, f4 val) {
+  const bnb_u8v xv = __builtin_bit_cast(bnb_u8v, ldg16(xrow));
+  bnb_u8v ov = __builtin_bit_cast(bnb_u8v, val);
+#pragma unroll
+  for (int h = 0; h < 2; ++h) {
+    const f4 mu = *reinterpret_cast<const f4 *>(b.par + 4 * h), is = *reinterpret_cast<const f4 *>(b.par + 64 + 4 * h);
+    const f4 ga = *reinterpret_cast<const f4 *>(b.par + 128 + 4 * h), be = *reinterpret_cast<const f4 *>(b.par + 192 + 4 * h);
+#pragma unroll
+    for (int k = 0; k < 4; ++k) {
+      unsigned short o = ov[4 * h + k];
+      bnb_elem(bf16_bits_to_f32(xv[4 * h + k]), mu[k], is[k], ga[k], be[k], relu, o, b.s0[4 * h + k], b.s1[4 * h + k]);
+      ov[4 * h + k] = o;
+    }
+  }
+  return __builtin_bit_cast(f4, ov);
+}
+__device__ __forceinline__ void bnb_flush(const BnbLane &b, const ConvArgs &p, char *red_bytes, long long prow, int col0, int lane) {
+  float *red = reinterpret_cast<float *>(red_bytes);
+  asm volatile("s_waitcnt lgkmcnt(0)" ::: "memory");
+#pragma unroll
+  for (int k = 0; k < 8; ++k) { red[k * 64 + lane] = b.s0[k]; red[(8 + k) * 64 + lane] = b.s1[k]; }
+  asm volatile("s_waitcnt lgkmcnt(0)" ::: "memory");
+  const int seg = lane >> 3, e = lane & 7;
+  float s = 0.f, q = 0.f;
+#pragma unroll
+  for (int g = 0; g < 8; ++g) { s += red[e * 64 + g * 8 + seg]; q += red[(8 + e) * 64 + g * 8 + seg]; }
+  const int col = col0 + lane;
+  if (col < p.Cout) {
+    p.bn_sums[(prow * 2) * p.Cout + col] = s;
+    p.bn_sums[(prow * 2 + 1) * p.Cout + col] = q;
+  }
+  asm volatile("s_waitcnt lgkmcnt(0)" ::: "memory");
+}
 
 __device__ __forceinline__ void store_col_stats(float *stats, long long pidx, int cout, int col, float s, float q, int lane) {
   s += __shfl_xor(s, 32, 64);
diff --git a/nerf_rpn_amd/csrc/elementwise.hip b/nerf_rpn_amd/csrc/elementwise.hip
--- a/nerf_rpn_amd/csrc/elementwise.hip
+++ b/nerf_rpn_amd/csrc/elementwise.hip
@@ -75,7 +75,7 @@
 #pragma unroll
       for (int k = 0; k < V; ++k) {
         mu[k] = mean[tx * V + k];
-        is[k] = 1.0f / sqrtf(var[tx * V + k] + eps);
+        is[k] = bn_invstd(var[tx * V + k], eps);
         if (beta) { ga[k] = gamma[tx * V + k]; be[k] = beta[tx * V + k]; }
       }
     }
@@ -91,7 +91,7 @@
         vecv<T, V>::ld(dy + r * c + tx * V, g);
         if (relu && beta) {
 #pragma unroll
-          for (int k = 0; k < V; ++k) g[k] = ((xv[k] - mu[k]) * is[k] * ga[k] + be[k]) > 0.f ? g[k] : 0.f;
+          for (int k = 0; k < V; ++k) g[k] = bn_relu_on(xv[k], mu[k], is[k], ga[k], be[k]) ? g[k] : 0.f;
         } else if (relu) {
           float yv[V];
           vecv<T, V>::ld(y + r * c + tx * V, yv);
@@ -99,7 +99,7 @@
           for (int k = 0; k < V; ++k) g[k] = yv[k] > 0.f ? g[k] : 0.f;
         }
 #pragma unroll
-        for (int k = 0; k < V; ++k) { s0[k] += g[k]; s1[k] += g[k] * ((xv[k] - mu[k]) * is[k]); }
+        for (int k = 0; k < V; ++k) { s0[k] += g[k]; s1[k] += g[k] * bn_xhat(xv[k], mu[k], is[k]); }
       }
     }
   }
@@ -248,8 +248,8 @@
     f4 o;
 #pragma unroll
     for (int k = 0; k < 4; ++k) {
-      const float is = 1.0f / sqrtf(vv[k] + eps);
-      o[k] = (xv[k] - mu[k]) * is * ga[k] + be[k];
+      const float is = bn_invstd(vv[k], eps);
+      o[k] = bn_affine(xv[k], mu[k], is, ga[k], be[k]);
       if (relu) o[k] = fmaxf(o[k], 0.f);
     }
     vec4<T>::st(y + g * 4, o);
@@ -291,14 +291,14 @@
   float mu[V], is[V], ga[V], be[V];
   ld_params<V>(mean + cg, mu); ld_params<V>(var + cg, is); ld_params<V>(gamma + cg, ga); ld_params<V>(beta + cg, be);
 #pragma unroll
-  for (int k = 0; k < V; ++k) is[k] = 1.0f / sqrtf(is[k] + eps);
+  for (int k = 0; k < V; ++k) is[k] = bn_invstd(is[k], eps);
 #pragma unroll 2
   for (; g < groups; g += stride) {
     float xv[V], o[V];
     vecv<T, V>::ld(x + g * V, xv);
 #pragma unroll
     for (int k = 0; k < V; ++k) {
-      o[k] = (xv[k] - mu[k]) * is[k] * ga[k] + be[k];
+      o[k] = bn_affine(xv[k], mu[k], is[k], ga[k], be[k]);
       if (relu) o[k] = fmaxf(o[k], 0.f);
     }
     vecv<T, V>::st(y + g * V, o);
@@ -319,7 +319,7 @@
   float mu[V], is[V], ga[V], dg[V], db[V], be[V];
   ld_params<V>(mean + cg, mu); ld_params<V>(var + cg, is); ld_params<V>(gamma + cg, ga); ld_params<V>(dgamma + cg, dg); ld_params<V>(dbeta + cg, db);
 #pragma unroll
-  for (int k = 0; k < V; ++k) { is[k] = 1.0f / sqrtf(is[k] + eps); be[k] = 0.f; }
+  for (int k = 0; k < V; ++k) { is[k] = bn_invstd(is[k], eps); be[k] = 0.f; }
   if (relu && beta) ld_params<V>(beta + cg, be);
 #pragma unroll 2
   for (; g < groups; g += stride) {
@@ -334,8 +334,8 @@
     }
 #pragma unroll
     for (int k = 0; k < V; ++k) {
-      if (relu && beta && !(((xv[k] - mu[k]) * is[k] * ga[k] + be[k]) > 0.f)) gv[k] = 0.f;
-      const float xh = (xv[k] - mu[k]) * is[k];
+      if (relu && beta && !bn_relu_on(xv[k], mu[k], is[k], ga[k], be[k])) gv[k] = 0.f;
+      const float xh = bn_xhat(xv[k], mu[k], is[k]);
       o[k] = ga[k] * is[k] * (gv[k] - db[k] * invr - xh * dg[k] * invr);
     }
     vecv<T, V>::st(dx + g * V, o);
@@ -387,9 +387,9 @@
     f4 o;
 #pragma unroll
     for (int k = 0; k < 4; ++k) {
-      const float is = 1.0f / sqrtf(vv[k] + eps);
-      if (relu && beta && !(((xv[k] - mu[k]) * is * ga[k] + be[k]) > 0.f)) gv[k] = 0.f;
-      const float xh = (xv[k] - mu[k]) * is;
+      const float is = bn_invstd(vv[k], eps);
+      if (relu && beta && !bn_relu_on(xv[k], mu[k], is, ga[k], be[k])) gv[k] = 0.f;
+      const float xh = bn_xhat(xv[k], mu[k], is);
       o[k] = ga[k] * is * (gv[k] - db[k] * invr - xh * dg[k] * invr);
     }
     vec4<T>::st(dx + g * 4, o);
@@ -430,6 +430,34 @@
                                          (const float *)dgamma, (const float *)dbeta, beta));
   }
   NRPN_LAUNCH_CHECK("bn_backward");
+  return NRPN_OK;
+}
+
+extern "C" int nrpn_bn_backward_finish(const void *x, const void *dy_masked, void *dx, int64_t rows, int c, int dtype, const float *mean,
+                                       const float *var, const float *gamma, const float *beta, float eps, const float *partials, int nparts,
+                                       float *dgamma, float *dbeta, float *acc_dgamma, float *acc_dbeta, nrpn_stream_t stream) {
+  (void)beta;
+  NRPN_REQUIRE(rows > 0 && c > 0 && c % 4 == 0, "bn_backward_finish: C=%d must be a multiple of 4", c);
+  NRPN_REQUIRE(x && dy_masked && dx && mean && var && gamma && dgamma && dbeta && partials && nparts > 0, "bn_backward_finish: null pointer");
+  hipStream_t st = as_stream(stream);
+  hipLaunchKernelGGL(bn_bwd_finalize_kernel, dim3((c + kFinCh - 1) / kFinCh), dim3(kFinCh, kFinLanes), 0, st, partials, nparts, c, dbeta, dgamma, acc_dbeta, acc_dgamma);
+  int fv = bn_fast_v(c, dtype);
+  if (fv == 8 && ((reinterpret_cast<uintptr_t>(x) | reinterpret_cast<uintptr_t>(dy_masked) | reinterpret_cast<uintptr_t>(dx)) & 15)) fv = 0;
+  const long long groups = rows * (c / (fv ? fv : 4));
+  if (fv == 8)
+    hipLaunchKernelGGL((bn_bwd_apply_fast_kernel<bf16s, 8>), dim3(bn_fast_blocks(groups, 5)), dim3(256), 0, st, (const bf16s *)x, (const bf16s *)nullptr,
+                       (const bf16s *)dy_masked, (bf16s *)dx, groups, c, (long long)rows, mean, var, gamma, eps, 0, (const float *)dgamma,
+                       (const float *)dbeta, (const float *)nullptr);
+  else if (fv == 4) {
+    DISPATCH_T(dtype, hipLaunchKernelGGL((bn_bwd_apply_fast_kernel<T, 4>), dim3(bn_fast_blocks(groups, 8)), dim3(256), 0, st, (const T *)x, (const T *)nullptr,
+                                         (const T *)dy_masked, (T *)dx, groups, c, (long long)rows, mean, var, gamma, eps, 0,
+                                         (const float *)dgamma, (const float *)dbeta, (const float *)nullptr));
+  } else {
+    DISPATCH_T(dtype, hipLaunchKernelGGL(bn_bwd_apply_kernel<T>, dim3(ew_blocks(groups)), dim3(256), 0, st, (const T *)x, (const T *)nullptr,
+                                         (const T *)dy_masked, (T *)dx, groups, c, (long long)rows, mean, var, gamma, eps, 0,
+                                         (const float *)dgamma, (const float *)dbeta, (const float *)nullptr));
+  }
+  NRPN_LAUNCH_CHECK("bn_backward_finish");
   return NRPN_OK;
 }
 
diff --git a/nerf_rpn_amd/lib.py b/nerf_rpn_amd/lib.py
--- a/nerf_rpn_amd/lib.py
+++ b/nerf_rpn_amd/lib.py
@@ -19,11 +19,18 @@
 class ConvOpts(ctypes.Structure):
     _fields_ = [("size", ctypes.c_int32), ("tile", ctypes.c_int32), ("lds_dma", ctypes.c_int32), ("kstep_bytes", ctypes.c_int32),
                 ("stagger", ctypes.c_int32), ("big_split", ctypes.c_int32), ("debug", ctypes.c_int32), ("halo_pairing", ctypes.c_int32),
-                ("scale", ctypes.c_void_p), ("relu_mask", ctypes.c_void_p), ("stats", ctypes.c_void_p)]
+                ("scale", ctypes.c_void_p), ("relu_mask", ctypes.c_void_p), ("stats", ctypes.c_void_p),
+                ("bn_x", ctypes.c_void_p), ("bn_mean", ctypes.c_void_p), ("bn_var", ctypes.c_void_p), ("bn_gamma", ctypes.c_void_p),
+                ("bn_beta", ctypes.c_void_p), ("bn_eps", ctypes.c_float), ("bn_relu", ctypes.c_int32), ("bn_sums", ctypes.c_void_p)]
 
     def __init__(self, tile=0, lds_dma=-1, kstep_bytes=0, stagger=-1, big_split=-1, debug=0, scale=0, relu_mask=0, stats=0, halo_pairing=0):
         super().__init__(ctypes.sizeof(ConvOpts), tile, lds_dma, kstep_bytes, stagger, big_split, debug, halo_pairing, scale or None,
                          relu_mask or None, stats or None)
+
+    def set_bn(self, x, mean, var, gamma, beta, eps, relu, sums=0):
+        self.bn_x, self.bn_mean, self.bn_var, self.bn_gamma, self.bn_beta = x or None, mean or None, var or None, gamma or None, beta or None
+        self.bn_eps, self.bn_relu, self.bn_sums = float(eps), int(bool(relu)), sums or None
+        return self
 
     def ptr(self):
         return ctypes.addressof(self)
diff --git a/nerf_rpn_amd/model/hip_nn.py b/nerf_rpn_amd/model/hip_nn.py
--- a/nerf_rpn_amd/model/hip_nn.py
+++ b/nerf_rpn_amd/model/hip_nn.py
@@ -12,7 +12,7 @@
     return pk
 
 
-def conv3d(mod, x, relu=False, out_f32=False, segs=None, chain=0, stats=None, affine=None):
+def conv3d(mod, x, relu=False, out_f32=False, segs=None, chain=0, stats=None, affine=None, link=None):
     k = mod.kernel_size[0]
     if k == 7:
         if mod.in_channels != 4 or mod.padding[0] != 3:
@@ -30,6 +30,8 @@
         raise NotImplementedError(f"Conv3d k={k} stride={mod.stride} padding={mod.padding} has no HIP kernel yet")
     if segs is not None and (k == 7 or mod.stride[0] != 1):
         raise NotImplementedError("ragged voxel lists are supported by the stride-1 k1 / k3 convolutions only")
+    if link is not None and segs is None and mod.stride[0] == 1:
+        return ops.ConvFn.apply(x, _pack_of(mod), mod.out_channels, (relu, chain, stats, affine, link), out_f32, 1, mod.weight, mod.bias)
     mode = (relu, chain, stats, affine) if affine is not None else ((relu, chain, stats) if stats is not None else ((relu, chain) if chain else relu))
     return ops.ConvFn.apply(x, _pack_of(mod), mod.out_channels, mode, out_f32, 1 if segs is None else (1, tuple(segs)), mod.weight, mod.bias)
 
@@ -86,6 +88,7 @@
 import os as _os
 
 FUSED_BN_STATS = _os.environ.get("NRPN_BN_FUSED_STATS", "1") != "0"
+FUSED_BN_BWD = _os.environ.get("NRPN_BN_FUSED_BWD", "1") != "0"
 FOLD_EVAL_BN = _os.environ.get("NRPN_BN_FOLD", "1") != "0"
 
 
@@ -122,13 +125,13 @@
     return batch_norm(bn, conv3d(conv, x, stats=holder), relu, counted, holder)
 
 
-def batch_norm(mod, x, relu, counted=False, stats=None):
+def batch_norm(mod, x, relu, counted=False, stats=None, link=None):
     training = mod.training or mod.running_mean is None
     if mod.training and mod.track_running_stats and mod.num_batches_tracked is not None and not counted:
         mod.num_batches_tracked.add_(1)
     return ops.BatchNormFn.apply(x, mod.weight, mod.bias, mod.running_mean, mod.running_var, training,
                                  mod.momentum if mod.momentum is not None else 0.1, mod.eps, relu,
-                                 stats.get("partials") if (stats and training) else None)
+                                 stats.get("partials") if (stats and training) else None, link if training else None)
 
 
 def max_pool(mod, x):
@@ -141,10 +144,12 @@
 def run_modules(mods, x, counted=False):
     mods = list(mods)
     i = 0
+    pending = None
     while i < len(mods):
         m = mods[i]
         nxt = mods[i + 1] if i + 1 < len(mods) else None
         nxt2 = mods[i + 2] if i + 2 < len(mods) else None
+        link, pending = pending, None
         if isinstance(m, nn.Conv3d):
             if isinstance(nxt, nn.BatchNorm3d) and _can_fold(m, nxt, x):
                 fuse = isinstance(nxt2, nn.ReLU)
@@ -152,15 +157,19 @@
                 i += 3 if fuse else 2
             elif isinstance(nxt, nn.BatchNorm3d):
                 holder = {} if (FUSED_BN_STATS and (nxt.training or nxt.running_mean is None)) else None
-                x = conv3d(m, x, stats=holder)
+                x = conv3d(m, x, stats=holder, link=link)
                 fuse = isinstance(nxt2, nn.ReLU)
-                x = batch_norm(nxt, x, fuse, counted, holder)
                 i += 3 if fuse else 2
+                after = mods[i] if i < len(mods) else None
+                if (FUSED_BN_BWD and (nxt.training or nxt.running_mean is None) and torch.is_grad_enabled() and isinstance(after, nn.Conv3d)
+                        and after.kernel_size[0] in (1, 3) and after.stride[0] == 1):
+                    pending = ops.BnLink()
+                x = batch_norm(nxt, x, fuse, counted, holder, pending)
             elif isinstance(nxt, nn.ReLU):
-                x = conv3d(m, x, relu=True)
+                x = conv3d(m, x, relu=True, link=link)
                 i += 2
             else:
-                x = conv3d(m, x)
+                x = conv3d(m, x, link=link)
                 i += 1
         elif isinstance(m, nn.MaxPool3d):
             x = max_pool(m, x)
diff --git a/nerf_rpn_amd/ops.py b/nerf_rpn_amd/ops.py
--- a/nerf_rpn_amd/ops.py
+++ b/nerf_rpn_amd/ops.py
@@ -671,7 +671,18 @@
     return (ctypes.c_int32 * len(flat))(*flat)
 
 
-def _conv_fwd(x, wp, bias, cout, wrows, ksize, flags, out_dtype, segs=None, mask=None, stats=None, scale=None, tile=0, halo_pairing=0):
+class BnLink:
+    __slots__ = ("x", "y_ptr", "mean", "var", "g32", "b32", "eps", "relu", "partials", "dy", "dy_version")
+
+    def __init__(self):
+        self.x = self.y_ptr = self.mean = self.var = self.g32 = self.b32 = self.eps = self.relu = None
+        self.partials = self.dy = self.dy_version = None
+
+    def clear_backward(self):
+        self.partials = self.dy = self.dy_version = None
+
+
+def _conv_fwd(x, wp, bias, cout, wrows, ksize, flags, out_dtype, segs=None, mask=None, stats=None, scale=None, tile=0, halo_pairing=0, bn=None):
     import ctypes
     n, gx, gy, gz, cin = x.shape
     y = torch.empty((n, gx, gy, gz, cout), dtype=out_dtype, device=x.device)
@@ -699,6 +710,15 @@
             return y
     wsb = _query_opts("conv3d_fwd_workspace_bytes_ex", opts, n, gx, gy, gz, cin, cout, ksize, _dt(x))
     ws = torch.empty(wsb, dtype=torch.uint8, device=x.device) if wsb else None
+    if (bn is not None and segs is None and mask is None and scale is None and bias is None and flags == 0 and out_dtype == x.dtype
+            and x.dtype == torch.bfloat16 and wrows == cout and bn.x.dtype == x.dtype and bn.x.shape == y.shape):
+        rows = _query_opts("conv3d_bn_bwd_rows_ex", opts, n, gx, gy, gz, cin, cout, ksize, _dt(x))
+        if rows > 0:
+            part = torch.empty((rows, 2, cout), dtype=torch.float32, device=x.device)
+            opts.set_bn(_p(bn.x), _p(bn.mean), _p(bn.var), _p(bn.g32), _p(bn.b32), bn.eps, bn.relu, part.data_ptr())
+            call("conv3d_fwd_ex", _p(x), _p(wp), _p(bias), _p(y), n, gx, gy, gz, cin, cout, wrows, ksize, _dt(x), flags, _p(ws), opts.ptr(), _s())
+            bn.partials, bn.dy, bn.dy_version = part, y, y._version
+            return y
     call("conv3d_fwd_ex", _p(x), _p(wp), _p(bias), _p(y), n, gx, gy, gz, cin, cout, wrows, ksize, _dt(x), flags, _p(ws), opts.ptr(), _s())
     return y
 
@@ -734,10 +754,12 @@
         chain = 0
         stats = None
         affine = None
+        link = None
         if isinstance(relu, tuple):
             relu, chain, *rest = relu
             stats = rest[0] if rest else None
             affine = rest[1] if len(rest) > 1 else None
+            link = rest[2] if len(rest) > 2 else None
         if isinstance(nw, tuple):
             nw, segs = nw
         weights, biases = wb[:nw], wb[nw:]
@@ -772,6 +794,7 @@
         y = _conv_fwd(xin, wp, bias, rows_total, rows_total, ksize, CONV_RELU if relu else 0, out_dtype, segs, None, stats)
         ctx.save_for_backward(x, y if relu else None, wpd, *weights)
         ctx.x3 = x3
+        ctx.bn_link = link if (link is not None and link.y_ptr == x.data_ptr() and not x3 and segs is None) else None
         ctx.meta = (rows_total, relu, nw, ksize, biases[0] is not None, segs, chain)
         ctx.sinks = ([_sink(w) for w in weights], [_sink(b) for b in biases])
         return y
@@ -814,7 +837,7 @@
                     call("relu_backward", _p(x), _p(dx), _p(dxm), dx.numel(), _dt(dx), _s())
                     dx = dxm
             else:
-                dx = _conv_fwd(dy, wpd, None, cin, cin, ksize, 0, x.dtype, segs, mask)
+                dx = _conv_fwd(dy, wpd, None, cin, cin, ksize, 0, x.dtype, segs, mask, bn=getattr(ctx, "bn_link", None))
         taps = ksize ** 3
         wsinks, bsinks = ctx.sinks
         side = _wgrad_side_stream(x.device) if all(k is not None for k in wsinks) and (not has_bias or all(k is not None for k in bsinks)) else None
@@ -1300,7 +1323,7 @@
 class BatchNormFn(torch.autograd.Function):
 
     @staticmethod
-    def forward(ctx, x, gamma, beta, rmean, rvar, training, momentum, eps, relu, partials=None):
+    def forward(ctx, x, gamma, beta, rmean, rvar, training, momentum, eps, relu, partials=None, link=None):
         _chk(x)
         c = x.shape[-1]
         rows = x.numel() // c
@@ -1320,6 +1343,9 @@
         y = torch.empty_like(x)
         call("bn_apply", _p(x), _p(y), rows, c, _dt(x), _p(mean), _p(var), _p(g32), _p(b32), float(eps), int(relu), _s())
         ctx.save_for_backward(x, mean, var, g32, b32)
+        ctx.bn_link = link if training else None
+        if ctx.bn_link is not None:
+            link.x, link.y_ptr, link.mean, link.var, link.g32, link.b32, link.eps, link.relu = x, y.data_ptr(), mean, var, g32, b32, float(eps), bool(relu)
         ctx.meta = (training, eps, relu)
         ctx.sinks = (_sink(gamma), _sink(beta))
         return y
@@ -1339,15 +1365,26 @@
         dbeta = torch.empty(c, dtype=torch.float32, device=dev)
         ws = torch.empty(query("bn_workspace_bytes", rows, c), dtype=torch.uint8, device=dev)
         gsink, bsink = ctx.sinks
-        call("bn_backward", _p(x), 0, _p(dy), _p(dx), rows, c, _dt(x), _p(mean), _p(var), _p(g32), _p(b32), float(eps), int(relu), _p(dgamma),
-             _p(dbeta), _p(gsink.slot) if gsink is not None else 0, _p(bsink.slot) if bsink is not None else 0, _p(ws), _s())
+        link = getattr(ctx, "bn_link", None)
+        part = None
+        if link is not None:
+            if (link.dy is not None and dy.data_ptr() == link.dy.data_ptr() and dy.shape == link.dy.shape and dy.dtype == link.dy.dtype
+                    and dy._version == link.dy_version):
+                part = link.partials
+            link.clear_backward()
+        if part is not None:
+            call("bn_backward_finish", _p(x), _p(dy), _p(dx), rows, c, _dt(x), _p(mean), _p(var), _p(g32), _p(b32), float(eps), _p(part),
+                 part.shape[0], _p(dgamma), _p(dbeta), _p(gsink.slot) if gsink is not None else 0, _p(bsink.slot) if bsink is not None else 0, _s())
+        else:
+            call("bn_backward", _p(x), 0, _p(dy), _p(dx), rows, c, _dt(x), _p(mean), _p(var), _p(g32), _p(b32), float(eps), int(relu), _p(dgamma),
+                 _p(dbeta), _p(gsink.slot) if gsink is not None else 0, _p(bsink.slot) if bsink is not None else 0, _p(ws), _s())
         if gsink is not None:
             gsink.notify()
             dgamma = None
         if bsink is not None:
             bsink.notify()
             dbeta = None
-        return dx, dgamma, dbeta, None, None, None, None, None, None, None
+        return dx, dgamma, dbeta, None, None, None, None, None, None, None, None
 
 
 class MaxPoolFn(torch.autograd.Function):
```

Result: no change. 116.2 scenes/sec, median of 6 (+0.5%).
